# mateomarin/two_towers

Hardware: AMD Instinct MI355X
Metric: training pairs/sec at global batch=8192, 1/2/4/8 GPUs; MRR@10 match (higher is better)
Workload: dtype bf16; 1 GPU; BASELINE configs[2]: EnhancedTwoTowerModel(300, 256), seq_len 64, batch 8192 per GPU, bf16, hard-negative mining k=5 + margin 0.2, dropout 0.1, Adam; global_batch=8192, seq_len=64, hidden=256, embedding_dim=300, parallelism=dp1, loss=hardneg_margin

## Files before the change

include/tt_hip.h:

```cpp
#ifndef TT_HIP_H
#define TT_HIP_H
#include <stdint.h>

#ifdef __cplusplus
extern "C" {
#endif

#define TT_OK 0
#define TT_EINVAL 1000
#define TT_DT_F32 0
#define TT_DT_BF16 1

const char* tt_version(void);
const char* tt_last_error(void);
int tt_set_option(const char* name, int value);
int tt_get_option(const char* name, int* value);

int tt_embed_gather(int dtype, const void* table, long vocab, int ep, const int32_t* ids, long n,
                    void* out, void* stream);

int tt_pack_rows(int dtype, const float* src, long n, int e, int ep, void* out, void* stream);
typedef struct {
  const float* src;
  const float* src2;
  void* dst;
  int rows, cols, dcols;
  long lds, ldd;
  int dst_bf16;
} tt_pack_job;
int tt_pack_multi(const tt_pack_job* jobs, int njobs, void* stream);

int tt_cast(int dtype, const float* x, long n, void* y, void* stream);

int tt_colsum(const float* x, long rows, int cols, long ld, float* out, int accumulate, void* stream);

typedef struct {
  const void* a[4];
  const void* b[4];
  void* c[4];
  const float* bias[4];
  int bshift[4];
  const void* a_hi[4];
  int a_split;
  uint32_t drop_row0;
} tt_gemm_batch;

int tt_gemm(int dtype, int out_dtype, int a_kouter, int b_kouter, int m, int n, int k,
            const tt_gemm_batch* batch, int nbatch, long lda, long ldb, long ldc, float alpha,
            int beta_accum, int relu, int seq_t, uint32_t drop_seed, float drop_p, int splits,
            float* splitk_ws, void* stream);
long tt_gemm_ws_size(int m, int n, int nbatch, int splits);
int tt_gemm_pick_splits(int m, int n, int k, int nbatch);

typedef struct {
  const void* g;
  const void* whh;
  const float* bhn;
  void* y;
  void* x1;
  void* save;
  float* hstate;
  int dir;
  uint32_t drop_seed;
  int drop_col0;
  uint32_t drop_row0;
} tt_gru_fwd_rec;

int tt_gru_fwd(int dtype, const tt_gru_fwd_rec* recs, int nrec, int B, int T, int H, long ldg,
               long ldy, float drop_p, void* ws, long ws_bytes, void* stream);
int tt_gru_fwd_launches(int dtype, int T, int H);
long tt_gru_fwd_ws_size(int dtype, int nrec, int B, int T, int H, long ldg, long ldy);
int tt_gru_fwd_launches_for(int dtype, int nrec, int B, int T, int H, long ldg, long ldy);

typedef struct {
  const void* g; const void* whh; const float* bhn;
  void* y;
  void* hfinal;
  void* scratch;
  int dir;
} tt_gru_infer_rec;
int  tt_gru_fwd_infer(int dtype, const tt_gru_infer_rec* recs, int nrec, int B, int T, int H, long ldg,
                      long ldy, long ldf, void* ws, long ws_bytes, void* stream);
long tt_gru_infer_scratch_size(int dtype, int B, int T, int H, int final_only);

typedef struct {
  const void* save;
  const void* y;
  const void* dy;
  const float* dfinal;
  const void* whh;
  void* dgx;
  void* dgh;
  void* dhstate;
  float* dbias_part;
  int dir;
} tt_gru_bwd_rec;

int tt_gru_bwd(int dtype, const tt_gru_bwd_rec* recs, int nrec, int B, int T, int H, long ldy,
               long ldd, long ldf, void* stream);
int tt_gru_bwd_launches(int dtype, int T, int H);
int tt_gru_bwd_carry_on_chip(int dtype, int T, int H);
int tt_gru_bias_rows(int B);

typedef struct {
  const void* w1; const float* b1; const float* ln_g; const float* ln_b;
  const void* w2; const float* b2;
  const void* x;
  void* p1;
  float* mean;
  float* rstd;
  void* u;
  float* out;
} tt_head_fwd_io;

int tt_proj_head_fwd(int dtype, const tt_head_fwd_io* io, int ntower, int B, int h, float ln_eps,
                     void* stream);

typedef struct {
  const void* w1; const float* ln_g; const float* ln_b; const void* w2;
  const void* x; const void* p1; const float* mean; const float* rstd; const void* u;
  const float* dout;
  float* dx;
  float* dw1; float* db1; float* dg; float* dbeta; float* dw2; float* db2;
  void* ws;
} tt_head_bwd_io;

int tt_proj_head_bwd(int dtype, const tt_head_bwd_io* io, int ntower, int B, int h, float ln_eps,
                     void* stream);
long tt_proj_head_bwd_ws_size(int dtype, int B, int h);

typedef struct {
  const void* x;
  const void* w1; const float* b1; const float* ln_g; const float* ln_b;
  void* p1;
  float* mean;
  float* rstd;
  float* out;
} tt_head1_fwd_io;

int tt_proj_head1_fwd(int dtype, const tt_head1_fwd_io* io, long rows, int C, float ln_eps, float drop_p,
                      uint32_t drop_seed, void* stream);

typedef struct {
  const void* x; const void* w1; const float* ln_g; const float* ln_b;
  const void* p1; const float* mean; const float* rstd;
  const float* dout;
  float* dx;
  float* dw1; float* db1; float* dg; float* dbeta;
  void* ws;
} tt_head1_bwd_io;

int tt_proj_head1_bwd(int dtype, const tt_head1_bwd_io* io, long rows, int C, float drop_p, uint32_t drop_seed,
                      void* stream);
long tt_proj_head1_bwd_ws_size(int dtype, long rows, int C);

int tt_l2norm_fwd(int dtype, const float* x, long rows, int cols, float eps, void* y, float* y32,
                  float* norm, void* stream);
int tt_l2norm_bwd(const float* dy, const float* y32, const float* norm, long rows, int cols,
                  float eps, float* dx, int accumulate, void* stream);

int tt_infonce_fwd(int dtype, const void* qn, long bq, const void* dn, long nd, int h,
                   float inv_tau, float offdiag_sub, long label_offset, float* lse,
                   float* row_loss, void* ws, void* stream);
long tt_infonce_fwd_ws_size(long bq, long nd);
int tt_infonce_bwd(int dtype, const void* qn, long bq, const void* dn, long nd, int h,
                   float inv_tau, float offdiag_sub, long label_offset, const float* lse,
                   const float* gscale, float* dqn, float* ddn, void* ws, void* stream);
long tt_infonce_bwd_ws_size(int dtype, long bq, long nd, int h);

int tt_hardneg_topk(int dtype, const void* qn, long bq, const void* dn, long nd, int h,
                    long label_offset, int k, int32_t* idx, float* val, void* ws, void* stream);
long tt_hardneg_ws_size(int dtype, long bq, long nd, int h, int k);

int tt_search_topk(int dtype, const float* qn, long Q, const void* dn, long N, int h, int k,
                   int32_t* idx, float* val, void* ws, void* stream);
long tt_search_ws_size(int dtype, long Q, long N, int h, int k);

int tt_margin_fwd(const float* qn, long bq, const float* dn, long nd, int h, long label_offset,
                  const int32_t* idx, int k, float margin, float* row_loss, void* stream);
int tt_margin_bwd(const float* qn, long bq, const float* dn, long nd, int h, long label_offset,
                  const int32_t* idx, int k, float margin, const float* gscale, float* dqn, float* ddn,
                  void* ws, void* stream);
long tt_margin_bwd_ws_size(long bq, long nd, int h, int k);

int tt_sum(const float* x, long n, float scale, float* out, void* stream);
// ... 10 lines not shown
```

two_towers_amd/_lib.py:

```python
from __future__ import annotations

import contextlib
import ctypes
import os
from ctypes import POINTER, c_float, c_int, c_long, c_uint32, c_void_p

import torch

_HERE = os.path.dirname(os.path.abspath(__file__))
LIB_PATH = os.environ.get("TT_HIP_LIB", os.path.join(_HERE, "lib", "libtt_hip.so"))

DT_F32 = 0
DT_BF16 = 1
TT_EINVAL = 1000


class TTError(RuntimeError):
    pass


class GruTimeoutError(TTError):
    """A column-split GRU forward launch gave up waiting for one of its member workgroups
    (tt_gru_fwd's status word): that launch's outputs are invalid."""


class GemmBatch(ctypes.Structure):
    _fields_ = [
        ("a", c_void_p * 4),
        ("b", c_void_p * 4),
        ("c", c_void_p * 4),
        ("bias", c_void_p * 4),
        ("bshift", c_int * 4),
        ("a_hi", c_void_p * 4),
        ("a_split", c_int),
        ("drop_row0", c_uint32),
    ]


class PackJob(ctypes.Structure):
    _fields_ = [
        ("src", c_void_p),
        ("src2", c_void_p),
        ("dst", c_void_p),
        ("rows", c_int),
        ("cols", c_int),
        ("dcols", c_int),
        ("lds", c_long),
        ("ldd", c_long),
        ("dst_bf16", c_int),
    ]


class GruFwdRec(ctypes.Structure):
    _fields_ = [
        ("g", c_void_p), ("whh", c_void_p), ("bhn", c_void_p), ("y", c_void_p), ("x1", c_void_p),
        ("save", c_void_p), ("hstate", c_void_p), ("dir", c_int), ("drop_seed", c_uint32),
        ("drop_col0", c_int), ("drop_row0", c_uint32),
    ]


class GruInferRec(ctypes.Structure):
    _fields_ = [
        ("g", c_void_p), ("whh", c_void_p), ("bhn", c_void_p), ("y", c_void_p), ("hfinal", c_void_p),
        ("scratch", c_void_p), ("dir", c_int),
    ]


class GruBwdRec(ctypes.Structure):
    _fields_ = [
        ("save", c_void_p), ("y", c_void_p), ("dy", c_void_p), ("dfinal", c_void_p), ("whh", c_void_p),
        ("dgx", c_void_p), ("dgh", c_void_p), ("dhstate", c_void_p), ("dbias_part", c_void_p),
        ("dir", c_int),
    ]


class HeadFwdIO(ctypes.Structure):
    _fields_ = [
        ("w1", c_void_p), ("b1", c_void_p), ("ln_g", c_void_p), ("ln_b", c_void_p), ("w2", c_void_p),
        ("b2", c_void_p), ("x", c_void_p), ("p1", c_void_p), ("mean", c_void_p), ("rstd", c_void_p),
        ("u", c_void_p), ("out", c_void_p),
    ]


class HeadBwdIO(ctypes.Structure):
    _fields_ = [
        ("w1", c_void_p), ("ln_g", c_void_p), ("ln_b", c_void_p), ("w2", c_void_p), ("x", c_void_p),
        ("p1", c_void_p), ("mean", c_void_p), ("rstd", c_void_p), ("u", c_void_p), ("dout", c_void_p),
        ("dx", c_void_p), ("dw1", c_void_p), ("db1", c_void_p), ("dg", c_void_p), ("dbeta", c_void_p),
        ("dw2", c_void_p), ("db2", c_void_p), ("ws", c_void_p),
    ]


class Head1FwdIO(ctypes.Structure):
    _fields_ = [
        ("x", c_void_p), ("w1", c_void_p), ("b1", c_void_p), ("ln_g", c_void_p), ("ln_b", c_void_p),
        ("p1", c_void_p), ("mean", c_void_p), ("rstd", c_void_p), ("out", c_void_p),
    ]


class Head1BwdIO(ctypes.Structure):
    _fields_ = [
        ("x", c_void_p), ("w1", c_void_p), ("ln_g", c_void_p), ("ln_b", c_void_p), ("p1", c_void_p),
        ("mean", c_void_p), ("rstd", c_void_p), ("dout", c_void_p), ("dx", c_void_p), ("dw1", c_void_p),
        ("db1", c_void_p), ("dg", c_void_p), ("dbeta", c_void_p), ("ws", c_void_p),
    ]


_SIGS = {
    "tt_version": (ctypes.c_char_p, []),
    "tt_last_error": (ctypes.c_char_p, []),
    "tt_set_option": (c_int, [ctypes.c_char_p, c_int]),
    "tt_get_option": (c_int, [ctypes.c_char_p, POINTER(c_int)]),
    "tt_embed_gather": (c_int, [c_int, c_void_p, c_long, c_int, c_void_p, c_long, c_void_p, c_void_p]),
    "tt_pack_rows": (c_int, [c_int, c_void_p, c_long, c_int, c_int, c_void_p, c_void_p]),
    "tt_pack_multi": (c_int, [c_void_p, c_int, c_void_p]),
    "tt_cast": (c_int, [c_int, c_void_p, c_long, c_void_p, c_void_p]),
    "tt_colsum": (c_int, [c_void_p, c_long, c_int, c_long, c_void_p, c_int, c_void_p]),
    "tt_gemm": (c_int, [c_int, c_int, c_int, c_int, c_int, c_int, c_int, POINTER(GemmBatch), c_int, c_long,
                        c_long, c_long, c_float, c_int, c_int, c_int, c_uint32, c_float, c_int, c_void_p,
                        c_void_p]),
    "tt_gemm_ws_size": (c_long, [c_int, c_int, c_int, c_int]),
    "tt_gemm_pick_splits": (c_int, [c_int, c_int, c_int, c_int]),
    "tt_gru_fwd": (c_int, [c_int, POINTER(GruFwdRec), c_int, c_int, c_int, c_int, c_long, c_long, c_float,
                           c_void_p, c_long, c_void_p]),
    "tt_gru_bwd": (c_int, [c_int, POINTER(GruBwdRec), c_int, c_int, c_int, c_int, c_long, c_long, c_long,
                           c_void_p]),
    "tt_gru_bias_rows": (c_int, [c_int]),
    "tt_gru_bwd_launches": (c_int, [c_int, c_int, c_int]),
    "tt_gru_bwd_carry_on_chip": (c_int, [c_int, c_int, c_int]),
    "tt_gru_fwd_launches": (c_int, [c_int, c_int, c_int]),
    "tt_gru_fwd_ws_size": (c_long, [c_int, c_int, c_int, c_int, c_int, c_long, c_long]),
    "tt_gru_fwd_launches_for": (c_int, [c_int, c_int, c_int, c_int, c_int, c_long, c_long]),
    "tt_gru_fwd_infer": (c_int, [c_int, POINTER(GruInferRec), c_int, c_int, c_int, c_int, c_long, c_long, c_long,
                                 c_void_p, c_long, c_void_p]),
    "tt_gru_infer_scratch_size": (c_long, [c_int, c_int, c_int, c_int, c_int]),
    "tt_proj_head_fwd": (c_int, [c_int, POINTER(HeadFwdIO), c_int, c_int, c_int, c_float, c_void_p]),
    "tt_proj_head_bwd": (c_int, [c_int, POINTER(HeadBwdIO), c_int, c_int, c_int, c_float, c_void_p]),
    "tt_proj_head_bwd_ws_size": (c_long, [c_int, c_int, c_int]),
    "tt_proj_head1_fwd": (c_int, [c_int, POINTER(Head1FwdIO), c_long, c_int, c_float, c_float, c_uint32,
                                  c_void_p]),
    "tt_proj_head1_bwd": (c_int, [c_int, POINTER(Head1BwdIO), c_long, c_int, c_float, c_uint32, c_void_p]),
    "tt_proj_head1_bwd_ws_size": (c_long, [c_int, c_long, c_int]),
    "tt_l2norm_fwd": (c_int, [c_int, c_void_p, c_long, c_int, c_float, c_void_p, c_void_p, c_void_p, c_void_p]),
    "tt_l2norm_bwd": (c_int, [c_void_p, c_void_p, c_void_p, c_long, c_int, c_float, c_void_p, c_int, c_void_p]),
    "tt_infonce_fwd": (c_int, [c_int, c_void_p, c_long, c_void_p, c_long, c_int, c_float, c_float, c_long,
                               c_void_p, c_void_p, c_void_p, c_void_p]),
    "tt_infonce_fwd_ws_size": (c_long, [c_long, c_long]),
    "tt_infonce_bwd": (c_int, [c_int, c_void_p, c_long, c_void_p, c_long, c_int, c_float, c_float, c_long,
                               c_void_p, c_void_p, c_void_p, c_void_p, c_void_p, c_void_p]),
    "tt_infonce_bwd_ws_size": (c_long, [c_int, c_long, c_long, c_int]),
    "tt_hardneg_topk": (c_int, [c_int, c_void_p, c_long, c_void_p, c_long, c_int, c_long, c_int, c_void_p,
                                c_void_p, c_void_p, c_void_p]),
    "tt_hardneg_ws_size": (c_long, [c_int, c_long, c_long, c_int, c_int]),
    "tt_search_topk": (c_int, [c_int, c_void_p, c_long, c_void_p, c_long, c_int, c_int, c_void_p, c_void_p,
                               c_void_p, c_void_p]),
    "tt_search_ws_size": (c_long, [c_int, c_long, c_long, c_int, c_int]),
    "tt_margin_fwd": (c_int, [c_void_p, c_long, c_void_p, c_long, c_int, c_long, c_void_p, c_int, c_float,
                              c_void_p, c_void_p]),
    "tt_margin_bwd": (c_int, [c_void_p, c_long, c_void_p, c_long, c_int, c_long, c_void_p, c_int, c_float,
                              c_void_p, c_void_p, c_void_p, c_void_p, c_void_p]),
    "tt_margin_bwd_ws_size": (c_long, [c_long, c_long, c_int, c_int]),
    "tt_sum": (c_int, [c_void_p, c_long, c_float, c_void_p, c_void_p]),
    "tt_adam_multi": (c_int, [POINTER(c_void_p), POINTER(c_void_p), POINTER(c_void_p), POINTER(c_void_p),
                              POINTER(c_long), c_int, c_float, c_float, c_float, c_float, c_float, c_int,
                              c_void_p, c_void_p]),
}

EXPORTED = tuple(_SIGS)

_lib = None
_load_error: str | None = None


def load():
    global _lib, _load_error
    if _lib is not None:
        return _lib
    if _load_error is not None:
        raise TTError(_load_error)
    if not os.path.exists(LIB_PATH):
        _load_error = (f"two_towers_amd: native library not found at {LIB_PATH}; "
                       "build it with `python -c 'import __graft_entry__ as g; g.build()'` (hipcc, gfx950)")
        raise TTError(_load_error)
    lib = ctypes.CDLL(LIB_PATH, mode=ctypes.RTLD_GLOBAL)
    for name, (res, args) in _SIGS.items():
        fn = getattr(lib, name)
        fn.restype = res
        fn.argtypes = args
    _lib = lib
    return lib


def check(rc: int, what: str = ""):
    if rc != 0:
        msg = _lib.tt_last_error().decode(errors="replace") if _lib is not None else ""
        raise TTError(f"{what or 'tt_hip'} failed (rc={rc}): {msg}")


def call(name: str, *args):
    lib = load()
    check(getattr(lib, name)(*args), name)


def get_option(name: str) -> int:
    v = c_int(0)
    call("tt_get_option", name.encode(), ctypes.byref(v))
    return v.value


def set_option(name: str, value: int) -> int:
# ... 43 lines not shown
```

two_towers_amd/csrc/tt_elem.hip:

```cpp
#include <algorithm>

#include "tt_api.h"
#include "tt_common.h"

namespace {

__global__ __launch_bounds__(256) void embed_gather_kernel(const uint4* __restrict__ table, long vocab,
                                                           int cpr, const int32_t* __restrict__ ids,
                                                           long n, uint4* __restrict__ out) {
  const long total = n * cpr;
  for (long e = (long)blockIdx.x * 256 + threadIdx.x; e < total; e += (long)gridDim.x * 256) {
    const long row = e / cpr;
    const int c = (int)(e - row * cpr);
    const int id = ids[row];
    uint4 v = make_uint4(0, 0, 0, 0);
    if (id >= 0 && id < vocab) v = table[(long)id * cpr + c];
    out[e] = v;
  }
}

template <typename T>
__global__ __launch_bounds__(256) void pack_rows_kernel(const float* __restrict__ src, long n, int e, int ep,
                                                        T* __restrict__ out) {
  const long total = n * ep;
  for (long i = (long)blockIdx.x * 256 + threadIdx.x; i < total; i += (long)gridDim.x * 256) {
    const long r = i / ep;
    const int c = (int)(i - r * ep);
    Elt<T>::st(out + i, c < e ? src[r * e + c] : 0.f);
  }
}

template <typename T>
__global__ __launch_bounds__(256) void cast_kernel(const float* __restrict__ x, long n, T* __restrict__ y) {
  for (long i = (long)blockIdx.x * 256 + threadIdx.x; i < n; i += (long)gridDim.x * 256) Elt<T>::st(y + i, x[i]);
}

__global__ __launch_bounds__(1024) void colsum_kernel(const float* __restrict__ x, long rows, int cols, long ld,
                                                      int accumulate, float* __restrict__ out) {
  __shared__ float red[16][64];
  const int wave = threadIdx.x >> 6, lane = threadIdx.x & 63;
  const int c = blockIdx.x * 64 + lane;
  float s = 0.f;
  if (c < cols)
    for (long r = wave; r < rows; r += 16) s += x[r * ld + c];
  red[wave][lane] = s;
  __syncthreads();
  if (wave == 0 && c < cols) {
    float t = 0.f;
#pragma unroll
    for (int w = 0; w < 16; ++w) t += red[w][lane];
    out[c] = accumulate ? out[c] + t : t;
  }
}

__global__ __launch_bounds__(256) void sum_kernel(const float* __restrict__ x, long n, float scale,
                                                  float* __restrict__ out) {
  __shared__ float part[4];
  float s = 0.f;
  for (long i = threadIdx.x; i < n; i += 256) s += x[i];
  s = wave_sum(s);
  if ((threadIdx.x & 63) == 0) part[threadIdx.x >> 6] = s;
  __syncthreads();
  if (threadIdx.x == 0) out[0] = scale * (part[0] + part[1] + part[2] + part[3]);
}

struct PackArgs {
  tt_pack_job j[16];
  long start[17];
  int n;
};
__global__ __launch_bounds__(256) void pack_multi_kernel(PackArgs a) {
  const long total = a.start[a.n];
  for (long i = blockIdx.x * 256L + threadIdx.x; i < total; i += (long)gridDim.x * 256) {
    int k = 0;
    while (k + 1 < a.n && i >= a.start[k + 1]) ++k;
    const tt_pack_job& J = a.j[k];
    const long q = i - a.start[k];
    const int g4 = J.dcols / 4;
    const long r = q / g4;
    const int c = (int)(q - r * g4) * 4;
    float4 v = make_float4(0.f, 0.f, 0.f, 0.f);
    if (c < J.cols) {
      v = *reinterpret_cast<const float4*>(J.src + r * J.lds + c);
      if (J.src2) {
        const float4 w = *reinterpret_cast<const float4*>(J.src2 + r * J.lds + c);
        v.x += w.x; v.y += w.y; v.z += w.z; v.w += w.w;
      }
    }
    if (J.dst_bf16) {
      const uint2 o = make_uint2((uint32_t)f2bf(v.x) | ((uint32_t)f2bf(v.y) << 16),
                                 (uint32_t)f2bf(v.z) | ((uint32_t)f2bf(v.w) << 16));
      *reinterpret_cast<uint2*>(static_cast<bf16_t*>(J.dst) + r * J.ldd + c) = o;
    } else {
      *reinterpret_cast<float4*>(static_cast<float*>(J.dst) + r * J.ldd + c) = v;
    }
  }
}

inline unsigned grid_for(long work, int per_block = 256, int cap = 8192) {
  long g = (work + per_block - 1) / per_block;
  if (g < 1) g = 1;
  return (unsigned)std::min<long>(g, cap);
}

}

extern "C" int tt_embed_gather(int dtype, const void* table, long vocab, int ep, const int32_t* ids, long n,
                               void* out, void* stream) {
  TT_CHECK_ARG(dtype == TT_DT_F32 || dtype == TT_DT_BF16, "tt_embed_gather: bad dtype");
  const int esz = dtype == TT_DT_BF16 ? 2 : 4;
  TT_CHECK_ARG((ep * esz) % 16 == 0, "tt_embed_gather: ep*sizeof(dtype) must be a multiple of 16 (ep=%d)", ep);
  if (n == 0) return 0;
  const int cpr = ep * esz / 16;
  hipLaunchKernelGGL(embed_gather_kernel, dim3(grid_for(n * cpr)), dim3(256), 0, (hipStream_t)stream,
                     (const uint4*)table, vocab, cpr, ids, n, (uint4*)out);
  TT_CHECK_LAUNCH("embed_gather_kernel");
  return 0;
}

extern "C" int tt_pack_rows(int dtype, const float* src, long n, int e, int ep, void* out, void* stream) {
  TT_CHECK_ARG(ep >= e, "tt_pack_rows: ep < e");
  if (n == 0) return 0;
  dim3 g(grid_for(n * ep));
  if (dtype == TT_DT_BF16)
    hipLaunchKernelGGL(pack_rows_kernel<bf16_t>, g, dim3(256), 0, (hipStream_t)stream, src, n, e, ep, (bf16_t*)out);
  else
    hipLaunchKernelGGL(pack_rows_kernel<float>, g, dim3(256), 0, (hipStream_t)stream, src, n, e, ep, (float*)out);
  TT_CHECK_LAUNCH("pack_rows_kernel");
  return 0;
}

extern "C" int tt_pack_multi(const tt_pack_job* jobs, int njobs, void* stream) {
  TT_CHECK_ARG(njobs >= 0 && njobs <= 16 && (njobs == 0 || jobs), "tt_pack_multi: njobs %d not in [0,16]", njobs);
  PackArgs a{};
  a.n = njobs;
  a.start[0] = 0;
  for (int k = 0; k < njobs; ++k) {
    const tt_pack_job& J = jobs[k];
    TT_CHECK_ARG(J.src && J.dst && J.rows >= 0 && J.cols >= 0 && J.dcols >= J.cols, "tt_pack_multi: job %d", k);
    TT_CHECK_ARG(J.cols % 4 == 0 && J.dcols % 4 == 0 && J.lds % 4 == 0 && J.ldd % 4 == 0 && J.lds >= J.cols &&
                     J.ldd >= J.dcols,
                 "tt_pack_multi: job %d: cols, dcols and leading dimensions must be multiples of 4", k);
    const bool src_ok = ((uintptr_t)J.src | (uintptr_t)J.src2) % 16 == 0;
    TT_CHECK_ARG(src_ok && (uintptr_t)J.dst % (J.dst_bf16 ? 8 : 16) == 0, "tt_pack_multi: job %d: misaligned operand", k);
    a.j[k] = J;
    a.start[k + 1] = a.start[k] + (long)J.rows * (J.dcols / 4);
  }
  if (a.start[njobs] == 0) return 0;
  hipLaunchKernelGGL(pack_multi_kernel, dim3(grid_for(a.start[njobs], 256, 4096)), dim3(256), 0, (hipStream_t)stream, a);
  TT_CHECK_LAUNCH("pack_multi_kernel");
  return 0;
}

extern "C" int tt_cast(int dtype, const float* x, long n, void* y, void* stream) {
  if (n == 0) return 0;
  dim3 g(grid_for(n));
  if (dtype == TT_DT_BF16)
    hipLaunchKernelGGL(cast_kernel<bf16_t>, g, dim3(256), 0, (hipStream_t)stream, x, n, (bf16_t*)y);
  else
    hipLaunchKernelGGL(cast_kernel<float>, g, dim3(256), 0, (hipStream_t)stream, x, n, (float*)y);
  TT_CHECK_LAUNCH("cast_kernel");
  return 0;
}

extern "C" int tt_colsum(const float* x, long rows, int cols, long ld, float* out, int accumulate, void* stream) {
  hipStream_t st = (hipStream_t)stream;
  if (cols == 0) return 0;
  if (rows == 0) {
    if (!accumulate) TT_CHECK_HIP(hipMemsetAsync(out, 0, sizeof(float) * cols, st));
    return 0;
  }
  hipLaunchKernelGGL(colsum_kernel, dim3(tt_ceil_div(cols, 64)), dim3(1024), 0, st, x, rows, cols, ld, accumulate,
                     out);
  TT_CHECK_LAUNCH("colsum_kernel");
  return 0;
}

extern "C" int tt_sum(const float* x, long n, float scale, float* out, void* stream) {
  hipLaunchKernelGGL(sum_kernel, dim3(1), dim3(256), 0, (hipStream_t)stream, x, n, scale, out);
  TT_CHECK_LAUNCH("sum_kernel");
  return 0;
}
```

two_towers_amd/csrc/tt_gemm.hip:

```cpp
#include <float.h>
#include <stdarg.h>
#include <stdlib.h>

#include <atomic>
#include <type_traits>

#include "tt_api.h"
#include "tt_gemm_core.h"

namespace tt {
static thread_local char g_err[512];
void set_error(const char* fmt, ...) {
  va_list ap;
  va_start(ap, fmt);
  vsnprintf(g_err, sizeof(g_err), fmt, ap);
  va_end(ap);
}
}

namespace tt {
namespace {
struct OptDef {
  const char* name;
  const char* env;
// ... 927 lines not shown
          if (i >= i0 && i < i0 + 2)
#pragma unroll
            for (int j = 0; j < 4; ++j)
#pragma unroll
              for (int rr = 0; rr < 4; ++rr)
                stg[(16 * (i - i0) + 4 * (lane >> 4) + rr) * 256 + wn + 16 * j + (lane & 15)] = acc[i][j][rr];
      }
      asm volatile("s_waitcnt lgkmcnt(0)" ::: "memory");
      __builtin_amdgcn_s_barrier();
#pragma unroll
      for (int k = 0; k < 2; ++k) {
        const int rl = rlo + 16 * k;
        const int gm = m0 + p * 32 + rl, gn = n0 + cg;
        if (gm < g.M && gn < g.N) {
          float v[8];
          const float4 x0 = *reinterpret_cast<const float4*>(stg + rl * 256 + cg);
          const float4 x1 = *reinterpret_cast<const float4*>(stg + rl * 256 + cg + 4);
          v[0] = x0.x; v[1] = x0.y; v[2] = x0.z; v[3] = x0.w; v[4] = x1.x; v[5] = x1.y; v[6] = x1.z; v[7] = x1.w;
#pragma unroll
          for (int e = 0; e < 8; ++e) {
            float x = v[e] * g.alpha + bv[e];
            if (g.relu) x = fmaxf(x, 0.f);
            if (g.drop_thresh) x *= tt_dropout_scale(g.drop_seed, g.drop_row0 + (uint32_t)gm, gn + e, g.drop_thresh, g.drop_inv_keep);
            v[e] = x;
          }
          TO* dst = C + (long)gm * g.ldc + gn;
          if (gn + 8 <= g.N && g.vec_ok) {
            if (g.stream_out)
              st8_sc1(crs, (int)(((long)(gm - m0) * g.ldc + (gn - n0)) * (long)sizeof(TO)), v, (TO*)nullptr);
            else
              st8(dst, v);
          } else {
            for (int e = 0; e < 8 && gn + e < g.N; ++e) Elt<TO>::st(dst + e, v[e]);
          }
        }
      }
      __builtin_amdgcn_s_barrier();
    }
    if (late && qn < qend) __builtin_amdgcn_s_barrier();
  }
  if constexpr (IE && A3 && !HN && PERSIST_BAL && std::is_same<TO, bf16_t>::value) {
    if (have_prev) {
      iepi(C0{}, C0{});
      iepi(C0{}, C1{});
      iepi(C1{}, C1{});
      iepi(C1{}, C0{});
    }
  }
  if constexpr (A3)
    if (!late) __builtin_amdgcn_s_barrier();
  asm volatile("s_waitcnt vmcnt(0)" ::: "memory");
}

template <typename TO, int V>
__global__ __launch_bounds__(256) void splitk_reduce_kernel(const float* ws, long part_stride, int splits,
                                                            int M, int N, GemmArgs g) {
  const int bi = blockIdx.y;
  const float* P = ws + (long)bi * splits * part_stride;
  TO* C = static_cast<TO*>(g.c[bi]);
  const float* bias = g.bias[bi];
  const long total = (long)M * N / V;
  for (long e = (long)blockIdx.x * 256 + threadIdx.x; e < total; e += (long)gridDim.x * 256) {
    float v[V];
    if constexpr (V == 4) {
      float4 a = make_float4(0.f, 0.f, 0.f, 0.f);
      for (int s = 0; s < splits; ++s) {
        const float4 b = reinterpret_cast<const float4*>(P + (long)s * part_stride)[e];
        a.x += b.x;
        a.y += b.y;
        a.z += b.z;
        a.w += b.w;
      }
      v[0] = a.x, v[1] = a.y, v[2] = a.z, v[3] = a.w;
    } else {
      v[0] = 0.f;
      for (int s = 0; s < splits; ++s) v[0] += P[(long)s * part_stride + e];
    }
    const int m = (int)(e * V / N), n0 = (int)(e * V % N);
#pragma unroll
    for (int u = 0; u < V; ++u) {
      float x = v[u] * g.alpha;
      if (bias) x += bias[n0 + u];
      TO* p = C + (long)m * g.ldc + n0 + u;
      if (g.beta) x += Elt<TO>::ld(p);
      Elt<TO>::st(p, x);
    }
  }
}

template <typename T, typename TO, int TBM, int TBN, int WGM, int WGN, bool DMA, bool A3 = false, bool BUF = false>
int launch_t(int akout, int bkout, bool shift, const GemmArgs& g, long nwg, hipStream_t st) {
  dim3 grid((unsigned)nwg), blk(64 * WGM * WGN);
#define TT_L(AK, BK, SH) \
  hipLaunchKernelGGL((gemm_kernel<T, AK, BK, SH, TO, TBM, TBN, WGM, WGN, DMA, A3, BUF>), grid, blk, 0, st, g)
  if (!akout && !bkout) TT_L(false, false, false);
  else if (!akout && bkout && !shift) TT_L(false, true, false);
  else if (!akout && bkout && shift) TT_L(false, true, true);
  else if (akout && !bkout) TT_L(true, false, false);
  else if (akout && bkout && !shift) TT_L(true, true, false);
  else TT_L(true, true, true);
#undef TT_L
  TT_CHECK_LAUNCH("gemm_kernel");
  return 0;
}

inline bool use_big(int m, int n, long tiles256) { return m >= 256 && n >= 256 && tiles256 >= 256; }

template <typename T, typename TO>
int launch_persist(int akout, int bkout, bool shift, const GemmArgs& g0, int ntiles, bool buf, hipStream_t st) {
  dim3 grid((unsigned)std::min(ntiles, 256)), blk(512);
  GemmArgs g = g0;
  g.walk_g = g.walk_x = 0;
  if (tt::opt(tt::OPT_GEMM_ORDER) && ntiles % 256 == 0 && ((g.N + 255) / 256) % 4 == 0) {
    g.walk_g = 4;
    g.walk_x = 8;
  }
#define TT_L(AK, BK, SH, A3, BUF) \
  hipLaunchKernelGGL((gemm_persist<T, AK, BK, SH, TO, A3, BUF>), grid, blk, 0, st, g, ntiles)
#define TT_L2(AK, BK, SH) \
  do {                     \
    if (a3 && buf) TT_L(AK, BK, SH, true, true); \
    else if (a3) TT_L(AK, BK, SH, true, false); \
    else TT_L(AK, BK, SH, false, false);   \
  } while (0)
  const bool a3 = tt::opt(tt::OPT_GEMM_A3) != 0;
  if constexpr (std::is_same<TO, bf16_t>::value) {
    if (PERSIST_IEPI && tt::opt(tt::OPT_GEMM_IEPI) && !akout && !bkout && !shift && a3 && buf && g.M % 256 == 0 &&
        g.N % 256 == 0 && g.vec_ok && g.bias_vec_ok && g.alpha == 1.f && !g.relu && !g.drop_thresh && !g.beta &&
        g.stream_out <= 2 && g.force_regstage == 0) {
      hipLaunchKernelGGL((gemm_persist<T, false, false, false, TO, true, true, false, true>), grid, blk, 0, st, g, ntiles);
      TT_CHECK_LAUNCH("gemm_persist");
      return 0;
    }
  }
  if (!akout && !bkout) TT_L2(false, false, false);
  else if (!akout && bkout && !shift) TT_L2(false, true, false);
  else if (!akout && bkout && shift) TT_L2(false, true, true);
  else if (akout && !bkout) TT_L2(true, false, false);
  else if (akout && bkout && !shift) TT_L2(true, true, false);
  else TT_L2(true, true, true);
#undef TT_L2
#undef TT_L
  TT_CHECK_LAUNCH("gemm_persist");
  return 0;
}

#ifndef W4_LEAD
#define W4_LEAD 2
#endif
namespace w4 {
constexpr int SLOT = 32768;
constexpr int NS = 4;
struct Frags {
  uint4 a[8], b[8];
};
TT_DEV uint4 frag(const char* img, int r0) {
  const int lane = threadIdx.x & 63;
  const int row = r0 + (lane & 15);
  return *reinterpret_cast<const uint4*>(img + row * 64 + (((lane >> 4) ^ ((row >> 1) & 3)) << 4));
}
}

template <bool RS>
__global__ __launch_bounds__(256, 1) void gemm_w4(GemmArgs g, int ntm, int ntn) {
  constexpr int NSL = RS ? 3 : w4::NS;
  __shared__ __attribute__((aligned(16))) char lds[NSL * w4::SLOT];
// ... 267 lines not shown
  }
  hipLaunchKernelGGL((gemm_persist<bf16_t, false, false, false, float, true, true, true>),
                     dim3((unsigned)std::min<long>(ntiles, 256)), dim3(512), 0, st, g, (int)ntiles);
  TT_CHECK_LAUNCH("gemm_persist (hard-negative scan)");
  return 0;
}

extern "C" long tt_gemm_ws_size(int m, int n, int nbatch, int splits) {
  (void)m;
  return splits > 1 ? (long)m * n * nbatch * splits : 0;
}

extern "C" int tt_gemm_pick_splits(int m, int n, int k, int nbatch) {
  const bool big = m >= 256 && n >= 256;
  const long tiles = big ? (long)tt_ceil_div(m, 256) * tt_ceil_div(n, 256) * nbatch
                         : (long)tt_ceil_div(m, BM) * tt_ceil_div(n, BN) * nbatch;
  const long target = big ? 512 : 1024;
  if (tiles >= target) return 1;
  const int smax = std::max(1, std::min(64, tt_ceil_div(k, 64) / 8));
  int best = 1;
  double best_eff = 0.0;
  const int s_lo = (int)std::min<long>(smax, std::max<long>(1, target / tiles));
  for (int s = s_lo; s <= std::min<long>(smax, 3 * target / tiles + 1); ++s) {
    const long w = tiles * s;
    const double eff = (double)w / (256.0 * (double)tt_ceil_div(w, 256));
    if (eff > best_eff + 1e-9) { best_eff = eff; best = s; }
  }
  return std::min(best, smax);
}

extern "C" int tt_gemm(int dtype, int out_dtype, int a_kouter, int b_kouter, int m, int n, int k,
                       const tt_gemm_batch* batch, int nbatch, long lda, long ldb, long ldc,
                       float alpha, int beta_accum, int relu, int seq_t, uint32_t drop_seed,
                       float drop_p, int splits, float* splitk_ws, void* stream) {
  TT_CHECK_ARG(dtype == TT_DT_F32 || dtype == TT_DT_BF16, "tt_gemm: bad dtype %d", dtype);
  TT_CHECK_ARG(out_dtype == TT_DT_F32 || out_dtype == dtype, "tt_gemm: bad out_dtype %d", out_dtype);
  TT_CHECK_ARG(nbatch >= 1 && nbatch <= 4, "tt_gemm: nbatch %d not in [1,4]", nbatch);
  TT_CHECK_ARG(m >= 0 && n >= 0 && k >= 0, "tt_gemm: negative dims");
  if (m == 0 || n == 0) return 0;
  const int esz = dtype == TT_DT_BF16 ? 2 : 4;
  const int epc = 16 / esz;
  (void)epc;
  TT_CHECK_ARG((lda * esz) % 16 == 0 && (ldb * esz) % 16 == 0,
               "tt_gemm: leading dimensions must be 16-byte multiples (lda=%ld ldb=%ld)", lda, ldb);
  if (splits < 1) splits = 1;
  TT_CHECK_ARG(splits == 1 || (relu == 0 && drop_p == 0.f), "tt_gemm: split-K excludes relu/dropout");
  TT_CHECK_ARG(splits == 1 || splitk_ws != nullptr, "tt_gemm: split-K needs a workspace");
  TT_CHECK_ARG(drop_p >= 0.f && drop_p < 1.f, "tt_gemm: drop_p %f", drop_p);
  bool shift = false;
  GemmArgs g{};
  for (int b = 0; b < nbatch; ++b) {
    TT_CHECK_ARG(batch->a[b] && batch->b[b] && batch->c[b], "tt_gemm: null operand in batch %d", b);
    TT_CHECK_ARG(((uintptr_t)batch->a[b] | (uintptr_t)batch->b[b]) % 16 == 0,
                 "tt_gemm: operands must be 16-byte aligned (batch %d)", b);
    g.a[b] = batch->a[b];
    g.b[b] = batch->b[b];
    g.c[b] = batch->c[b];
    g.bias[b] = batch->bias[b];
    g.bshift[b] = batch->bshift[b];
    g.a_hi[b] = batch->a_hi[b];
    if (batch->a_split > 0)
      TT_CHECK_ARG(batch->a_hi[b] && (uintptr_t)batch->a_hi[b] % 16 == 0, "tt_gemm: a_hi[%d] null or misaligned", b);
    if (batch->bshift[b] != 0) shift = true;
  }
  TT_CHECK_ARG(!shift || (b_kouter && seq_t > 0), "tt_gemm: bshift needs b_kouter and seq_t");
  TT_CHECK_ARG(batch->a_split >= 0 && (batch->a_split == 0 || (a_kouter && batch->a_split % (16 / esz) == 0)),
               "tt_gemm: a_split %d needs a_kouter and a 16-byte multiple", batch->a_split);
  g.a_split = batch->a_split;
  g.lda = lda; g.ldb = ldb; g.ldc = ldc;
  g.M = m; g.N = n; g.K = k;
  g.alpha = alpha; g.beta = beta_accum; g.relu = relu; g.seq_t = seq_t;
  g.force_regstage = tt::opt(tt::OPT_GEMM_REGSTAGE);
  g.nbatch = nbatch;
  g.skew = tt::opt(tt::OPT_GEMM_SKEW);
  g.drop_seed = drop_seed;
  g.drop_row0 = batch->drop_row0;
  g.drop_thresh = drop_p > 0.f ? (uint32_t)(drop_p * 16777216.0f + 0.5f) : 0u;
  g.drop_inv_keep = drop_p > 0.f ? 1.0f / (1.0f - drop_p) : 1.0f;
  const int nk = tt_ceil_div((long)k * esz, 128);
  if (splits > nk) splits = nk > 0 ? nk : 1;
  g.kt_per_split = nk > 0 ? tt_ceil_div(nk, splits) : 1;
  splits = nk > 0 ? tt_ceil_div(nk, g.kt_per_split) : 1;
  g.splits = splits;
  {
    const int osz = out_dtype == TT_DT_BF16 ? 2 : 4;
    bool ok = (ldc * osz) % 16 == 0;
    for (int b = 0; b < nbatch; ++b) ok = ok && ((uintptr_t)batch->c[b] % 16 == 0);
    g.vec_ok = ok;
    bool bok = true;
    for (int b = 0; b < nbatch; ++b) bok = bok && ((uintptr_t)batch->bias[b] % 16 == 0);
    g.bias_vec_ok = bok;
    g.stream_out = ok && (long)m * n * osz >= (64L << 20) && (long)256 * ldc * osz < (1L << 31);
    g.stream_out = g.stream_out ? tt::opt(tt::OPT_GEMM_STREAM_OUT) : 0;
  }
  hipStream_t st = static_cast<hipStream_t>(stream);
  TT_CHECK_ARG((long)tt_ceil_div(m, 128) * tt_ceil_div(n, 128) * nbatch * splits < (1L << 31), "tt_gemm: too many tiles");

  if (splits > 1) {
    GemmArgs gp = g;
    gp.part_stride = (long)m * n;
    gp.vec_ok = (n % 4 == 0);
    for (int b = 0; b < nbatch; ++b) gp.c[b] = splitk_ws + (long)b * splits * gp.part_stride;
    int rc = dtype == TT_DT_BF16 ? launch_gemm<bf16_t, float>(a_kouter, b_kouter, shift, gp, nbatch, st)
                                 : launch_gemm<float, float>(a_kouter, b_kouter, shift, gp, nbatch, st);
    if (rc) return rc;
    const bool v4 = n % 4 == 0 && (uintptr_t)splitk_ws % 16 == 0;
    const long total = (long)m * n / (v4 ? 4 : 1);
    dim3 rg((unsigned)std::min<long>(tt_ceil_div(total, 256), 2048), nbatch);
#define TT_RED(TO, V) hipLaunchKernelGGL((splitk_reduce_kernel<TO, V>), rg, dim3(256), 0, st, splitk_ws, gp.part_stride, splits, m, n, g)
    if (out_dtype == TT_DT_F32) {
      if (v4) TT_RED(float, 4); else TT_RED(float, 1);
    } else {
      if (v4) TT_RED(bf16_t, 4); else TT_RED(bf16_t, 1);
    }
#undef TT_RED
    TT_CHECK_LAUNCH("splitk_reduce_kernel");
    return 0;
  }
  if (dtype == TT_DT_BF16) {
    return out_dtype == TT_DT_BF16 ? launch_gemm<bf16_t, bf16_t>(a_kouter, b_kouter, shift, g, nbatch, st)
                                   : launch_gemm<bf16_t, float>(a_kouter, b_kouter, shift, g, nbatch, st);
  }
  return launch_gemm<float, float>(a_kouter, b_kouter, shift, g, nbatch, st);
}
```

two_towers_amd/csrc/tt_gru.hip:

```cpp
#include <algorithm>
#include <cstdlib>
#include <mutex>
#include <type_traits>

#include "tt_api.h"
#include "tt_gemm_core.h"

namespace {

struct FwdRec {
  const void* g; const void* whh; const float* bhn; void* y; void* x1; void* save; float* hs;
  int dir; uint32_t seed; int col0;
  uint32_t row0;
};
struct FwdArgs {
  FwdRec r[4];
  int B, T, H;
  long ldg, ldy;
  int s;
  uint32_t drop_thresh;
  float inv_keep;
#ifdef TT_DIAG
  int dbg;
#endif
};
struct InfArgs : FwdArgs {
  void* hfin[4];
  void* himg[4];
  long ldf;
};
TT_DEV void* inf_hfin(const FwdArgs&, int) { return nullptr; }
TT_DEV void* inf_hfin(const InfArgs& a, int rz) { return a.hfin[rz]; }
TT_DEV long inf_ldf(const FwdArgs&) { return 0; }
TT_DEV long inf_ldf(const InfArgs& a) { return a.ldf; }

struct BwdRec {
  const void* save; const void* y; const void* dy; const float* dfinal; const void* whh;
  void* dgx; void* dgh; void* dh; float* dbias; int dir;
};
struct BwdArgs {
  BwdRec r[4];
  int B, T, H;
  long ldy, ldd, ldf;
  int s;
  int skew;
#ifdef TT_DIAG
  int dbg;
#endif
};


TT_DEV void gru_cell(float xr, float xz, float xn, float lr, float lz, float ln, float bn, float hp, float& y,
                     float& ar, float& az, float& an, float& ghn) {
#pragma clang fp contract(off)
  constexpr float L2E = 0x1.715476p+0f;
  ghn = ln + bn;
  ar = xr + lr;
  az = xz + lz;
  const float rg = __builtin_amdgcn_rcpf(1.0f + __builtin_amdgcn_exp2f(L2E * -ar));
  const float zg = __builtin_amdgcn_rcpf(1.0f + __builtin_amdgcn_exp2f(L2E * -az));
  an = __builtin_fmaf(rg, ghn, xn);
  const float ng = 1.0f - 2.0f * __builtin_amdgcn_rcpf(__builtin_amdgcn_exp2f(L2E * (2.0f * an)) + 1.0f);
  y = __builtin_fmaf(zg, hp, (1.0f - zg) * ng);
}

template <typename T>
struct GateRows {
  static constexpr bool SHIFTED = false, KSPLIT = false;
  const T* w; int H, j0;
  TT_DEV const T* rowptr(int r) const {
    const int half = r / 96, rem = r - half * 96;
    const int g = rem >> 5, j = j0 + half * 32 + (rem & 31);
    return j < H ? w + (long)(g * H + j) * H : nullptr;
  }
  TT_DEV const T* at(int r, int k) const { const T* p = rowptr(r); return p ? p + k : nullptr; }
};

template <typename T, int BMR, int NS = 2, typename A = FwdArgs>
__global__ __launch_bounds__(2 * BMR) void gru_fwd_step(A a) {
  constexpr bool INF = std::is_same_v<A, InfArgs>;
  constexpr int NT = 2 * BMR;
  using ML = ttg::DLoop<T, false, false, BMR, 192, BMR / 64, 2, NS>;
  __shared__ __attribute__((aligned(16))) char lds[ML::LDS_BYTES];
  const int ntj = (a.H + 63) / 64, ntm = (a.B + BMR - 1) / BMR;
  const int id = ttg::xcd_remap(blockIdx.x, gridDim.x);
  const int rz = id / (ntm * ntj), rem = id - rz * ntm * ntj;
  const FwdRec R = a.r[rz];
  const int H = a.H, T_ = a.T, s = a.s;
  const int m0 = (rem / ntj) * BMR, j0 = (rem % ntj) * 64;
  const int t = R.dir ? T_ - 1 - s : s;
  const int tp = R.dir ? t + 1 : t - 1;
  const T* Y = static_cast<const T*>(R.y);

  f32x4 acc[ML::TM][ML::TN];
#pragma unroll
  for (int i = 0; i < ML::TM; ++i)
#pragma unroll
    for (int j = 0; j < ML::TN; ++j) acc[i][j] = f32x4{0.f, 0.f, 0.f, 0.f};
  bool prod = s > 0, epi = true;
#ifdef TT_DIAG
  if (a.dbg & 8) prod = false;
  if (a.dbg & 16) epi = false;
#endif
  const int tid = threadIdx.x;
  const int cur = s & 1, prv = cur ^ 1;
  const T* G = static_cast<const T*>(R.g);
  const float* hs_prv = R.hs + (long)prv * a.B * H;
  if (prod) {
    ttg::KCPlain<T> la{Y + (long)tp * a.ldy, (long)T_ * a.ldy, m0, a.B};
    if constexpr (INF) {
      if (!Y) la = ttg::KCPlain<T>{static_cast<const T*>(a.himg[rz]) + (long)prv * a.B * H, (long)H, m0, a.B};
    }
    GateRows<T> lb{static_cast<const T*>(R.whh), H, j0};
    const int nk = (H * (int)sizeof(T) + ttg::KTB - 1) / ttg::KTB;
    ML::run(la, lb, H, 0, nk, lds, acc);
  }
  if (!epi) {
    if (acc[0][0][0] == 1.2345f) static_cast<T*>(R.y)[0] = T(0);
    return;
  }

  const int wave = threadIdx.x >> 6, lane = threadIdx.x & 63;
  float* L = reinterpret_cast<float*>(lds);
  constexpr int FLD = 68;
  T* Yw = static_cast<T*>(R.y);
  T* X1 = static_cast<T*>(R.x1);
  T* S = static_cast<T*>(R.save);
  float* hs_cur = R.hs + (long)cur * a.B * H;
  const __amdgpu_buffer_rsrc_t srs = tt_rsrc(S + ((long)m0 * T_ + t) * (4L * H));
  const __amdgpu_buffer_rsrc_t xrs = tt_rsrc(X1 ? X1 + ((long)m0 * T_ + t) * a.ldy : Yw);
  for (int hf = 0; hf < BMR / 64; ++hf) {
    if ((wave >> 1) == hf) {
      const int nb = (wave & 1) * 32;
#pragma unroll
      for (int g = 0; g < 3; ++g)
#pragma unroll
        for (int i = 0; i < 4; ++i)
#pragma unroll
          for (int jh = 0; jh < 2; ++jh)
#pragma unroll
            for (int r = 0; r < 4; ++r)
              L[(g * 64 + 16 * i + 4 * (lane >> 4) + r) * FLD + nb + 16 * jh + (lane & 15)] = acc[i][g * 2 + jh][r];
    }
    __syncthreads();
#pragma unroll
    for (int k = 0; k < 512 / NT; ++k) {
      const int rl = (tid >> 3) + (NT / 8) * k, jg = (tid & 7) * 8;
      const int b = m0 + hf * 64 + rl, j = j0 + jg;
      if (b < a.B && j < H) {
        const long row = (long)b * T_ + t;
        float xr[8], xz[8], xn[8], hp[8], bn[8], y[8], sr[8], sz[8], sn[8], sg[8];
        ld8(G + row * a.ldg + j, xr);
        ld8(G + row * a.ldg + H + j, xz);
        ld8(G + row * a.ldg + 2 * H + j, xn);
        ld8(R.bhn + j, bn);
        if (s > 0) ld8(hs_prv + (long)b * H + j, hp);
        else {
#pragma unroll
          for (int e = 0; e < 8; ++e) hp[e] = 0.f;
        }
        const float* Lr = L + (0 * 64 + rl) * FLD + jg;
        const float* Lz = L + (1 * 64 + rl) * FLD + jg;
        const float* Ln = L + (2 * 64 + rl) * FLD + jg;
#pragma unroll
        for (int e = 0; e < 8; ++e)
          gru_cell(xr[e], xz[e], xn[e], Lr[e], Lz[e], Ln[e], bn[e], hp[e], y[e], sr[e], sz[e], sn[e], sg[e]);
        st8(hs_cur + (long)b * H + j, y);
        if constexpr (INF) {
          if (Yw) st8(Yw + row * a.ldy + j, y);
          else st8(static_cast<T*>(a.himg[rz]) + ((long)cur * a.B + b) * H + j, y);
          T* hf = static_cast<T*>(a.hfin[rz]);
          if (hf && s == T_ - 1) st8(hf + (long)b * a.ldf + j, y);
          continue;
        }
        st8(Yw + row * a.ldy + j, y);
        const int so = (int)((((long)(b - m0) * T_) * 4L * H + j) * (long)sizeof(T));
        st8_sc1(srs, so, sr, (T*)nullptr);
        st8_sc1(srs, so + H * (int)sizeof(T), sz, (T*)nullptr);
        st8_sc1(srs, so + 2 * H * (int)sizeof(T), sn, (T*)nullptr);
        st8_sc1(srs, so + 3 * H * (int)sizeof(T), sg, (T*)nullptr);
        if (X1) {
#pragma unroll
          for (int e = 0; e < 8; ++e)
            y[e] *= a.drop_thresh ? tt_dropout_scale(R.seed, R.row0 + (uint32_t)row, (uint32_t)(R.col0 + j + e),
                                                     a.drop_thresh, a.inv_keep)
                                  : 1.f;
          st8_sc1(xrs, (int)((((long)(b - m0) * T_) * a.ldy + j) * (long)sizeof(T)), y, (T*)nullptr);
        }
      }
    }
    __syncthreads();
  }
}

template <typename T, int BMR, int NS = 2>
__global__ __launch_bounds__(256) void gru_bwd_step(BwdArgs a) {
  using ML = ttg::DLoop<T, false, true, BMR, 128, 2, 2, NS>;
  constexpr int LDSB = ML::LDS_BYTES > 64 * 132 * 4 ? ML::LDS_BYTES : 64 * 132 * 4;
  __shared__ __attribute__((aligned(16))) char lds[LDSB];
  const int ntj = (a.H + 127) / 128, ntm = (a.B + BMR - 1) / BMR;
  const int id = ttg::xcd_remap(blockIdx.x, gridDim.x);
  const int rz = id / (ntm * ntj), rem = id - rz * ntm * ntj;
  const int mt = rem / ntj;
  const BwdRec R = a.r[rz];
  const int H = a.H, T_ = a.T, s = a.s;
  const int m0 = mt * BMR, j0 = (rem % ntj) * 128;
  const int t = R.dir ? T_ - 1 - s : s;
  const int tn = R.dir ? t - 1 : t + 1;
  const int tp = R.dir ? t + 1 : t - 1;
  const bool last = (s == T_ - 1);
  const T* DGX = static_cast<const T*>(R.dgx);
  const T* DGH = static_cast<const T*>(R.dgh);

  f32x4 acc[ML::TM][ML::TN];
#pragma unroll
  for (int i = 0; i < ML::TM; ++i)
#pragma unroll
    for (int j = 0; j < ML::TN; ++j) acc[i][j] = f32x4{0.f, 0.f, 0.f, 0.f};
  if (!last) {
    ttg::KCSplit<T> la{DGX + (long)tn * a.ldd, DGH + (long)tn * a.ldd, (long)T_ * a.ldd, m0, a.B, 2 * H};
    ttg::KOPlain<T> lb{static_cast<const T*>(R.whh), H, j0, H - j0};
    const int K = 3 * H;
    const int nk = (K * (int)sizeof(T) + ttg::KTB - 1) / ttg::KTB;
    ML::run(la, lb, K, 0, nk, lds, acc);
  }

  const int wave = threadIdx.x >> 6, lane = threadIdx.x & 63, tid = threadIdx.x;
  float* L = reinterpret_cast<float*>(lds);
  constexpr int BLD = 132;
  const int cur = s & 1, nxt = cur ^ 1;
  const T* S = static_cast<const T*>(R.save);
  const T* Y = static_cast<const T*>(R.y);
  const T* DY = static_cast<const T*>(R.dy);
  T* DGXw = static_cast<T*>(R.dgx);
  T* DGHw = static_cast<T*>(R.dgh);
  T* cr_cur = static_cast<T*>(R.dh) + (long)cur * a.B * H;
  const T* cr_nxt = static_cast<const T*>(R.dh) + (long)nxt * a.B * H;
  const long S4 = 4L * H;
  const int jg = (tid & 15) * 8;
  const int j = j0 + jg;
  const __amdgpu_buffer_rsrc_t grs = tt_rsrc(DGXw + ((long)m0 * T_ + t) * a.ldd);
  float bsum[4][8];
#pragma unroll
  for (int q = 0; q < 4; ++q)
#pragma unroll
    for (int e = 0; e < 8; ++e) bsum[q][e] = 0.f;
  for (int hf = 0; hf < BMR / 64; ++hf) {
    const int wrow = (wave >> 1) * (BMR / 2) - hf * 64;
    if (wrow >= 0 && wrow < 64) {
      const int wn = (wave & 1) * 64;
#pragma unroll
      for (int i = 0; i < ML::TM; ++i)
#pragma unroll
        for (int jt = 0; jt < 4; ++jt)
#pragma unroll
          for (int r = 0; r < 4; ++r)
            L[(wrow + 16 * i + 4 * (lane >> 4) + r) * BLD + wn + 16 * jt + (lane & 15)] = acc[i][jt][r];
    }
// ... 870 lines not shown
      bn[4] = bn1.x; bn[5] = bn1.y; bn[6] = bn1.z; bn[7] = bn1.w;
#pragma unroll
      for (int h = 0; h < 2; ++h) {
        const float4 v0 = *reinterpret_cast<const float4*>(stg + stg_off(rl, 0 * 64 + jg + 4 * h));
        const float4 v1 = *reinterpret_cast<const float4*>(stg + stg_off(rl, 1 * 64 + jg + 4 * h));
        const float4 v2 = *reinterpret_cast<const float4*>(stg + stg_off(rl, 2 * 64 + jg + 4 * h));
        lr[4 * h] = v0.x; lr[4 * h + 1] = v0.y; lr[4 * h + 2] = v0.z; lr[4 * h + 3] = v0.w;
        lz[4 * h] = v1.x; lz[4 * h + 1] = v1.y; lz[4 * h + 2] = v1.z; lz[4 * h + 3] = v1.w;
        ln[4 * h] = v2.x; ln[4 * h + 1] = v2.y; ln[4 * h + 2] = v2.z; ln[4 * h + 3] = v2.w;
      }
#pragma unroll
      for (int e = 0; e < 8; ++e) {
#ifdef TT_DIAG
        if (a.dbg & 4) {
          sg[e] = ln[e] + bn[e];
          sr[e] = xr[e] + lr[e]; sz[e] = xz[e] + lz[e];
          const float rg = sr[e] * 0.25f + 0.5f, zg = sz[e] * 0.25f + 0.5f;
          sn[e] = xn[e] + rg * sg[e];
          y[e] = (1.f - zg) * sn[e] * 0.5f + zg * hreg[0][e];
          continue;
        }
#endif
        gru_cell(xr[e], xz[e], xn[e], lr[e], lz[e], ln[e], bn[e], hreg[0][e], y[e], sr[e], sz[e], sn[e], sg[e]);
      }
      float ynew[8];
#pragma unroll
      for (int e = 0; e < 8; ++e) ynew[e] = y[e];
      {
        const uint32_t oy = sok ? (uint32_t)(lrow * (int)a.ldy + j) * 2u : 0x80000000u;
        const uint32_t os = sok ? (uint32_t)(lrow * 4 * H + j) * 2u : 0x80000000u;
        st16_buf(rY, oy, 0, pack8bf(y));
        if constexpr (INF) {
          const uint32_t of = sok && s == T_ - 1 ? (uint32_t)(rl * (int)a.ldf + j) * 2u : 0x80000000u;
          st16_buf(rS, os, 0, pack8bf(y));
          st16_buf(rS, os, 2 * H, pack8bf(y));
          st16_buf(rS, os, 4 * H, pack8bf(y));
          st16_buf(rS, os, 6 * H, pack8bf(y));
          st16_buf(rX1, of, 0, pack8bf(y));
        } else {
          st16_buf(rS, os, 0, pack8bf(sr));
          st16_buf(rS, os, 2 * H, pack8bf(sz));
          st16_buf(rS, os, 4 * H, pack8bf(sn));
          st16_buf(rS, os, 6 * H, pack8bf(sg));
          if (X1 && a.drop_thresh) {
#pragma unroll
            for (int e = 0; e < 8; ++e)
              y[e] *= tt_dropout_scale(R.seed, R.row0 + (uint32_t)row, (uint32_t)(R.col0 + j + e), a.drop_thresh,
                                       a.inv_keep);
          }
          st16_buf(rX1, oy, 0, pack8bf(y));
        }
      }
      TT_STAMP(e2);
      TT_ACC(4, e2 - e1);
#pragma unroll
      for (int i = 0; i < PH_MAX / 64 - 1; ++i)
#pragma unroll
        for (int e = 0; e < 8; ++e) hreg[i][e] = hreg[i + 1][e];
#pragma unroll
      for (int e = 0; e < 8; ++e) hreg[PH_MAX / 64 - 1][e] = ynew[e];
    }
    for (int r = nblk; r < PH_MAX / 64; ++r) {
#pragma unroll
      for (int e = 0; e < 8; ++e) {
        const float v = hreg[0][e];
#pragma unroll
        for (int i = 0; i < PH_MAX / 64 - 1; ++i) hreg[i][e] = hreg[i + 1][e];
        hreg[PH_MAX / 64 - 1][e] = v;
      }
    }
#pragma unroll
    for (int i = 0; i < PH_MAX / 64; ++i) {
      if (i < nblk) {
        uint32_t w[4];
#pragma unroll
        for (int k = 0; k < 4; ++k)
          w[k] = (uint32_t)f2bf(hreg[i][2 * k]) | ((uint32_t)f2bf(hreg[i][2 * k + 1]) << 16);
        *reinterpret_cast<uint4*>(hb + i * (PR * ttg::KTB) + ttg::kc_off(rl, tid & 7)) =
            make_uint4(w[0], w[1], w[2], w[3]);
      }
    }
    __syncthreads();
  }
#ifdef TT_DIAG
  TT_STAMP(k_end);
  prf[7] = k_end - k_start;
  if (threadIdx.x == 0 && blockIdx.x < 2048)
    for (int i = 0; i < 8; ++i) g_fwd_prof[blockIdx.x][i] = prf[i];
#endif
}

typedef __attribute__((address_space(1))) unsigned xc_gu32;
#ifndef XC_G_AUX
#define XC_G_AUX 2
#endif
#ifndef XC_OUT_AUX
#define XC_OUT_AUX 2
#endif
#ifndef XC_VALU_PER_MFMA
#define XC_VALU_PER_MFMA 3
#endif
namespace xc {
constexpr int NT = 256;
constexpr int CR = 32;
constexpr int RR = 256;
constexpr int NCH = RR / CR;
constexpr int SSTR = 68;
constexpr int STG = CR * 192 * 4;
constexpr int CSTR = 64;
constexpr unsigned OOB = 0x80000000u;
template <int H>
struct Cfg {
  static constexpr int M = H / 64;
  static constexpr int NKT = H / 32;
  static constexpr int QPW = H / 64;
  static constexpr int SLOT = CR * H * 2;
  static constexpr int ST = RR * SSTR * 4;
  static constexpr int LDS = ST + 2 * SLOT + STG;
};
static_assert(Cfg<512>::LDS <= 163840 && Cfg<256>::LDS <= 163840, "gru_fwd_xc LDS budget");
}

struct XcWs {
  bf16_t* xb;
  unsigned* cnt;
  unsigned* err;
  unsigned* status;
  unsigned spins;
  int skip;
  int xmap;
  int qg;
  int nrec;
  int rpg;
  int nround;
  int fast_ok;
  int skew;
};

TT_DEV void xc_wait(xc_gu32* cnt, unsigned target, const XcWs& ws) {
  xc_gu32* err = (xc_gu32*)(uintptr_t)ws.err;
  for (unsigned spins = 0;; ++spins) {
    if (__hip_atomic_load(cnt, __ATOMIC_RELAXED, __HIP_MEMORY_SCOPE_AGENT) >= target) return;
    if ((spins & 1023u) == 1023u) {
      if (__hip_atomic_load(err, __ATOMIC_RELAXED, __HIP_MEMORY_SCOPE_AGENT) != 0u) return;
      if (spins > ws.spins) {
        __hip_atomic_store(err, 1u, __ATOMIC_RELAXED, __HIP_MEMORY_SCOPE_AGENT);
        __hip_atomic_fetch_or((xc_gu32*)(uintptr_t)ws.status, 1u, __ATOMIC_RELAXED, __HIP_MEMORY_SCOPE_AGENT);
        return;
      }
    }
    __builtin_amdgcn_s_sleep(1);
  }
}

TT_DEV bool xc_group_on_one_xcd(unsigned* cntw, int M, int mem, bool allowed, const XcWs& ws) {
  __shared__ int s_fast;
  if (threadIdx.x == 0) {
    unsigned xcc;
    asm volatile("s_getreg_b32 %0, hwreg(HW_REG_XCC_ID)" : "=s"(xcc));
    xc_gu32* w = (xc_gu32*)(uintptr_t)cntw;
    __hip_atomic_store(w + 8 + mem, (xcc & 15u) + 1u, __ATOMIC_RELAXED, __HIP_MEMORY_SCOPE_AGENT);
    asm volatile("s_waitcnt vmcnt(0)" ::: "memory");
    __hip_atomic_fetch_add(w + 1, 1u, __ATOMIC_RELAXED, __HIP_MEMORY_SCOPE_AGENT);
    xc_wait(w + 1, (unsigned)M, ws);
    unsigned first = __hip_atomic_load(w + 8, __ATOMIC_RELAXED, __HIP_MEMORY_SCOPE_AGENT);
    bool same = allowed && first != 0u;
    for (int m = 1; m < M; ++m) same &= __hip_atomic_load(w + 8 + m, __ATOMIC_RELAXED, __HIP_MEMORY_SCOPE_AGENT) == first;
    s_fast = same ? 1 : 0;
  }
  __syncthreads();
  return s_fast != 0;
}

template <int H>
TT_DEV void xc_h_offsets(uint32_t (&ho)[xc::Cfg<H>::QPW]) {
  const int lane = threadIdx.x & 63, w = threadIdx.x >> 6;
#pragma unroll
  for (int p = 0; p < xc::Cfg<H>::QPW; ++p) {
    const int q = w * xc::Cfg<H>::QPW + p, kt = q >> 1, rb = q & 1;
    ho[p] = (uint32_t)(((rb * 16 + (lane & 15)) * H + kt * 32 + (lane >> 4) * 8) * 2);
  }
}
template <int H>
TT_DEV void xc_load_h(__amdgpu_buffer_rsrc_t rx, const uint32_t (&ho)[xc::Cfg<H>::QPW], int c,
                      tt_u32x4 (&hv)[xc::Cfg<H>::QPW]) {
#pragma unroll
  for (int p = 0; p < xc::Cfg<H>::QPW; ++p)
    hv[p] = __builtin_amdgcn_raw_buffer_load_b128(rx, (int)ho[p], c * xc::CR * H * 2, 16);
}
template <int H>
TT_DEV void xc_put_h(char* slot, const tt_u32x4 (&hv)[xc::Cfg<H>::QPW]) {
  const int lane = threadIdx.x & 63, w = threadIdx.x >> 6;
#pragma unroll
// ... 88 lines not shown
  }
  const bf16_t* G = static_cast<const bf16_t*>(R.g);
  bf16_t* Yw = static_cast<bf16_t*>(R.y);
  bf16_t* X1 = static_cast<bf16_t*>(R.x1);
  bf16_t* S = static_cast<bf16_t*>(R.save);
  const bool fast = xc_group_on_one_xcd(ws.cnt + grp * xc::CSTR, M, mem, ws.fast_ok != 0, ws);
  if (ws.skew > 0 && (grp & 1))
    for (int i = 0; i < ws.skew; ++i) __builtin_amdgcn_s_sleep(127);
  const int NS = ws.nround * T_;
  struct Step {
    int s, t, rb0, nrow;
  };
  auto step_of = [&](int idx) {
    Step q;
    const int r = idx / T_;
    q.s = idx - r * T_;
    q.t = R.dir ? T_ - 1 - q.s : q.s;
    q.rb0 = gb0 + r * xc::RR;
    q.nrow = min(min(ws.rpg - r * xc::RR, xc::RR), B - q.rb0);
    return q;
  };
  auto g_rsrc = [&](const Step& q) {
    return tt_rsrc_n(G + (long)(q.nrow > 0 ? q.rb0 : 0) * T_ * a.ldg, q.nrow > 0);
  };
  auto load_g = [&](const Step& q, __amdgpu_buffer_rsrc_t rG, int c, tt_u32x4 (&gx)[3]) {
    const uint32_t og = c * xc::CR + cr < q.nrow ? (uint32_t)(((c * xc::CR + cr) * T_ + q.t) * (int)a.ldg + j) * 2u
                                                  : xc::OOB;
#pragma unroll
    for (int g = 0; g < 3; ++g) gx[g] = __builtin_amdgcn_raw_buffer_load_b128(rG, (int)og, g * H * 2, XC_G_AUX);
  };
  tt_u32x4 hv[C::QPW];
  auto load_h = [&](const Step& q, int qidx, int c) {
    if (q.s == 0) {
#pragma unroll
      for (int p = 0; p < C::QPW; ++p) hv[p] = tt_u32x4{0u, 0u, 0u, 0u};
    } else {
      xc_load_h<H>(rx[(qidx - 1) & 1], ho, c, hv);
    }
  };
  float lr[8], lz[8], ln[8], hp[8];
  auto read_gates = [&](int c, bool first) {
    const int rr = c * xc::CR + cr;
#pragma unroll
    for (int h = 0; h < 2; ++h) {
      const float4 v0 = *reinterpret_cast<const float4*>(stg + stg_off(cr, 0 * 64 + u0 + 4 * h));
      const float4 v1 = *reinterpret_cast<const float4*>(stg + stg_off(cr, 1 * 64 + u0 + 4 * h));
      const float4 v2 = *reinterpret_cast<const float4*>(stg + stg_off(cr, 2 * 64 + u0 + 4 * h));
      const float4 p = *reinterpret_cast<const float4*>(stt + rr * xc::SSTR + u0 + 4 * h);
      lr[4 * h] = v0.x; lr[4 * h + 1] = v0.y; lr[4 * h + 2] = v0.z; lr[4 * h + 3] = v0.w;
      lz[4 * h] = v1.x; lz[4 * h + 1] = v1.y; lz[4 * h + 2] = v1.z; lz[4 * h + 3] = v1.w;
      ln[4 * h] = v2.x; ln[4 * h + 1] = v2.y; ln[4 * h + 2] = v2.z; ln[4 * h + 3] = v2.w;
      hp[4 * h] = first ? 0.f : p.x; hp[4 * h + 1] = first ? 0.f : p.y;
      hp[4 * h + 2] = first ? 0.f : p.z; hp[4 * h + 3] = first ? 0.f : p.w;
    }
  };
  f32x4 acc[2][3];
  for (int i = tid; i < 2 * C::SLOT / 16; i += xc::NT)
    reinterpret_cast<float4*>(slots)[i] = make_float4(0.f, 0.f, 0.f, 0.f);
  Step cur = step_of(0);
  __amdgpu_buffer_rsrc_t rGc = g_rsrc(cur);
  tt_u32x4 gq[2][3];
  load_g(cur, rGc, 0, gq[0]);
#pragma unroll
  for (int p = 0; p < C::QPW; ++p) hv[p] = tt_u32x4{0u, 0u, 0u, 0u};
  __syncthreads();
  xc_mfma<H>(slots, wa, acc);
  xc_stage(stg, acc);
  __syncthreads();
  read_gates(0, true);
  for (int idx = 0; idx < NS; ++idx) {
    const bool has_next = idx + 1 < NS;
    const Step nxt = step_of(has_next ? idx + 1 : idx);
    const __amdgpu_buffer_rsrc_t rGn = g_rsrc(nxt);
    const long r0w = (long)(cur.nrow > 0 ? cur.rb0 : 0) * T_;
    const bool on = cur.nrow > 0;
    bf16_t* HF = static_cast<bf16_t*>(inf_hfin(a, rz));
    const __amdgpu_buffer_rsrc_t rY =
        INF ? tt_rsrc_n(Yw ? (const void*)(Yw + r0w * a.ldy) : G, on && Yw != nullptr) : tt_rsrc_n(Yw + r0w * a.ldy, on);
    const __amdgpu_buffer_rsrc_t rX1 =
        INF ? tt_rsrc_n(HF ? (const void*)(HF + (long)(on ? cur.rb0 : 0) * inf_ldf(a)) : G, on && HF != nullptr && cur.s == T_ - 1)
            : tt_rsrc_n(X1 ? X1 + r0w * a.ldy : Yw, on && X1 != nullptr);
    const __amdgpu_buffer_rsrc_t rS = INF ? tt_rsrc_n(G, false) : tt_rsrc_n(S + r0w * 4L * H, on);
    const __amdgpu_buffer_rsrc_t rdst_h = rx[idx & 1];
    const int t = cur.t;
#pragma unroll
    for (int c = 0; c < xc::NCH; ++c) {
      const bool more = c + 1 < xc::NCH || has_next;
      if (c + 1 < xc::NCH) load_g(cur, rGc, c + 1, gq[(c + 1) & 1]);
      else if (has_next) load_g(nxt, rGn, 0, gq[0]);
      {
        const int rr = c * xc::CR + cr;
        const bool ok = rr < cur.nrow;
        float xr[8], xz[8], xn[8], y[8], sr[8], sz[8], sn[8], sg[8], msk[8];
        const uint32_t grow = (uint32_t)(cur.rb0 + rr) * (uint32_t)T_ + (uint32_t)t;
        const tt_u32x4(&gcur)[3] = gq[c & 1];
        unpack8(make_uint4(gcur[0][0], gcur[0][1], gcur[0][2], gcur[0][3]), xr);
        unpack8(make_uint4(gcur[1][0], gcur[1][1], gcur[1][2], gcur[1][3]), xz);
        unpack8(make_uint4(gcur[2][0], gcur[2][1], gcur[2][2], gcur[2][3]), xn);
        if (more) {
          const char* base = slots + ((c + 1) & 1) * C::SLOT + lane * 16;
          auto frag = [&](int kt, int rb) { return *reinterpret_cast<const tt_u32x4*>(base + (kt * 2 + rb) * 1024); };
#pragma unroll
          for (int rb = 0; rb < 2; ++rb)
#pragma unroll
            for (int g = 0; g < 3; ++g) acc[rb][g] = f32x4{0.f, 0.f, 0.f, 0.f};
          tt_u32x4 f[3][2];
          f[0][0] = frag(0, 0); f[0][1] = frag(0, 1);
          f[1][0] = frag(1, 0); f[1][1] = frag(1, 1);
          __builtin_amdgcn_sched_barrier(0);
#pragma unroll
          for (int kt = 0; kt < NKT; ++kt) {
            if (kt + 2 < NKT) {
              f[(kt + 2) % 3][0] = frag(kt + 2, 0);
              f[(kt + 2) % 3][1] = frag(kt + 2, 1);
            }
#pragma unroll
            for (int rb = 0; rb < 2; ++rb)
#pragma unroll
              for (int g = 0; g < 3; ++g)
                acc[rb][g] = __builtin_amdgcn_mfma_f32_16x16x32_bf16(
                    __builtin_bit_cast(bf16x8v, wa[g][kt]), __builtin_bit_cast(bf16x8v, f[kt % 3][rb]), acc[rb][g], 0, 0, 0);
            if constexpr (DROP) {
#pragma unroll
              for (int e = 0; e < 8; ++e)
                if (e * NKT / 8 == kt) {
                  msk[e] = tt_dropout_scale(R.seed, R.row0 + grow, (uint32_t)(R.col0 + j + e), a.drop_thresh, a.inv_keep);
                  asm volatile("" : "+v"(msk[e]));
                }
            }
#pragma unroll
            for (int e = 0; e < 8; ++e)
              if ((e + 1) * NKT / 8 - 1 == kt) {
                asm volatile("" : "+v"(xr[e]), "+v"(xz[e]), "+v"(xn[e]), "+v"(lr[e]), "+v"(lz[e]), "+v"(ln[e]),
                             "+v"(hp[e]));
                gru_cell(xr[e], xz[e], xn[e], lr[e], lz[e], ln[e], bn[e], hp[e], y[e], sr[e], sz[e], sn[e], sg[e]);
                asm volatile("" : "+v"(y[e]), "+v"(sr[e]), "+v"(sz[e]), "+v"(sn[e]), "+v"(sg[e]));
              }
#pragma unroll
            for (int i = 0; i < 6; ++i) {
              __builtin_amdgcn_sched_group_barrier(0x008, 1, 0);
              __builtin_amdgcn_sched_group_barrier(0x002, XC_VALU_PER_MFMA, 0);
            }
            __builtin_amdgcn_sched_barrier(0);
          }
        } else {
#pragma unroll
          for (int e = 0; e < 8; ++e) {
            gru_cell(xr[e], xz[e], xn[e], lr[e], lz[e], ln[e], bn[e], hp[e], y[e], sr[e], sz[e], sn[e], sg[e]);
            if constexpr (DROP)
              msk[e] = tt_dropout_scale(R.seed, R.row0 + grow, (uint32_t)(R.col0 + j + e), a.drop_thresh, a.inv_keep);
          }
        }
        *reinterpret_cast<float4*>(stt + rr * xc::SSTR + u0) = make_float4(y[0], y[1], y[2], y[3]);
        *reinterpret_cast<float4*>(stt + rr * xc::SSTR + u0 + 4) = make_float4(y[4], y[5], y[6], y[7]);
        const uint4 yb = pack8bf(y);
        if (fast) st16_buf(rdst_h, (uint32_t)(rr * H + j) * 2u, 0, yb);
        else st16_buf_sc1(rdst_h, (uint32_t)(rr * H + j) * 2u, 0, yb);
        asm volatile("" ::: "memory");
        const int lrow = rr * T_ + t;
        const uint32_t oy = ok ? (uint32_t)(lrow * (int)a.ldy + j) * 2u : xc::OOB;
        const uint32_t os = ok ? (uint32_t)(lrow * 4 * H + j) * 2u : xc::OOB;
        st16_buf_aux<XC_OUT_AUX>(rY, (int)oy, yb);
        if constexpr (INF) {
          st16_buf_aux<XC_OUT_AUX>(rS, (int)os, yb);
          st16_buf_aux<XC_OUT_AUX>(rS, (int)(os + 2u * H), yb);
          st16_buf_aux<XC_OUT_AUX>(rS, (int)(os + 4u * H), yb);
          st16_buf_aux<XC_OUT_AUX>(rS, (int)(os + 6u * H), yb);
          st16_buf_aux<XC_OUT_AUX>(rX1, (int)(ok ? (uint32_t)(rr * (int)a.ldf + j) * 2u : xc::OOB), yb);
        } else {
          st16_buf_aux<XC_OUT_AUX>(rS, (int)os, pack8bf(sr));
          st16_buf_aux<XC_OUT_AUX>(rS, (int)(os + 2u * H), pack8bf(sz));
          st16_buf_aux<XC_OUT_AUX>(rS, (int)(os + 4u * H), pack8bf(sn));
          st16_buf_aux<XC_OUT_AUX>(rS, (int)(os + 6u * H), pack8bf(sg));
          if constexpr (DROP) {
#pragma unroll
            for (int e = 0; e < 8; ++e) y[e] *= msk[e];
            st16_buf_aux<XC_OUT_AUX>(rX1, (int)oy, pack8bf(y));
          } else {
            st16_buf_aux<XC_OUT_AUX>(rX1, (int)oy, yb);
          }
        }
      }
      if (c == 3 || c == 7) asm volatile("s_nop 0\n\ts_waitcnt vmcnt(6)" ::: "memory");
      if (c + 2 < xc::NCH || has_next) xc_put_h<H>(slots + (c & 1) * C::SLOT, hv);
      if (c + 3 < xc::NCH) load_h(cur, idx, c + 3);
      else if (has_next) load_h(nxt, idx + 1, c + 3 - xc::NCH);
      if (tid == 0) {
        if (c == 0 && idx > 0) xc_wait(cntB, (unsigned)(M * idx), ws);
        if (c == 4 && has_next) xc_wait(cntA, (unsigned)(M * (idx + 1)), ws);
      }
      __syncthreads();
      if (tid == 0 && c == 3 && publish) __hip_atomic_fetch_add(cntA, 1u, __ATOMIC_RELAXED, __HIP_MEMORY_SCOPE_AGENT);
      if (tid == 0 && c == 7 && publish) __hip_atomic_fetch_add(cntB, 1u, __ATOMIC_RELAXED, __HIP_MEMORY_SCOPE_AGENT);
      if (more) {
        xc_stage(stg, acc);
        __syncthreads();
        if (c + 1 < xc::NCH) read_gates(c + 1, cur.s == 0);
        else read_gates(0, nxt.s == 0);
      }
    }
    cur = nxt;
    rGc = rGn;
  }
}

#ifndef XS_VPRIO
#define XS_VPRIO 0
#endif
#ifndef XS_MPUB
#define XS_MPUB 1
#endif
#ifndef XS_MPOLL
#define XS_MPOLL 1
#endif
#ifndef XS_GA
#define XS_GA 1
#endif
namespace xs {
constexpr int NT = 512;
template <int H>
struct Cfg {
  static constexpr int SLOT = xc::Cfg<H>::SLOT;
  static constexpr int LDS = 2 * SLOT + 2 * xc::STG;
};
static_assert(Cfg<512>::LDS <= 163840, "gru_fwd_xs LDS budget");
}

template <int H, bool DROP, typename A = FwdArgs>
__global__ __launch_bounds__(xs::NT, 1) __attribute__((amdgpu_waves_per_eu(2, 2))) void gru_fwd_xs(A a, XcWs ws) {
  constexpr bool INF = std::is_same_v<A, InfArgs>;
  static_assert(!(INF && DROP), "no dropout copy in the inference form");
  using C = xc::Cfg<H>;
  constexpr int M = C::M, NKT = C::NKT, QPW = C::QPW;
#ifdef TT_DIAG
  const int dbg = a.dbg;
#else
  constexpr int dbg = 0;
#endif
// ... 93 lines not shown
    for (int idx = 0; idx < NS; ++idx) {
      const bool has_next = idx + 1 < NS;
#pragma unroll
      for (int c = 0; c < xc::NCH; ++c) {
        if (c + 1 < xc::NCH || has_next) chunk(slots + ((c + 1) & 1) * C::SLOT, stgb + ((c + 1) & 1) * (xc::STG / 4));
#if XS_MPOLL
        if (tid == 0 && !(dbg & 32)) {
          if (c == 0 && idx > 0) xc_wait(cntB, (unsigned)(M * idx), ws);
          if (c == 4 && has_next) xc_wait(cntA, (unsigned)(M * (idx + 1)), ws);
        }
#endif
        __syncthreads();
#if XS_MPUB
        if (tid == 0 && c == 3 && publish) __hip_atomic_fetch_add(cntA, 1u, __ATOMIC_RELAXED, __HIP_MEMORY_SCOPE_AGENT);
        if (tid == 0 && c == 7 && publish) __hip_atomic_fetch_add(cntB, 1u, __ATOMIC_RELAXED, __HIP_MEMORY_SCOPE_AGENT);
#endif
      }
    }
    return;
  }
  uint32_t ho[QPW];
#pragma unroll
  for (int p = 0; p < QPW; ++p) {
    const int q = vw * QPW + p, kt = q >> 1, rb = q & 1;
    ho[p] = (uint32_t)(((rb * 16 + (lane & 15)) * H + kt * 32 + (lane >> 4) * 8) * 2);
  }
  const int cr = vt >> 3, u0 = (vt & 7) * 8, j = 64 * mem + u0;
  float bn[8];
  {
    const float4 b0 = *reinterpret_cast<const float4*>(R.bhn + j);
    const float4 b1 = *reinterpret_cast<const float4*>(R.bhn + j + 4);
    bn[0] = b0.x; bn[1] = b0.y; bn[2] = b0.z; bn[3] = b0.w;
    bn[4] = b1.x; bn[5] = b1.y; bn[6] = b1.z; bn[7] = b1.w;
  }
  const bf16_t* G = static_cast<const bf16_t*>(R.g);
  bf16_t* Yw = static_cast<bf16_t*>(R.y);
  bf16_t* X1 = static_cast<bf16_t*>(R.x1);
  bf16_t* S = static_cast<bf16_t*>(R.save);
  auto g_rsrc = [&](const Step& q) { return tt_rsrc_n(G + (long)(q.nrow > 0 ? q.rb0 : 0) * T_ * a.ldg, q.nrow > 0); };
  auto load_g = [&](const Step& q, __amdgpu_buffer_rsrc_t rG, int c, tt_u32x4 (&gx)[3]) {
    const uint32_t og = c * xc::CR + cr < q.nrow ? (uint32_t)(((c * xc::CR + cr) * T_ + q.t) * (int)a.ldg + j) * 2u
                                                  : xc::OOB;
#pragma unroll
    for (int g = 0; g < 3; ++g)
      gx[g] = (dbg & 2) ? tt_u32x4{0u, 0u, 0u, 0u} : __builtin_amdgcn_raw_buffer_load_b128(rG, (int)og, g * H * 2, XC_G_AUX);
  };
  tt_u32x4 hv[QPW];
  auto load_h = [&](const Step& q, int qidx, int c) {
    if (q.s == 0 || (dbg & 4)) {
#pragma unroll
      for (int p = 0; p < QPW; ++p) hv[p] = tt_u32x4{0u, 0u, 0u, 0u};
    } else {
#pragma unroll
      for (int p = 0; p < QPW; ++p)
        hv[p] = __builtin_amdgcn_raw_buffer_load_b128(rx[(qidx - 1) & 1], (int)ho[p], c * xc::CR * H * 2, 16);
    }
  };
  float st[xc::NCH][8];
  Step cur = step_of(0);
  __amdgpu_buffer_rsrc_t rGc = g_rsrc(cur);
  constexpr int GR = XS_GA < 2 ? 2 : 4;
  static_assert(XS_GA >= 1 && XS_GA < GR && xc::NCH % GR == 0, "gate-input ring");
  tt_u32x4 gq[GR][3];
#pragma unroll
  for (int c = 0; c < XS_GA; ++c) load_g(cur, rGc, c, gq[c]);
#pragma unroll
  for (int p = 0; p < QPW; ++p) hv[p] = tt_u32x4{0u, 0u, 0u, 0u};
  __syncthreads();
  if (XS_VPRIO) __builtin_amdgcn_s_setprio(1);
  for (int idx = 0; idx < NS; ++idx) {
    const bool has_next = idx + 1 < NS;
    const Step nxt = step_of(has_next ? idx + 1 : idx);
    const __amdgpu_buffer_rsrc_t rGn = g_rsrc(nxt);
    const long r0w = (long)(cur.nrow > 0 ? cur.rb0 : 0) * T_;
    const bool on = cur.nrow > 0;
    bf16_t* HF = static_cast<bf16_t*>(inf_hfin(a, rz));
    const __amdgpu_buffer_rsrc_t rY =
        INF ? tt_rsrc_n(Yw ? (const void*)(Yw + r0w * a.ldy) : G, on && Yw != nullptr) : tt_rsrc_n(Yw + r0w * a.ldy, on);
    const __amdgpu_buffer_rsrc_t rX1 =
        INF ? tt_rsrc_n(HF ? (const void*)(HF + (long)(on ? cur.rb0 : 0) * inf_ldf(a)) : G, on && HF != nullptr && cur.s == T_ - 1)
            : tt_rsrc_n(X1 ? X1 + r0w * a.ldy : Yw, on && X1 != nullptr);
    const __amdgpu_buffer_rsrc_t rS = INF ? tt_rsrc_n(G, false) : tt_rsrc_n(S + r0w * 4L * H, on);
    const __amdgpu_buffer_rsrc_t rdst_h = rx[idx & 1];
    const int t = cur.t;
    const bool first = cur.s == 0;
#pragma unroll
    for (int c = 0; c < xc::NCH; ++c) {
      const int gslot = c % GR, gnext = (c + XS_GA) % GR;
      if (c + XS_GA < xc::NCH) load_g(cur, rGc, c + XS_GA, gq[gnext]);
      else if (has_next) load_g(nxt, rGn, c + XS_GA - xc::NCH, gq[gnext]);
      {
        const int rr = c * xc::CR + cr;
        const bool ok = rr < cur.nrow;
        const float* gb = stgb + (c & 1) * (xc::STG / 4);
        float xr[8], xz[8], xn[8], lr[8], lz[8], ln[8], y[8], sr[8], sz[8], sn[8], sg[8];
        const tt_u32x4(&gcur)[3] = gq[gslot];
        unpack8(make_uint4(gcur[0][0], gcur[0][1], gcur[0][2], gcur[0][3]), xr);
        unpack8(make_uint4(gcur[1][0], gcur[1][1], gcur[1][2], gcur[1][3]), xz);
        unpack8(make_uint4(gcur[2][0], gcur[2][1], gcur[2][2], gcur[2][3]), xn);
#pragma unroll
        for (int h = 0; h < 2; ++h) {
          const float4 v0 = *reinterpret_cast<const float4*>(gb + stg_off(cr, 0 * 64 + u0 + 4 * h));
          const float4 v1 = *reinterpret_cast<const float4*>(gb + stg_off(cr, 1 * 64 + u0 + 4 * h));
          const float4 v2 = *reinterpret_cast<const float4*>(gb + stg_off(cr, 2 * 64 + u0 + 4 * h));
          lr[4 * h] = v0.x; lr[4 * h + 1] = v0.y; lr[4 * h + 2] = v0.z; lr[4 * h + 3] = v0.w;
          lz[4 * h] = v1.x; lz[4 * h + 1] = v1.y; lz[4 * h + 2] = v1.z; lz[4 * h + 3] = v1.w;
          ln[4 * h] = v2.x; ln[4 * h + 1] = v2.y; ln[4 * h + 2] = v2.z; ln[4 * h + 3] = v2.w;
        }
        const uint32_t grow = (uint32_t)(cur.rb0 + rr) * (uint32_t)T_ + (uint32_t)t;
#pragma unroll
        for (int e = 0; e < 8; ++e) {
          const float hp = first ? 0.f : st[c][e];
          if (dbg & 16) {
            y[e] = xr[e] + lr[e] + hp; sr[e] = xz[e] + lz[e]; sz[e] = xn[e] + ln[e]; sn[e] = bn[e]; sg[e] = hp;
          } else {
            gru_cell(xr[e], xz[e], xn[e], lr[e], lz[e], ln[e], bn[e], hp, y[e], sr[e], sz[e], sn[e], sg[e]);
          }
          st[c][e] = y[e];
        }
        const uint4 yb = pack8bf(y);
        if (fast) st16_buf(rdst_h, (uint32_t)(rr * H + j) * 2u, 0, yb);
        else st16_buf_sc1(rdst_h, (uint32_t)(rr * H + j) * 2u, 0, yb);
        asm volatile("" ::: "memory");
        const int lrow = rr * T_ + t;
        const bool okd = ok && !(dbg & 1);
        const uint32_t oy = okd ? (uint32_t)(lrow * (int)a.ldy + j) * 2u : xc::OOB;
        const uint32_t os = okd ? (uint32_t)(lrow * 4 * H + j) * 2u : xc::OOB;
        st16_buf_aux<XC_OUT_AUX>(rY, (int)oy, yb);
        if constexpr (INF) {
          st16_buf_aux<XC_OUT_AUX>(rS, (int)os, yb);
          st16_buf_aux<XC_OUT_AUX>(rS, (int)(os + 2u * H), yb);
          st16_buf_aux<XC_OUT_AUX>(rS, (int)(os + 4u * H), yb);
          st16_buf_aux<XC_OUT_AUX>(rS, (int)(os + 6u * H), yb);
          st16_buf_aux<XC_OUT_AUX>(rX1, (int)(okd ? (uint32_t)(rr * (int)a.ldf + j) * 2u : xc::OOB), yb);
        } else {
          st16_buf_aux<XC_OUT_AUX>(rS, (int)os, pack8bf(sr));
          st16_buf_aux<XC_OUT_AUX>(rS, (int)(os + 2u * H), pack8bf(sz));
          st16_buf_aux<XC_OUT_AUX>(rS, (int)(os + 4u * H), pack8bf(sn));
          st16_buf_aux<XC_OUT_AUX>(rS, (int)(os + 6u * H), pack8bf(sg));
          if constexpr (DROP) {
#pragma unroll
            for (int e = 0; e < 8; ++e)
              y[e] *= tt_dropout_scale(R.seed, R.row0 + grow, (uint32_t)(R.col0 + j + e), a.drop_thresh, a.inv_keep);
            st16_buf_aux<XC_OUT_AUX>(rX1, (int)oy, pack8bf(y));
          } else {
            st16_buf_aux<XC_OUT_AUX>(rX1, (int)oy, yb);
          }
        }
      }
      if (c == 3 || c == 7) asm volatile("s_nop 0\n\ts_waitcnt vmcnt(6)" ::: "memory");
      if (c + 2 < xc::NCH || has_next) {
#pragma unroll
        for (int p = 0; p < QPW; ++p)
          *reinterpret_cast<tt_u32x4*>(slots + (c & 1) * C::SLOT + (vw * QPW + p) * 1024 + lane * 16) = hv[p];
      }
      if (c + 3 < xc::NCH) load_h(cur, idx, c + 3);
      else if (has_next) load_h(nxt, idx + 1, c + 3 - xc::NCH);
      if (!XS_MPOLL && vt == 0 && !(dbg & 32)) {
        if (c == 0 && idx > 0) xc_wait(cntB, (unsigned)(M * idx), ws);
        if (c == 4 && has_next) xc_wait(cntA, (unsigned)(M * (idx + 1)), ws);
      }
      __syncthreads();
      if (!XS_MPUB && vt == 0 && c == 3 && publish) __hip_atomic_fetch_add(cntA, 1u, __ATOMIC_RELAXED, __HIP_MEMORY_SCOPE_AGENT);
      if (!XS_MPUB && vt == 0 && c == 7 && publish) __hip_atomic_fetch_add(cntB, 1u, __ATOMIC_RELAXED, __HIP_MEMORY_SCOPE_AGENT);
    }
    cur = nxt;
    rGc = rGn;
  }
}
#ifdef TT_DIAG
}
extern "C" int tt_diag_fwd_prof(unsigned long long* out) {
  return hipMemcpyFromSymbol(out, HIP_SYMBOL(g_fwd_prof), sizeof(g_fwd_prof)) == hipSuccess ? 0 : 1;
}
namespace {
#endif
bool gru_fwd_persistent(int dtype, int H) {
  if (dtype != TT_DT_BF16 || H % 64 != 0 || H > PH_MAX) return false;
  return tt::opt(tt::OPT_GRU_STEP) != 1;
}

}

static int bwd_rows(int B, int H, int nrec) {
  const int o = tt::opt(tt::OPT_GRU_BWD_ROWS);
  if (o == 64 || o == 128) return o;
  return (long)tt_ceil_div(H, 128) * tt_ceil_div(B, 128) * nrec <= 256 ? 64 : 128;
}
extern "C" int tt_gru_bias_rows(int B) { return tt_ceil_div(B, 64); }

extern "C" int tt_gru_fwd_launches(int dtype, int T, int H) { return gru_fwd_persistent(dtype, H) ? 1 : T; }

static bool gru_bwd_persistent(int dtype, int H) {
  const int o = tt::opt(tt::OPT_GRU_BWD_PERSIST);
  return dtype == TT_DT_BF16 && (H == 256 || H == 512 || (H == 1024 && o == 2)) &&
         tt::opt(tt::OPT_GRU_BWD_ROWS) != 64 && o != 0;
}
extern "C" int tt_gru_bwd_launches(int dtype, int T, int H) { return gru_bwd_persistent(dtype, H) ? 1 : T; }
extern "C" int tt_gru_bwd_carry_on_chip(int dtype, int T, int H) {
  (void)T;
  return TT_BWD_CREG != 0 && gru_bwd_persistent(dtype, H) && H <= 512 ? 1 : 0;
}

struct SideStream {
  hipStream_t s = nullptr;
  hipEvent_t fork = nullptr, join = nullptr;
};
static int side_stream(SideStream** out) {
  static SideStream ss[64];
  static std::mutex mu;
  int dev = 0;
  TT_CHECK_HIP(hipGetDevice(&dev));
  TT_CHECK_ARG(dev >= 0 && dev < 64, "tt_gru_bwd: device %d", dev);
  std::lock_guard<std::mutex> lock(mu);
  SideStream& x = ss[dev];
  if (!x.s) {
    SideStream n;
    TT_CHECK_HIP(hipStreamCreateWithFlags(&n.s, hipStreamNonBlocking));
    TT_CHECK_HIP(hipEventCreateWithFlags(&n.fork, hipEventDisableTiming));
    TT_CHECK_HIP(hipEventCreateWithFlags(&n.join, hipEventDisableTiming));
    x = n;
  }
  *out = &x;
  return 0;
}

constexpr int XC_MAX_GROUPS = 512;
constexpr long XC_HDR = 256;
struct XcGeo {
  XcWs w{};
  int grid = 0, ng = 0;
  long cnt_bytes = 0, img_off = 0, bytes = 0;
};

struct XcDev {
  int cus = 0;
  int occ[2][2] = {{0, 0}, {0, 0}};
  int occ_xs[2] = {0, 0};
  int occ_inf[2] = {0, 0};
  int occ_xs_inf = 0;
};
static std::mutex g_xc_mu;
static XcDev g_xc[64];

template <int H, bool DROP>
static const void* xc_kernel() {
  return reinterpret_cast<const void*>(&gru_fwd_xcp<H, DROP>);
}
template <bool DROP>
static const void* xs_kernel() {
  return reinterpret_cast<const void*>(&gru_fwd_xs<512, DROP>);
}
template <int H>
static const void* xc_infer_kernel() {
  return reinterpret_cast<const void*>(&gru_fwd_xcp<H, false, InfArgs>);
}
static const void* xs_infer_kernel() { return reinterpret_cast<const void*>(&gru_fwd_xs<512, false, InfArgs>); }
static bool xs_on(int H) { return H == 512 && tt::opt(tt::OPT_GRU_FWD_XS) != 0; }

static int xc_device(XcDev** out) {
  int dev = 0;
  TT_CHECK_HIP(hipGetDevice(&dev));
  TT_CHECK_ARG(dev >= 0 && dev < 64, "tt_gru_fwd: device %d", dev);
  std::lock_guard<std::mutex> lock(g_xc_mu);
  XcDev& x = g_xc[dev];
  if (!x.cus) {
    int cus = 0;
    TT_CHECK_HIP(hipDeviceGetAttribute(&cus, hipDeviceAttributeMultiprocessorCount, dev));
    const void* k[2][2] = {{xc_kernel<256, false>(), xc_kernel<256, true>()},
                           {xc_kernel<512, false>(), xc_kernel<512, true>()}};
    for (int h = 0; h < 2; ++h)
      for (int d = 0; d < 2; ++d) TT_CHECK_HIP(hipOccupancyMaxActiveBlocksPerMultiprocessor(&x.occ[h][d], k[h][d], xc::NT, 0));
    const void* kx[2] = {xs_kernel<false>(), xs_kernel<true>()};
    for (int d = 0; d < 2; ++d) TT_CHECK_HIP(hipOccupancyMaxActiveBlocksPerMultiprocessor(&x.occ_xs[d], kx[d], xs::NT, 0));
    const void* ki[2] = {xc_infer_kernel<256>(), xc_infer_kernel<512>()};
    for (int h = 0; h < 2; ++h) TT_CHECK_HIP(hipOccupancyMaxActiveBlocksPerMultiprocessor(&x.occ_inf[h], ki[h], xc::NT, 0));
    TT_CHECK_HIP(hipOccupancyMaxActiveBlocksPerMultiprocessor(&x.occ_xs_inf, xs_infer_kernel(), xs::NT, 0));
    x.cus = cus;
  }
  *out = &x;
  return 0;
}

static bool xc_geometry(const XcDev& dev, int dtype, int H, int nrec, int B, int T, long ldg, long ldy, bool drop,
// ... 77 lines not shown
  const hipError_t e = tt::opt(tt::OPT_GRU_XC_COOP)
                           ? hipLaunchCooperativeKernel(fn, dim3(g.grid), dim3(nt), args, 0, st)
                           : hipLaunchKernel(fn, dim3(g.grid), dim3(nt), args, 0, st);
  if (e == hipErrorCooperativeLaunchTooLarge) {
    (void)hipGetLastError();
    return 0;
  }
  TT_CHECK_HIP(e);
  TT_CHECK_LAUNCH("gru_fwd_xcp");
  *used = true;
  return 0;
}

extern "C" int tt_gru_fwd_launches_for(int dtype, int nrec, int B, int T, int H, long ldg, long ldy) {
  XcGeo g;
  bool ok = false;
  if (xc_plan(dtype, nrec, B, T, H, ldg, ldy, true, g, &ok) == 0 && ok) return 1;
  return tt_gru_fwd_launches(dtype, T, H);
}

template <typename A>
static int launch_fwd_seq(const A& a, int nrec, int B, int H, hipStream_t st) {
  const dim3 grid(tt_ceil_div(B, PR) * nrec);
  int depth = (H / 64) % 4 == 0 ? 4 : (H / 64) % 2 == 0 ? 2 : 1;
  depth = std::min(depth, tt::opt(tt::OPT_GRU_DEPTH));
#define TT_SEQ(D, N) (gru_fwd_seq<D, N, A>)
  if (depth >= 4 && H == 512) hipLaunchKernelGGL(TT_SEQ(4, 8), grid, dim3(PNT), 0, st, a);
  else if (depth >= 4 && H == 256) hipLaunchKernelGGL(TT_SEQ(4, 4), grid, dim3(PNT), 0, st, a);
  else if (depth >= 4) hipLaunchKernelGGL(TT_SEQ(4, 0), grid, dim3(PNT), 0, st, a);
  else if (depth == 2 && H == 512) hipLaunchKernelGGL(TT_SEQ(2, 8), grid, dim3(PNT), 0, st, a);
  else if (depth == 2 && H == 256) hipLaunchKernelGGL(TT_SEQ(2, 4), grid, dim3(PNT), 0, st, a);
  else if (depth == 2) hipLaunchKernelGGL(TT_SEQ(2, 0), grid, dim3(PNT), 0, st, a);
  else if (H == 512) hipLaunchKernelGGL(TT_SEQ(1, 8), grid, dim3(PNT), 0, st, a);
  else if (H == 256) hipLaunchKernelGGL(TT_SEQ(1, 4), grid, dim3(PNT), 0, st, a);
  else hipLaunchKernelGGL(TT_SEQ(1, 0), grid, dim3(PNT), 0, st, a);
#undef TT_SEQ
  TT_CHECK_LAUNCH("gru_fwd_seq");
  return 0;
}

template <typename A>
static int launch_fwd_steps(int dtype, A a, int nrec, int B, int T, int H, long ldg, long ldy, hipStream_t st) {
  const int esz = dtype == TT_DT_BF16 ? 2 : 4;
  int bmr = tt::opt(tt::OPT_GRU_FWD_STEP_ROWS);
  if (bmr != 128 && bmr != 256)
    bmr = (long)tt_ceil_div(H, 64) * tt_ceil_div(B, 256) * nrec >= 512 ? 256 : 128;
  const long span = (long)T * std::max({4L * H, ldy, ldg}) * esz;
  if (bmr == 256 && 256L * span >= (1L << 31)) bmr = 128;
  TT_CHECK_ARG((long)bmr * span < (1L << 31), "tt_gru_fwd: tile byte offsets exceed 2 GiB (B tile %d)", bmr);
  dim3 grid(tt_ceil_div(H, 64) * tt_ceil_div(B, bmr) * nrec);
  XcDev* xd = nullptr;
  TT_PROPAGATE(xc_device(&xd));
  const bool ring = tt::opt(tt::OPT_GRU_STEP_RING) >= 3 && (long)grid.x <= xd->cus;
#define TT_STEP(T, R, NS) (gru_fwd_step<T, R, NS, A>)
  for (int s = 0; s < T; ++s) {
    a.s = s;
    if (dtype == TT_DT_BF16) {
      if (bmr == 256) hipLaunchKernelGGL(TT_STEP(bf16_t, 256, 2), grid, dim3(512), 0, st, a);
      else if (ring) hipLaunchKernelGGL(TT_STEP(bf16_t, 128, 3), grid, dim3(256), 0, st, a);
      else hipLaunchKernelGGL(TT_STEP(bf16_t, 128, 2), grid, dim3(256), 0, st, a);
    } else {
      if (bmr == 256) hipLaunchKernelGGL(TT_STEP(float, 256, 2), grid, dim3(512), 0, st, a);
      else if (ring) hipLaunchKernelGGL(TT_STEP(float, 128, 3), grid, dim3(256), 0, st, a);
      else hipLaunchKernelGGL(TT_STEP(float, 128, 2), grid, dim3(256), 0, st, a);
    }
    TT_CHECK_LAUNCH("gru_fwd_step");
  }
#undef TT_STEP
  return 0;
}

extern "C" int tt_gru_fwd(int dtype, const tt_gru_fwd_rec* recs, int nrec, int B, int T, int H, long ldg,
                          long ldy, float drop_p, void* ws, long ws_bytes, void* stream) {
  TT_CHECK_ARG(dtype == TT_DT_F32 || dtype == TT_DT_BF16, "tt_gru_fwd: bad dtype");
  TT_CHECK_ARG(nrec >= 1 && nrec <= 4, "tt_gru_fwd: nrec %d", nrec);
  TT_CHECK_ARG(B > 0 && T > 0 && H > 0, "tt_gru_fwd: bad shape");
  TT_CHECK_ARG(ws_bytes >= 0 && (ws != nullptr || ws_bytes == 0), "tt_gru_fwd: ws / ws_bytes");
  const int esz = dtype == TT_DT_BF16 ? 2 : 4;
  TT_CHECK_ARG(H % 8 == 0 && (ldy * esz) % 16 == 0, "tt_gru_fwd: H=%d (multiple of 8)/ldy=%ld misaligned", H, ldy);
  TT_CHECK_ARG(drop_p >= 0.f && drop_p < 1.f, "tt_gru_fwd: drop_p");
  TT_CHECK_ARG(tt_ceil_div(B, 128) <= 65535, "tt_gru_fwd: B too large");
  TT_CHECK_ARG(128L * T * std::max({4L * H, ldy, ldg}) * esz < (1L << 31), "tt_gru_fwd: tile byte offsets exceed 2 GiB");
  FwdArgs a{};
  for (int i = 0; i < nrec; ++i) {
    const tt_gru_fwd_rec& r = recs[i];
    TT_CHECK_ARG(r.g && r.whh && r.bhn && r.y && r.save && r.hstate, "tt_gru_fwd: null pointer in rec %d", i);
    a.r[i] = FwdRec{r.g, r.whh, r.bhn, r.y, r.x1, r.save, r.hstate, r.dir, r.drop_seed, r.drop_col0, r.drop_row0};
  }
  a.B = B; a.T = T; a.H = H; a.ldg = ldg; a.ldy = ldy;
  a.drop_thresh = drop_p > 0.f ? (uint32_t)(drop_p * 16777216.0f + 0.5f) : 0u;
  a.inv_keep = drop_p > 0.f ? 1.0f / (1.0f - drop_p) : 1.0f;
#ifdef TT_DIAG
  if (const char* e = getenv("TT_GRU_DBG")) a.dbg = atoi(e);
#endif
  hipStream_t st = (hipStream_t)stream;
  if (dtype == TT_DT_BF16) {
    bool used = false;
    TT_PROPAGATE(gru_fwd_xc_launch(a, nrec, B, T, H, ldg, ldy, ws, ws_bytes, st, &used));
    if (used) return 0;
  }
  if (gru_fwd_persistent(dtype, H)) return launch_fwd_seq(a, nrec, B, H, st);
  return launch_fwd_steps(dtype, a, nrec, B, T, H, ldg, ldy, st);
}

extern "C" long tt_gru_infer_scratch_size(int dtype, int B, int T, int H, int final_only) {
  if ((dtype != TT_DT_F32 && dtype != TT_DT_BF16) || B <= 0 || T <= 0 || H <= 0) return 0;
  if (gru_fwd_persistent(dtype, H)) return 0;
  const long esz = dtype == TT_DT_BF16 ? 2 : 4;
  return 2L * B * H * 4 + (final_only ? 2L * B * H * esz : 0);
}

extern "C" int tt_gru_fwd_infer(int dtype, const tt_gru_infer_rec* recs, int nrec, int B, int T, int H, long ldg,
                                long ldy, long ldf, void* ws, long ws_bytes, void* stream) {
  TT_CHECK_ARG(dtype == TT_DT_F32 || dtype == TT_DT_BF16, "tt_gru_fwd_infer: bad dtype");
  TT_CHECK_ARG(nrec >= 1 && nrec <= 4, "tt_gru_fwd_infer: nrec %d", nrec);
  TT_CHECK_ARG(B > 0 && T > 0 && H > 0, "tt_gru_fwd_infer: bad shape");
  TT_CHECK_ARG(ws_bytes >= 0 && (ws != nullptr || ws_bytes == 0), "tt_gru_fwd_infer: ws / ws_bytes");
  const int esz = dtype == TT_DT_BF16 ? 2 : 4;
  TT_CHECK_ARG(H % 8 == 0 && (ldy * esz) % 16 == 0, "tt_gru_fwd_infer: H=%d (multiple of 8)/ldy=%ld misaligned", H, ldy);
  TT_CHECK_ARG(tt_ceil_div(B, 128) <= 65535, "tt_gru_fwd_infer: B too large");
  TT_CHECK_ARG(128L * T * std::max({4L * H, ldy, ldg}) * esz < (1L << 31),
               "tt_gru_fwd_infer: tile byte offsets exceed 2 GiB");
  const bool has_y = recs[0].y != nullptr, has_f = recs[0].hfinal != nullptr;
  TT_CHECK_ARG(has_y || has_f, "tt_gru_fwd_infer: neither y nor hfinal given");
  TT_CHECK_ARG(!has_f || (ldf >= H && (ldf * esz) % 16 == 0 && 256L * ldf * esz < (1L << 31)),
               "tt_gru_fwd_infer: ldf=%ld misaligned or below H", ldf);
  const bool persistent = gru_fwd_persistent(dtype, H);
  const long state = 2L * B * H * 4;
  InfArgs a{};
  for (int i = 0; i < nrec; ++i) {
    const tt_gru_infer_rec& r = recs[i];
    TT_CHECK_ARG(r.g && r.whh && r.bhn, "tt_gru_fwd_infer: null pointer in rec %d", i);
    TT_CHECK_ARG((r.y != nullptr) == has_y && (r.hfinal != nullptr) == has_f,
                 "tt_gru_fwd_infer: rec %d disagrees with rec 0 on y / hfinal", i);
    TT_CHECK_ARG(persistent || (r.scratch && ((uintptr_t)r.scratch & 15) == 0),
                 "tt_gru_fwd_infer: rec %d needs 16-byte aligned scratch (tt_gru_infer_scratch_size)", i);
    a.r[i] = FwdRec{r.g, r.whh, r.bhn, r.y, nullptr, nullptr, static_cast<float*>(r.scratch), r.dir, 0u, 0, 0u};
    for (int k = nrec; k < 4; ++k) a.hfin[k] = a.himg[k] = nullptr;
    a.hfin[i] = r.hfinal;
    a.himg[i] = r.scratch && !has_y ? static_cast<char*>(r.scratch) + state : nullptr;
  }
  a.B = B; a.T = T; a.H = H; a.ldg = ldg; a.ldy = ldy; a.ldf = ldf;
  a.inv_keep = 1.0f;
  hipStream_t st = (hipStream_t)stream;
  if (dtype == TT_DT_BF16) {
    bool used = false;
    TT_PROPAGATE(gru_fwd_xc_launch(a, nrec, B, T, H, ldg, ldy, ws, ws_bytes, st, &used));
    if (used) return 0;
  }
  if (persistent) return launch_fwd_seq(a, nrec, B, H, st);
  return launch_fwd_steps(dtype, a, nrec, B, T, H, ldg, ldy, st);
}

template <typename T, int BMR>
static void launch_bwd_step(int ring, dim3 grid, hipStream_t st, const BwdArgs& a) {
  if (ring >= 4) hipLaunchKernelGGL((gru_bwd_step<T, BMR, 4>), grid, dim3(256), 0, st, a);
  else if (ring == 3) hipLaunchKernelGGL((gru_bwd_step<T, BMR, 3>), grid, dim3(256), 0, st, a);
  else hipLaunchKernelGGL((gru_bwd_step<T, BMR>), grid, dim3(256), 0, st, a);
}

extern "C" int tt_gru_bwd(int dtype, const tt_gru_bwd_rec* recs, int nrec, int B, int T, int H, long ldy,
                          long ldd, long ldf, void* stream) {
  TT_CHECK_ARG(dtype == TT_DT_F32 || dtype == TT_DT_BF16, "tt_gru_bwd: bad dtype");
  TT_CHECK_ARG(nrec >= 1 && nrec <= 4, "tt_gru_bwd: nrec %d", nrec);
  TT_CHECK_ARG(B > 0 && T > 0 && H > 0, "tt_gru_bwd: bad shape");
  const int esz = dtype == TT_DT_BF16 ? 2 : 4;
  TT_CHECK_ARG(H % 8 == 0 && (ldd * esz) % 16 == 0, "tt_gru_bwd: H=%d (multiple of 8)/ldd=%ld misaligned", H, ldd);
  TT_CHECK_ARG(256L * T * std::max({ldd, ldy, 4L * H}) * esz < (1L << 31), "tt_gru_bwd: tile byte offsets exceed 2 GiB");
  hipStream_t st = (hipStream_t)stream;
  BwdArgs a{};
  for (int i = 0; i < nrec; ++i) {
    const tt_gru_bwd_rec& r = recs[i];
    TT_CHECK_ARG(r.save && r.y && r.whh && r.dgx && r.dgh && r.dhstate && r.dbias_part,
                 "tt_gru_bwd: null pointer in rec %d", i);
    a.r[i] = BwdRec{r.save, r.y, r.dy, r.dfinal, r.whh, r.dgx, r.dgh, r.dhstate, r.dbias_part, r.dir};
    TT_CHECK_HIP(hipMemsetAsync(r.dbias_part, 0, sizeof(float) * 4L * H * tt_gru_bias_rows(B), st));
  }
  a.B = B; a.T = T; a.H = H; a.ldy = ldy; a.ldd = ldd; a.ldf = ldf;
  a.skew = tt::opt(tt::OPT_GRU_BWD_SKEW);
#ifdef TT_DIAG
  if (const char* e = getenv("TT_GRU_DBG")) a.dbg = atoi(e);
#endif
  const int bmr = bwd_rows(B, H, nrec);
  if (gru_bwd_persistent(dtype, H)) {
    TT_CHECK_ARG(128L * T * std::max({ldd, ldy, 4L * H}) * esz < (1L << 31), "tt_gru_bwd: tile offsets exceed 2 GiB");
    const dim3 grid(tt_ceil_div(B, 128) * nrec);
    if (H == 1024) hipLaunchKernelGGL(gru_bwd_rows<1024>, grid, dim3(512), 0, st, a);
    else if (H == 512) hipLaunchKernelGGL(gru_bwd_rows<512>, grid, dim3(512), 0, st, a);
    else hipLaunchKernelGGL(gru_bwd_rows<256>, grid, dim3(512), 0, st, a);
    TT_CHECK_LAUNCH("gru_bwd_rows");
    return 0;
  }
  if (dtype == TT_DT_BF16 && H % 256 == 0 && bmr == 128 && tt::opt(tt::OPT_GRU_BWD_BIG) != 0) {
    const dim3 grid((H / 256) * tt_ceil_div(B, 256) * nrec);
    for (int s = T - 1; s >= 0; --s) {
      a.s = s;
      hipLaunchKernelGGL(gru_bwd_big, grid, dim3(512), 0, st, a);
      TT_CHECK_LAUNCH("gru_bwd_big");
    }
    return 0;
  }
  const int ngrp = (nrec >= 2 && tt::opt(tt::OPT_GRU_BWD_STREAMS) != 1) ? 2 : 1;
  BwdArgs ga[2] = {a, a};
  int gn[2] = {nrec, 0};
  if (ngrp == 2) {
    gn[0] = nrec / 2;
    gn[1] = nrec - gn[0];
    for (int i = 0; i < gn[1]; ++i) ga[1].r[i] = a.r[gn[0] + i];
  }
  hipStream_t gs[2] = {st, st};
  SideStream* side = nullptr;
  if (ngrp == 2) {
    TT_PROPAGATE(side_stream(&side));
    gs[1] = side->s;
    TT_CHECK_HIP(hipEventRecord(side->fork, st));
    TT_CHECK_HIP(hipStreamWaitEvent(side->s, side->fork, 0));
  }
  XcDev* xd = nullptr;
  TT_PROPAGATE(xc_device(&xd));
  long wgs = 0;
  for (int g = 0; g < ngrp; ++g) wgs += (long)tt_ceil_div(H, 128) * tt_ceil_div(B, bmr) * gn[g];
  const int ring = wgs <= xd->cus ? tt::opt(tt::OPT_GRU_STEP_RING) : 2;
  for (int s = T - 1; s >= 0; --s) {
    for (int g = 0; g < ngrp; ++g) {
      ga[g].s = s;
      const dim3 grid(tt_ceil_div(H, 128) * tt_ceil_div(B, bmr) * gn[g]);
      if (dtype == TT_DT_BF16) {
        if (bmr == 64) launch_bwd_step<bf16_t, 64>(ring, grid, gs[g], ga[g]);
        else launch_bwd_step<bf16_t, 128>(ring, grid, gs[g], ga[g]);
      } else {
        if (bmr == 64) launch_bwd_step<float, 64>(ring, grid, gs[g], ga[g]);
        else launch_bwd_step<float, 128>(ring, grid, gs[g], ga[g]);
      }
      TT_CHECK_LAUNCH("gru_bwd_step");
    }
  }
  if (ngrp == 2) {
    TT_CHECK_HIP(hipEventRecord(side->join, side->s));
    TT_CHECK_HIP(hipStreamWaitEvent(st, side->join, 0));
  }
  return 0;
}
```

two_towers_amd/csrc/tt_head.hip:

```cpp
#include <algorithm>
#include <climits>

#include "tt_api.h"
#include "tt_common.h"

namespace {

constexpr int LN_MAXC = 16;

template <typename T, typename TO>
__global__ __launch_bounds__(256) void ln_relu_fwd_kernel(const T* __restrict__ x, long rows, int C,
                                                          const float* __restrict__ gam,
                                                          const float* __restrict__ bet, float eps,
                                                          TO* __restrict__ u, float* __restrict__ mean,
                                                          float* __restrict__ rstd, uint32_t drop_seed,
                                                          uint32_t drop_thresh, float inv_keep) {
  const long row = (long)blockIdx.x * 4 + (threadIdx.x >> 6);
  const int lane = threadIdx.x & 63;
  if (row >= rows) return;
  const T* xr = x + row * C;
  float v[LN_MAXC];
  float s = 0.f;
#pragma unroll
  for (int q = 0; q < LN_MAXC; ++q) {
// ... 109 lines not shown
  *o_part = off; off = al(off + nblk * 4L * 2 * h * 4);
  const int s2 = tt_gemm_pick_splits(h, 2 * h, B, 1);
  const int s1 = tt_gemm_pick_splits(2 * h, 4 * h, B, 1);
  const long sk = std::max(tt_gemm_ws_size(h, 2 * h, 1, s2), tt_gemm_ws_size(2 * h, 4 * h, 1, s1));
  *o_sk = off; off = al(off + sk * 4);
  return off;
}

}

extern "C" long tt_proj_head_bwd_ws_size(int dtype, int B, int h) {
  long a, b, c, d, e;
  return head_ws_layout(dtype, B, h, &a, &b, &c, &d, &e);
}

extern "C" int tt_proj_head_fwd(int dtype, const tt_head_fwd_io* io, int ntower, int B, int h, float ln_eps,
                                void* stream) {
  TT_CHECK_ARG(ntower >= 1 && ntower <= 4, "tt_proj_head_fwd: ntower");
  TT_CHECK_ARG(2 * h <= 64 * LN_MAXC, "tt_proj_head_fwd: h=%d too large", h);
  hipStream_t st = (hipStream_t)stream;
  tt_gemm_batch g1{}, g2{};
  for (int i = 0; i < ntower; ++i) {
    g1.a[i] = io[i].x; g1.b[i] = io[i].w1; g1.c[i] = io[i].p1; g1.bias[i] = io[i].b1;
    g2.a[i] = io[i].u; g2.b[i] = io[i].w2; g2.c[i] = io[i].out; g2.bias[i] = io[i].b2;
  }
  TT_PROPAGATE(tt_gemm(dtype, dtype, 0, 0, B, 2 * h, 4 * h, &g1, ntower, 4 * h, 4 * h, 2 * h, 1.f, 0, 0, 0, 0,
                       0.f, 1, nullptr, stream));
  for (int i = 0; i < ntower; ++i) {
    dim3 grid(tt_ceil_div(B, 4));
    if (dtype == TT_DT_BF16)
      hipLaunchKernelGGL((ln_relu_fwd_kernel<bf16_t, bf16_t>), grid, dim3(256), 0, st, (const bf16_t*)io[i].p1,
                         (long)B, 2 * h, io[i].ln_g, io[i].ln_b, ln_eps, (bf16_t*)io[i].u, io[i].mean, io[i].rstd,
                         0u, 0u, 1.f);
    else
      hipLaunchKernelGGL((ln_relu_fwd_kernel<float, float>), grid, dim3(256), 0, st, (const float*)io[i].p1,
                         (long)B, 2 * h, io[i].ln_g, io[i].ln_b, ln_eps, (float*)io[i].u, io[i].mean, io[i].rstd,
                         0u, 0u, 1.f);
    TT_CHECK_LAUNCH("ln_relu_fwd_kernel");
  }
  TT_PROPAGATE(tt_gemm(dtype, TT_DT_F32, 0, 0, B, h, 2 * h, &g2, ntower, 2 * h, 2 * h, h, 1.f, 0, 0, 0, 0, 0.f, 1,
                       nullptr, stream));
  return 0;
}

extern "C" int tt_proj_head_bwd(int dtype, const tt_head_bwd_io* io, int ntower, int B, int h, float ln_eps,
                                void* stream) {
  (void)ln_eps;
  TT_CHECK_ARG(ntower >= 1 && ntower <= 4, "tt_proj_head_bwd: ntower");
  TT_CHECK_ARG(2 * h <= 64 * LN_MAXC, "tt_proj_head_bwd: h=%d too large", h);
  hipStream_t st = (hipStream_t)stream;
  long o_dout, o_du, o_dp1, o_part, o_sk;
  head_ws_layout(dtype, B, h, &o_dout, &o_du, &o_dp1, &o_part, &o_sk);
  const int C = 2 * h;
  const long nblk = tt_ceil_div(B, LN_ROWS_PER_BLOCK);
  for (int i = 0; i < ntower; ++i) {
    const tt_head_bwd_io& q = io[i];
    char* ws = static_cast<char*>(q.ws);
    void* dout_t = ws + o_dout;
    float* du = reinterpret_cast<float*>(ws + o_du);
    void* dp1 = ws + o_dp1;
    float* part = reinterpret_cast<float*>(ws + o_part);
    float* sk = reinterpret_cast<float*>(ws + o_sk);
    TT_PROPAGATE(tt_cast(dtype, q.dout, (long)B * h, dout_t, stream));
    {
      tt_gemm_batch g{};
      g.a[0] = dout_t; g.b[0] = q.u; g.c[0] = q.dw2;
      const int sp = tt_gemm_pick_splits(h, C, B, 1);
      TT_PROPAGATE(tt_gemm(dtype, TT_DT_F32, 1, 1, h, C, B, &g, 1, h, C, C, 1.f, 0, 0, 0, 0, 0.f, sp, sk, stream));
    }
    {
      tt_gemm_batch g{};
      g.a[0] = dout_t; g.b[0] = q.w2; g.c[0] = du;
      TT_PROPAGATE(tt_gemm(dtype, TT_DT_F32, 0, 1, B, C, h, &g, 1, h, C, C, 1.f, 0, 0, 0, 0, 0.f, 1, nullptr, stream));
    }
    if (dtype == TT_DT_BF16)
      hipLaunchKernelGGL((ln_relu_bwd_kernel<bf16_t, 4>), dim3(nblk), dim3(256), 0, st, du, (const bf16_t*)q.p1,
                         q.ln_g, q.ln_b, q.mean, q.rstd, (long)B, C, LN_ROWS_PER_BLOCK, (bf16_t*)dp1, part, 0u, 0u,
                         1.f, q.dout, h);
    else
      hipLaunchKernelGGL((ln_relu_bwd_kernel<float, 4>), dim3(nblk), dim3(256), 0, st, du, (const float*)q.p1,
                         q.ln_g, q.ln_b, q.mean, q.rstd, (long)B, C, LN_ROWS_PER_BLOCK, (float*)dp1, part, 0u, 0u,
                         1.f, q.dout, h);
    TT_CHECK_LAUNCH("ln_relu_bwd_kernel");
    TT_PROPAGATE(tt_colsum(part, nblk, C, 4L * C, q.dg, 0, stream));
    TT_PROPAGATE(tt_colsum(part + C, nblk, C, 4L * C, q.dbeta, 0, stream));
    TT_PROPAGATE(tt_colsum(part + 2 * C, nblk, C, 4L * C, q.db1, 0, stream));
    TT_PROPAGATE(tt_colsum(part + 3 * C, nblk, h, 4L * C, q.db2, 0, stream));
    {
      tt_gemm_batch g{};
      g.a[0] = dp1; g.b[0] = q.x; g.c[0] = q.dw1;
      const int sp = tt_gemm_pick_splits(C, 2 * C, B, 1);
      TT_PROPAGATE(tt_gemm(dtype, TT_DT_F32, 1, 1, C, 2 * C, B, &g, 1, C, 2 * C, 2 * C, 1.f, 0, 0, 0, 0, 0.f, sp, sk,
                           stream));
    }
    {
      tt_gemm_batch g{};
      g.a[0] = dp1; g.b[0] = q.w1; g.c[0] = q.dx;
      TT_PROPAGATE(tt_gemm(dtype, TT_DT_F32, 0, 1, B, 2 * C, C, &g, 1, C, 2 * C, 2 * C, 1.f, 0, 0, 0, 0, 0.f, 1,
                           nullptr, stream));
    }
  }
  return 0;
}

namespace {

inline long head1_ws_layout(int dtype, long rows, int C, long* o_dp1, long* o_part, long* o_sk) {
  const int esz = dtype == TT_DT_BF16 ? 2 : 4;
  auto al = [](long x) { return (x + 255) & ~255L; };
  long off = 0;
  *o_dp1 = off;  off = al(off + rows * C * esz);
  const long nblk = tt_ceil_div(rows, LN_ROWS_PER_BLOCK);
  *o_part = off; off = al(off + nblk * 3L * C * 4);
  const int sp = tt_gemm_pick_splits(C, 2 * C, (int)rows, 1);
  *o_sk = off;   off = al(off + tt_gemm_ws_size(C, 2 * C, 1, sp) * 4);
  return off;
}

inline void drop_params(float p, uint32_t* thresh, float* inv_keep) {
  *thresh = p > 0.f ? (uint32_t)(p * 16777216.0f + 0.5f) : 0u;
  *inv_keep = p > 0.f ? 1.f / (1.f - p) : 1.f;
}

}

extern "C" long tt_proj_head1_bwd_ws_size(int dtype, long rows, int C) {
  long a, b, c;
  return head1_ws_layout(dtype, rows, C, &a, &b, &c);
}

extern "C" int tt_proj_head1_fwd(int dtype, const tt_head1_fwd_io* io, long rows, int C, float ln_eps,
                                 float drop_p, uint32_t drop_seed, void* stream) {
  TT_CHECK_ARG(C >= 1 && C <= 64 * LN_MAXC, "tt_proj_head1_fwd: C=%d out of range", C);
  TT_CHECK_ARG(rows >= 1 && rows <= INT_MAX, "tt_proj_head1_fwd: rows");
  TT_CHECK_ARG(drop_p >= 0.f && drop_p < 1.f, "tt_proj_head1_fwd: drop_p");
  hipStream_t st = (hipStream_t)stream;
  tt_gemm_batch g{};
  g.a[0] = io->x; g.b[0] = io->w1; g.c[0] = io->p1; g.bias[0] = io->b1;
  TT_PROPAGATE(tt_gemm(dtype, dtype, 0, 0, (int)rows, C, 2 * C, &g, 1, 2 * C, 2 * C, C, 1.f, 0, 0, 0, 0, 0.f, 1,
                       nullptr, stream));
  uint32_t thresh;
  float inv_keep;
  drop_params(drop_p, &thresh, &inv_keep);
  dim3 grid(tt_ceil_div(rows, 4));
  if (dtype == TT_DT_BF16)
    hipLaunchKernelGGL((ln_relu_fwd_kernel<bf16_t, float>), grid, dim3(256), 0, st, (const bf16_t*)io->p1, rows, C,
                       io->ln_g, io->ln_b, ln_eps, io->out, io->mean, io->rstd, drop_seed, thresh, inv_keep);
  else
    hipLaunchKernelGGL((ln_relu_fwd_kernel<float, float>), grid, dim3(256), 0, st, (const float*)io->p1, rows, C,
                       io->ln_g, io->ln_b, ln_eps, io->out, io->mean, io->rstd, drop_seed, thresh, inv_keep);
  TT_CHECK_LAUNCH("ln_relu_fwd_kernel");
  return 0;
}

extern "C" int tt_proj_head1_bwd(int dtype, const tt_head1_bwd_io* io, long rows, int C, float drop_p,
                                 uint32_t drop_seed, void* stream) {
  TT_CHECK_ARG(C >= 1 && C <= 64 * LN_MAXC, "tt_proj_head1_bwd: C=%d out of range", C);
  TT_CHECK_ARG(rows >= 1 && rows <= INT_MAX, "tt_proj_head1_bwd: rows");
  TT_CHECK_ARG(drop_p >= 0.f && drop_p < 1.f, "tt_proj_head1_bwd: drop_p");
  hipStream_t st = (hipStream_t)stream;
  long o_dp1, o_part, o_sk;
  head1_ws_layout(dtype, rows, C, &o_dp1, &o_part, &o_sk);
  char* ws = static_cast<char*>(io->ws);
  void* dp1 = ws + o_dp1;
  float* part = reinterpret_cast<float*>(ws + o_part);
  float* sk = reinterpret_cast<float*>(ws + o_sk);
  uint32_t thresh;
  float inv_keep;
  drop_params(drop_p, &thresh, &inv_keep);
  const long nblk = tt_ceil_div(rows, LN_ROWS_PER_BLOCK);
// ... 28 lines not shown
```

two_towers_amd/ops.py:

```python
from __future__ import annotations

import ctypes
from typing import Sequence

import torch

from . import _lib
from ._lib import GemmBatch, call, dtype_code, ptr, stream_ptr


def _esz(dt: torch.dtype) -> int:
    return 2 if dt == torch.bfloat16 else 4


def pad_cols(e: int, dt: torch.dtype) -> int:
    epc = 128 // _esz(dt)
    return (e + epc - 1) // epc * epc


def gemm(a: Sequence[torch.Tensor], b: Sequence[torch.Tensor], c: Sequence[torch.Tensor], *, m: int, n: int,
         k: int, lda: int, ldb: int, ldc: int, a_kouter: bool, b_kouter: bool, dtype: torch.dtype,
         out_dtype: torch.dtype, bias: Sequence[torch.Tensor | None] | None = None,
         bshift: Sequence[int] | None = None, alpha: float = 1.0, accumulate: bool = False,
         relu: bool = False, seq_t: int = 0, drop_seed: int = 0, drop_p: float = 0.0, drop_row0: int = 0,
         splits: int | None = None, a_hi: Sequence[torch.Tensor] | None = None, a_split: int = 0):
    nb = len(a)
    assert 1 <= nb <= 4 and len(b) == nb and len(c) == nb
    bt = GemmBatch()
    for i in range(nb):
        assert a[i].dtype == dtype and b[i].dtype == dtype, (a[i].dtype, b[i].dtype, dtype)
        assert c[i].dtype == out_dtype, (c[i].dtype, out_dtype)
        bt.a[i] = a[i].data_ptr()
        bt.b[i] = b[i].data_ptr()
        bt.c[i] = c[i].data_ptr()
        bt.bias[i] = bias[i].data_ptr() if bias is not None and bias[i] is not None else None
        bt.bshift[i] = bshift[i] if bshift is not None else 0
        if a_split:
            bt.a_hi[i] = a_hi[i].data_ptr()
    bt.a_split = a_split
    bt.drop_row0 = drop_row0 & 0xFFFFFFFF
    lib = _lib.load()
    if splits is None:
        splits = lib.tt_gemm_pick_splits(m, n, k, nb)
    ws = None
    if splits > 1 and not relu and drop_p == 0.0:
        ws = torch.empty(lib.tt_gemm_ws_size(m, n, nb, splits), dtype=torch.float32, device=c[0].device)
    else:
        splits = 1
    call("tt_gemm", dtype_code(dtype), dtype_code(out_dtype), int(a_kouter), int(b_kouter), m, n, k,
         ctypes.byref(bt), nb, lda, ldb, ldc, alpha, int(accumulate), int(relu), seq_t, drop_seed & 0xFFFFFFFF,
         drop_p, splits, ptr(ws), stream_ptr(c[0].device))


def embed_gather(table: torch.Tensor, ids: torch.Tensor, out: torch.Tensor):
    assert ids.dtype == torch.int32 and ids.is_contiguous()
    assert table.dim() == 2 and out.shape[-1] == table.shape[1] and out.dtype == table.dtype
    call("tt_embed_gather", dtype_code(table.dtype), table.data_ptr(), table.shape[0], table.shape[1],
         ids.data_ptr(), ids.numel(), out.data_ptr(), stream_ptr(out.device))


def pack_rows(src: torch.Tensor, out: torch.Tensor):
    assert src.dtype == torch.float32 and src.is_contiguous()
    e = src.shape[-1]
    n = src.numel() // e
    call("tt_pack_rows", dtype_code(out.dtype), src.data_ptr(), n, e, out.shape[-1], out.data_ptr(),
         stream_ptr(out.device))


def cast(x: torch.Tensor, out: torch.Tensor):
    assert x.dtype == torch.float32 and x.is_contiguous() and out.numel() == x.numel()
    call("tt_cast", dtype_code(out.dtype), x.data_ptr(), x.numel(), out.data_ptr(), stream_ptr(out.device))


def colsum(x: torch.Tensor, rows: int, cols: int, ld: int, out: torch.Tensor, accumulate: bool = False):
    assert x.dtype == torch.float32 and out.dtype == torch.float32
    call("tt_colsum", x.data_ptr(), rows, cols, ld, out.data_ptr(), int(accumulate), stream_ptr(out.device))


def total(x: torch.Tensor, scale: float, out: torch.Tensor):
    call("tt_sum", x.data_ptr(), x.numel(), scale, out.data_ptr(), stream_ptr(out.device))


def l2norm_fwd(x: torch.Tensor, eps: float, dt: torch.dtype, want_f32: bool = True):
    assert x.dtype == torch.float32 and x.is_contiguous() and x.dim() == 2
    rows, cols = x.shape
    y = torch.empty(rows, cols, dtype=dt, device=x.device)
    y32 = y if dt == torch.float32 else (torch.empty_like(x) if want_f32 else None)
    norm = torch.empty(rows, dtype=torch.float32, device=x.device)
    call("tt_l2norm_fwd", dtype_code(dt), x.data_ptr(), rows, cols, eps, y.data_ptr(),
         None if y32 is y else ptr(y32), norm.data_ptr(), stream_ptr(x.device))
    return y, y32, norm


def l2norm_bwd(dy: torch.Tensor, y32: torch.Tensor, norm: torch.Tensor, eps: float, dx: torch.Tensor | None = None,
               accumulate: bool = False):
    assert dy.dtype == torch.float32 and dy.is_contiguous() and y32.dtype == torch.float32
    rows, cols = dy.shape
    if dx is None:
        dx = torch.empty_like(dy)
        accumulate = False
    call("tt_l2norm_bwd", dy.data_ptr(), y32.data_ptr(), norm.data_ptr(), rows, cols, eps, dx.data_ptr(),
         int(accumulate), stream_ptr(dy.device))
    return dx
```

two_towers_amd/towers.py:

```python
from __future__ import annotations

import ctypes
import os
import threading
from dataclasses import dataclass

import torch
import torch.nn.functional as F

from . import _lib, dist, ops, timing
from ._lib import GruBwdRec, GruFwdRec, GruInferRec, HeadBwdIO, HeadFwdIO, call, dtype_code, stream_ptr

PARAMS_PER_TOWER = 22
LN_EPS = 1e-5
HEAD_DT = torch.float32


def gru_param_names():
    names = []
    for layer in (0, 1):
        for sfx in ("", "_reverse"):
            for w in ("weight_ih", "weight_hh", "bias_ih", "bias_hh"):
                names.append(f"{w}_l{layer}{sfx}")
    return names
# ... 137 lines not shown
def reset_guard_if_reported(dev):
    dev = torch.device(dev)
    with _status_lock:
        due = dev in _guard_reset
        _guard_reset.discard(dev)
    if due:
        with torch.cuda.device(dev):
            step_guard(dev).zero_()


def watch_gru_status(ws, arm: bool = True):
    with torch.cuda.device(ws.device):
        st = torch.cuda.current_stream(ws.device)
        word = ws[:4].view(torch.int32)
        if arm:
            step_guard(ws.device).bitwise_or_(word)
        host = torch.zeros(1, dtype=torch.int32, pin_memory=True)
        host.copy_(word, non_blocking=True)
        ev = torch.cuda.Event()
        ev.record(st)
    with _status_lock:
        _status_pending.append((ev, host, torch.device(ws.device)))


def check_gru_status(wait: bool = True):
    with _status_lock:
        pend = list(_status_pending)
        _status_pending.clear()
    bad = 0
    keep = []
    bad_devs = set()
    for ev, host, dev in pend:
        if not wait and not ev.query():
            keep.append((ev, host, dev))
            continue
        ev.synchronize()
        if host.item() != 0:
            bad += 1
            bad_devs.add(dev)
    with _status_lock:
        if keep:
            _status_pending[:0] = keep
        _guard_reset.update(bad_devs)
    if bad:
        raise _lib.GruTimeoutError(
            f"{bad} column-split GRU forward launch(es) timed out waiting for a member workgroup "
            "(not all workgroups were resident); their outputs are invalid and the optimiser step "
            "that followed (two_towers_amd.Adam) left the weights unchanged. Set option gru_fwd_xc=0 "
            "(env TT_GRU_FWD_XC=0) to use the row-owning kernel.")


def _xs_selected() -> bool:
    try:
        return bool(_lib.get_option("gru_fwd_xs"))
    except _lib.TTError:
        return False


def table_cols(table, x):
    return getattr(table, "real_cols", table.shape[1])


def featurize(x: torch.Tensor, table: torch.Tensor | None, Ep: int, dt: torch.dtype) -> torch.Tensor:
    if x.dtype in (torch.int32, torch.int64):
        if table is None:
            raise _lib.TTError("integer token ids need an embedding table (model.set_embedding_table)")
        if table.dtype != dt or table.shape[1] != Ep:
            raise _lib.TTError(f"embedding table must be {dt} with {Ep} columns, got {table.dtype} {tuple(table.shape)}")
        ids = x.reshape(-1).to(torch.int32).contiguous()
        out = _alloc((ids.numel(), Ep), dt, x.device)
        esz = 2 if dt == torch.bfloat16 else 4
        gb = ids.numel() * (4 + 2 * table_cols(table, x) * esz)
        with timing.region("embed_gather", 1, gb, gb):
            ops.embed_gather(table, ids, out)
        return out
    if x.dim() != 3:
        raise ValueError(f"expected [B, T, E] embeddings or [B, T] token ids, got shape {tuple(x.shape)}")
    src = x.float().contiguous()
    out = _alloc((src.shape[0] * src.shape[1], Ep), dt, x.device)
    ops.pack_rows(src, out)
    return out


def _gru_layer_fwd(cfg, xs, K, ldx, packs, layer, B, T, seeds, want_x1, ws):
    n, H, dt, dev = cfg.ntowers, cfg.H, cfg.dtype, xs[0].device
    BT = B * T
    G = [_alloc((BT, 6 * H), dt, dev) for _ in range(n)]
    esz = 2 if dt == torch.bfloat16 else 4
    kr = cfg.E if layer == 0 else K
    with timing.region(f"input_proj_l{layer}", 1, 2.0 * BT * 6 * H * kr * n,
                       float(n * esz * (BT * kr + 6 * H * kr + BT * 6 * H))):
        ops.gemm(xs, [p.wih[layer] for p in packs], G, m=BT, n=6 * H, k=K, lda=ldx, ldb=K, ldc=6 * H,
                 a_kouter=False, b_kouter=False, dtype=dt, out_dtype=dt, bias=[p.bias[layer] for p in packs])
    Y = [_alloc((BT, 2 * H), dt, dev) for _ in range(n)]
    X1 = [_alloc((BT, 2 * H), dt, dev) for _ in range(n)] if want_x1 else None
    S = [[_alloc((BT, 4 * H), dt, dev) for _ in range(2)] for _ in range(n)]
    hs = _alloc((n * 2, 2, B, H), torch.float32, dev)
    recs = (GruFwdRec * (2 * n))()
    for ti in range(n):
        for d in range(2):
            r = recs[ti * 2 + d]
            r.g = G[ti][:, d * 3 * H:].data_ptr()
            r.whh = packs[ti].whh[layer][d].data_ptr()
            r.bhn = packs[ti].bhn[layer][d].data_ptr()
            r.y = Y[ti][:, d * H:].data_ptr()
            r.x1 = X1[ti][:, d * H:].data_ptr() if want_x1 else None
            r.save = S[ti][d].data_ptr()
            r.hstate = hs[ti * 2 + d].data_ptr()
            r.dir = d
            r.drop_seed = seeds[ti] & 0xFFFFFFFF
            r.drop_col0 = d * H
            r.drop_row0 = (cfg.rank * B * T) & 0xFFFFFFFF
    nl = _lib.load().tt_gru_fwd_launches_for(dtype_code(dt), 2 * n, B, T, H, 6 * H, 2 * H) if ws is not None \
        else _lib.load().tt_gru_fwd_launches(dtype_code(dt), T, H)
    per = esz * (8 + (1 if want_x1 else 0)) + (0 if nl == 1 else esz + 8)
    if nl == 1 and ws is not None:
        form = "gru_fwd_xs" if H == 512 and _xs_selected() else "gru_fwd_xcp"
        kname = f"{form}<{H}, {'true' if want_x1 and cfg.drop_p > 0 else 'false'}"
    elif nl == 1:
        kname = "gru_fwd_seq<"
    else:
        kname = "gru_fwd_step<"
    with timing.region("gru_fwd", nl, 2.0 * B * H * 3 * H * 2 * n * (T - 1), float(B * T * H * 2 * n * per),
                       kernel=kname):
        call("tt_gru_fwd", dtype_code(dt), recs, 2 * n, B, T, H, 6 * H, 2 * H, cfg.drop_p if want_x1 else 0.0,
             ws.data_ptr() if ws is not None else None, ws.numel() if ws is not None else 0, stream_ptr(dev))
    del G
    return Y, X1, S


def _gru_layer_infer(cfg, xs, K, ldx, packs, layer, B, T, ws, final_only):
    n, H, dt, dev = cfg.ntowers, cfg.H, cfg.dtype, xs[0].device
    BT = B * T
    lib = _lib.load()
    G = [_alloc((BT, 6 * H), dt, dev) for _ in range(n)]
    esz = 2 if dt == torch.bfloat16 else 4
    kr = cfg.E if layer == 0 else K
    with timing.region(f"input_proj_infer_l{layer}", 1, 2.0 * BT * 6 * H * kr * n,
                       float(n * esz * (BT * kr + 6 * H * kr + BT * 6 * H))):
        ops.gemm(xs, [p.wih[layer] for p in packs], G, m=BT, n=6 * H, k=K, lda=ldx, ldb=K, ldc=6 * H,
                 a_kouter=False, b_kouter=False, dtype=dt, out_dtype=dt, bias=[p.bias[layer] for p in packs])
    out = [_alloc((B, 2 * H) if final_only else (BT, 2 * H), dt, dev) for _ in range(n)]
    nb = lib.tt_gru_infer_scratch_size(dtype_code(dt), B, T, H, int(final_only))
    scr = _alloc((2 * n, nb), torch.uint8, dev) if nb > 0 else None
    recs = (GruInferRec * (2 * n))()
    for ti in range(n):
        for d in range(2):
            r = recs[ti * 2 + d]
            r.g = G[ti][:, d * 3 * H:].data_ptr()
            r.whh = packs[ti].whh[layer][d].data_ptr()
            r.bhn = packs[ti].bhn[layer][d].data_ptr()
            r.y = None if final_only else out[ti][:, d * H:].data_ptr()
            r.hfinal = out[ti][:, d * H:].data_ptr() if final_only else None
            r.scratch = scr[ti * 2 + d].data_ptr() if scr is not None else None
            r.dir = d
    nl = lib.tt_gru_fwd_launches_for(dtype_code(dt), 2 * n, B, T, H, 6 * H, 2 * H) if ws is not None \
        else lib.tt_gru_fwd_launches(dtype_code(dt), T, H)
    per = esz * (3 if final_only else 4) + (0 if nl == 1 else esz * (2 if final_only else 1) + 8)
    if nl == 1 and ws is not None:
        kname = f"{'gru_fwd_xs' if H == 512 and _xs_selected() else 'gru_fwd_xcp'}<{H}, false, (anonymous namespace)::InfArgs>"
    elif nl == 1:
        kname = "gru_fwd_seq<"
    else:
        kname = "gru_fwd_step<"
    with timing.region("gru_infer", nl, 2.0 * B * H * 3 * H * 2 * n * (T - 1), float(B * T * H * 2 * n * per),
                       kernel=kname):
        call("tt_gru_fwd_infer", dtype_code(dt), recs, 2 * n, B, T, H, 6 * H, 2 * H, 2 * H,
             ws.data_ptr() if ws is not None else None, ws.numel() if ws is not None else 0, stream_ptr(dev))
    return out


def towers_infer(cfg: TowerCfg, table, xs, params):
    n = cfg.ntowers
    _lib.require_gpu(*xs, *params)
    check_gru_status(wait=True)
    dt, E, H, h = cfg.dtype, cfg.E, cfg.H, cfg.h
    dev = xs[0].device
    reset_guard_if_reported(dev)
    B, T = xs[0].shape[0], xs[0].shape[1]
    for x in xs:
        if x.shape[0] != B or x.shape[1] != T:
            raise ValueError("query and doc inputs must share [B, T] in one fused call")
    Ep = ops.pad_cols(E, dt)
    npt = cfg.nparams
    with torch.no_grad():
        packs = [_packed(params[i * npt:(i + 1) * npt], cfg, Ep, True) for i in range(n)]
        X0 = [featurize(x, table, Ep, dt) for x in xs]
        ws = gru_fwd_workspace(2 * n, B, T, H, dt, dev)
        Y0 = _gru_layer_infer(cfg, X0, Ep, Ep, packs, 0, B, T, ws, False)
        del X0
        hfin = _gru_layer_infer(cfg, Y0, 2 * H, 2 * H, packs, 1, B, T, ws, True)
        del Y0
        if ws is not None:
            watch_gru_status(ws, arm=False)
        hcat = [f if f.dtype == HEAD_DT else f.to(HEAD_DT) for f in hfin]
        if cfg.head == "none":
            return tuple(hcat)
        outs, keep = [], []
        io = (HeadFwdIO * n)()
        for ti in range(n):
            pk = packs[ti]
            p1 = _alloc((B, 2 * h), HEAD_DT, dev)
            u = _alloc((B, 2 * h), HEAD_DT, dev)
            mean = _alloc((B,), torch.float32, dev)
            rstd = _alloc((B,), torch.float32, dev)
            out = _alloc((B, h), torch.float32, dev)
            q = io[ti]
            q.w1, q.b1, q.ln_g, q.ln_b = pk.w1.data_ptr(), pk.b1.data_ptr(), pk.ln_g.data_ptr(), pk.ln_b.data_ptr()
            q.w2, q.b2 = pk.w2.data_ptr(), pk.b2.data_ptr()
            q.x, q.p1, q.mean, q.rstd, q.u, q.out = (hcat[ti].data_ptr(), p1.data_ptr(), mean.data_ptr(),
                                                     rstd.data_ptr(), u.data_ptr(), out.data_ptr())
            outs.append(out)
            keep += [p1, u, mean, rstd]
        call("tt_proj_head_fwd", dtype_code(HEAD_DT), io, n, B, h, LN_EPS, stream_ptr(dev))
        return tuple(outs)


def _gru_layer_bwd(cfg, layer, B, T, S, Y, dY, dfinal, packs):
    n, H, dt, dev = cfg.ntowers, cfg.H, cfg.dtype, Y[0].device
    BT = B * T
    lib = _lib.load()
    dG = [_alloc((BT, 8 * H), dt, dev) for _ in range(n)]
    dhs = _alloc((n * 2, 2, B, H), dt, dev)
    nbr = lib.tt_gru_bias_rows(B)
    part = _alloc((n * 2, nbr, 4 * H), torch.float32, dev)
    recs = (GruBwdRec * (2 * n))()
    for ti in range(n):
        for d in range(2):
            r = recs[ti * 2 + d]
            r.save = S[ti][d].data_ptr()
            r.y = Y[ti][:, d * H:].data_ptr()
            r.dy = dY[ti][:, d * H:].data_ptr() if dY is not None else None
            r.dfinal = dfinal[ti][:, d * H:].data_ptr() if dfinal is not None else None
            r.whh = packs[ti].whh[layer][d].data_ptr()
            r.dgx = dG[ti][:, d * 3 * H:].data_ptr()
            r.dgh = dG[ti][:, 6 * H + d * H:].data_ptr()
            r.dhstate = dhs[ti * 2 + d].data_ptr()
            r.dbias_part = part[ti * 2 + d].data_ptr()
            r.dir = d
    ldf = dfinal[0].shape[1] if dfinal is not None else 0
    esz = 2 if dt == torch.bfloat16 else 4
    nl = lib.tt_gru_bwd_launches(dtype_code(dt), T, H)
    carry = 0 if lib.tt_gru_bwd_carry_on_chip(dtype_code(dt), T, H) else 2
    per = esz * (12 + carry + (1 if dY is not None else 0))
    kname = (f"gru_bwd_rows<{H}>" if nl == 1 else
             "gru_bwd_big" if dt == torch.bfloat16 and H % 256 == 0 and _lib.get_option("gru_bwd_big") else "gru_bwd_step<")
    with timing.region("gru_bwd", nl, 2.0 * B * 3 * H * H * 2 * n * (T - 1), float(B * T * H * 2 * n * per),
                       kernel=kname):
        call("tt_gru_bwd", dtype_code(dt), recs, 2 * n, B, T, H, 2 * H, 8 * H, ldf, stream_ptr(dev))
    sums = _alloc((n * 2, 4 * H), torch.float32, dev)
    for i in range(2 * n):
        ops.colsum(part[i], nbr, 4 * H, 4 * H, sums[i])
    dbih = [[sums[ti * 2 + d, : 3 * H] for d in range(2)] for ti in range(n)]
    dbhh = [[torch.cat([sums[ti * 2 + d, : 2 * H], sums[ti * 2 + d, 3 * H:]]) for d in range(2)] for ti in range(n)]
    return dG, dbih, dbhh


_WGRAD_T = os.environ.get("TT_WGRAD_T", "1") != "0"
WGRAD_OVERLAP = os.environ.get("TT_WGRAD_OVERLAP", "0") == "1"
_wgrad_streams: dict = {}


def _wgrad_stream(dev) -> torch.cuda.Stream:
    dev = torch.device(dev)
    with _status_lock:
        s = _wgrad_streams.get(dev)
        if s is None:
            s = _wgrad_streams[dev] = torch.cuda.Stream(device=dev)
    return s


def _weight_grads(cfg, B, T, dG, Xin, K, ldx, Y, kr=None):
    n, H, dt, dev = cfg.ntowers, cfg.H, cfg.dtype, dG[0].device
    BT = B * T
    dWih = [[_alloc((3 * H, K), torch.float32, dev) for _ in range(2)] for _ in range(n)]
    dWhh = [[_alloc((3 * H, H), torch.float32, dev) for _ in range(2)] for _ in range(n)]
    a_ih, b_ih, c_ih, a_hh, a_hi, b_hh, c_hh, sh = [], [], [], [], [], [], [], []
    for ti in range(n):
        for d in range(2):
            a_ih.append(dG[ti][:, d * 3 * H:])
            b_ih.append(Xin[ti])
            c_ih.append(dWih[ti][d])
            a_hh.append(dG[ti][:, d * 3 * H:])
            a_hi.append(dG[ti][:, 6 * H + d * H:])
            b_hh.append(Y[ti][:, d * H:])
            c_hh.append(dWhh[ti][d])
            sh.append(-1 if d == 0 else 1)
    esz = 2 if dt == torch.bfloat16 else 4
    kr = K if kr is None else kr
    with timing.region("wgrad_ih", 1, 2.0 * 3 * H * kr * BT * 2 * n,
                       float(n * (esz * BT * (6 * H + kr) + 2 * 3 * H * kr * 4))):
        if _WGRAD_T and dt == torch.bfloat16 and 0 < K % 256 <= 128:
            cT = [_alloc((K, 3 * H), torch.float32, dev) for _ in c_ih]
            ops.gemm(b_ih, a_ih, cT, m=K, n=3 * H, k=BT, lda=ldx, ldb=8 * H, ldc=3 * H, a_kouter=True,
                     b_kouter=True, dtype=dt, out_dtype=torch.float32)
            for c, ct in zip(c_ih, cT):
                c.copy_(ct.t())
        else:
            ops.gemm(a_ih, b_ih, c_ih, m=3 * H, n=K, k=BT, lda=8 * H, ldb=ldx, ldc=K, a_kouter=True,
                     b_kouter=True, dtype=dt, out_dtype=torch.float32)
    with timing.region("wgrad_hh", 1, 2.0 * 3 * H * H * BT * 2 * n,
                       float(n * (esz * BT * (6 * H + 2 * H) + 2 * 3 * H * H * 4))):
        ops.gemm(a_hh, b_hh, c_hh, m=3 * H, n=H, k=BT, lda=8 * H, ldb=2 * H, ldc=H, a_kouter=True, b_kouter=True,
                 dtype=dt, out_dtype=torch.float32, bshift=sh, seq_t=T, a_hi=a_hi, a_split=2 * H)
    return dWih, dWhh


class TowersFn(torch.autograd.Function):

    @staticmethod
    def forward(ctx, cfg: TowerCfg, table, group, cache_ok, *args):
        n = cfg.ntowers
        xs, params = args[:n], args[n:]
        _lib.require_gpu(*xs, *params)
        check_gru_status(wait=True)
        dt, E, H, h = cfg.dtype, cfg.E, cfg.H, cfg.h
        dev = xs[0].device
        reset_guard_if_reported(dev)
        B, T = xs[0].shape[0], xs[0].shape[1]
        for x in xs:
            if x.shape[0] != B or x.shape[1] != T:
                raise ValueError("query and doc inputs must share [B, T] in one fused call")
        Ep = ops.pad_cols(E, dt)
        npt = cfg.nparams
        packs = [_packed(params[i * npt:(i + 1) * npt], cfg, Ep, cache_ok) for i in range(n)]
        X0 = [featurize(x, table, Ep, dt) for x in xs]
        train_drop = cfg.drop_p > 0.0
        seeds = [int(torch.randint(0, 2 ** 31 - 1, (1,)).item()) for _ in range(n)] if train_drop else [0] * n
        ws = gru_fwd_workspace(2 * n, B, T, H, dt, dev)
        Y0, X1, S0 = _gru_layer_fwd(cfg, X0, Ep, Ep, packs, 0, B, T, seeds, train_drop, ws)
        Xl1 = X1 if train_drop else Y0
        Y1, _, S1 = _gru_layer_fwd(cfg, Xl1, 2 * H, 2 * H, packs, 1, B, T, seeds, False, ws)
        if ws is not None:
            watch_gru_status(ws, arm=any(ctx.needs_input_grad))
        hcat = []
        for ti in range(n):
            y = Y1[ti].view(B, T, 2 * H)
            hcat.append(torch.cat([y[:, T - 1, :H], y[:, 0, H:]], 1).to(HEAD_DT).contiguous())
        ctx.cfg = cfg
        ctx.group = group
        ctx.params = params
        ctx.dims = (B, T, Ep)
        ctx.seeds = seeds
        ctx.packs = packs
        if cfg.head == "none":
            ctx.acts = (X0, Y0, X1, S0, Y1, S1, None, None, None, None, None)
            return tuple(hcat)
        outs, p1s, means, rstds, us = [], [], [], [], []
        io = (HeadFwdIO * n)()
        for ti in range(n):
            pk = packs[ti]
            p1 = _alloc((B, 2 * h), HEAD_DT, dev)
            u = _alloc((B, 2 * h), HEAD_DT, dev)
            mean = _alloc((B,), torch.float32, dev)
            rstd = _alloc((B,), torch.float32, dev)
            out = _alloc((B, h), torch.float32, dev)
            q = io[ti]
            q.w1, q.b1, q.ln_g, q.ln_b = pk.w1.data_ptr(), pk.b1.data_ptr(), pk.ln_g.data_ptr(), pk.ln_b.data_ptr()
            q.w2, q.b2 = pk.w2.data_ptr(), pk.b2.data_ptr()
            q.x, q.p1, q.mean, q.rstd, q.u, q.out = (hcat[ti].data_ptr(), p1.data_ptr(), mean.data_ptr(),
                                                     rstd.data_ptr(), u.data_ptr(), out.data_ptr())
            outs.append(out); p1s.append(p1); means.append(mean); rstds.append(rstd); us.append(u)
        call("tt_proj_head_fwd", dtype_code(HEAD_DT), io, n, B, h, LN_EPS, stream_ptr(dev))
        ctx.acts = (X0, Y0, X1, S0, Y1, S1, hcat, p1s, means, rstds, us)
        return tuple(outs)

    @staticmethod
    def backward(ctx, *gouts):
        cfg = ctx.cfg
        check_gru_status(wait=False)
        n, dt, E, H, h = cfg.ntowers, cfg.dtype, cfg.E, cfg.H, cfg.h
        B, T, Ep = ctx.dims
        packs = ctx.packs
        X0, Y0, X1, S0, Y1, S1, hcat, p1s, means, rstds, us = ctx.acts
        dev = Y0[0].device
        lib = _lib.load()
        st = stream_ptr(dev)
        head_grads = [[] for _ in range(n)]
        dhcat = []
        if cfg.head == "none":
            for ti in range(n):
                g = gouts[ti]
                dhcat.append(torch.zeros(B, 2 * H, dtype=torch.float32, device=dev) if g is None
                             else g.float().contiguous())
        ws = None
        if cfg.head == "proj2":
            ws = _alloc((lib.tt_proj_head_bwd_ws_size(dtype_code(HEAD_DT), B, h),), torch.uint8, dev)
        for ti in range(n if cfg.head == "proj2" else 0):
            g = gouts[ti]
            g = torch.zeros(B, h, dtype=torch.float32, device=dev) if g is None else g.float().contiguous()
            pk = packs[ti]
            dx = _alloc((B, 2 * H), torch.float32, dev)
            dw1 = _alloc(pk.w1.shape, torch.float32, dev)
            db1 = _alloc((2 * h,), torch.float32, dev)
            dg = _alloc((2 * h,), torch.float32, dev)
            dbeta = _alloc((2 * h,), torch.float32, dev)
            dw2 = _alloc(pk.w2.shape, torch.float32, dev)
            db2 = _alloc((h,), torch.float32, dev)
            io = HeadBwdIO()
            io.w1, io.ln_g, io.ln_b, io.w2 = pk.w1.data_ptr(), pk.ln_g.data_ptr(), pk.ln_b.data_ptr(), pk.w2.data_ptr()
            io.x, io.p1, io.mean, io.rstd, io.u = (hcat[ti].data_ptr(), p1s[ti].data_ptr(), means[ti].data_ptr(),
                                                   rstds[ti].data_ptr(), us[ti].data_ptr())
            io.dout, io.dx = g.data_ptr(), dx.data_ptr()
            io.dw1, io.db1, io.dg, io.dbeta, io.dw2, io.db2 = (dw1.data_ptr(), db1.data_ptr(), dg.data_ptr(),
                                                               dbeta.data_ptr(), dw2.data_ptr(), db2.data_ptr())
            io.ws = ws.data_ptr()
            call("tt_proj_head_bwd", dtype_code(HEAD_DT), ctypes.byref(io), 1, B, h, LN_EPS, st)
            head_grads[ti] = [dw1, db1, dg, dbeta, dw2, db2]
            dhcat.append(dx)
        dG1, dbih1, dbhh1 = _gru_layer_bwd(cfg, 1, B, T, S1, Y1, None, dhcat, packs)
        Xl1 = X1 if X1 is not None else Y0
        red = dist.OverlapReducer(ctx.group[0]) if ctx.group is not None else None
        gl = [{} for _ in range(n)]

        def layer1_wgrads():
            dWih1, dWhh1 = _weight_grads(cfg, B, T, dG1, Xl1, 2 * H, 2 * H, Y1)
            _layer_grads(gl, 1, E, Ep, dWih1, dWhh1, dbih1, dbhh1)
            if red is not None:
                _reduce_into(red, gl, head_grads)

        main = torch.cuda.current_stream(dev)
        side = _wgrad_stream(dev) if WGRAD_OVERLAP else None
        if side is None:
            layer1_wgrads()
        dY0 = [_alloc((B * T, 2 * H), dt, dev) for _ in range(n)]
        esz = 2 if dt == torch.bfloat16 else 4
        with timing.region("dgrad_l1", 1, 2.0 * B * T * 2 * H * 6 * H * n,
                           float(n * esz * (B * T * 6 * H + B * T * 2 * H))):
            if X1 is None:
                ops.gemm(dG1, [p.wih[1] for p in packs], dY0, m=B * T, n=2 * H, k=6 * H, lda=8 * H, ldb=2 * H,
                         ldc=2 * H, a_kouter=False, b_kouter=True, dtype=dt, out_dtype=dt)
            else:
                for ti in range(n):
                    ops.gemm([dG1[ti]], [packs[ti].wih[1]], [dY0[ti]], m=B * T, n=2 * H, k=6 * H, lda=8 * H,
                             ldb=2 * H, ldc=2 * H, a_kouter=False, b_kouter=True, dtype=dt, out_dtype=dt,
                             drop_seed=ctx.seeds[ti], drop_p=cfg.drop_p, drop_row0=cfg.rank * B * T)
        if side is not None:
            side.wait_stream(main)
            for t in (*dG1, *Xl1, *Y1, *[g for hg in head_grads for g in hg], *[x for b in dbih1 for x in b],
                      *[x for b in dbhh1 for x in b]):
                t.record_stream(side)
            with torch.cuda.stream(side):
                layer1_wgrads()
        del dG1
        dG0, dbih0, dbhh0 = _gru_layer_bwd(cfg, 0, B, T, S0, Y0, dY0, None, packs)
        del dY0
        dWih0, dWhh0 = _weight_grads(cfg, B, T, dG0, X0, Ep, Ep, Y0, kr=E)
        gl0 = [{} for _ in range(n)]
        _layer_grads(gl0, 0, E, Ep, dWih0, dWhh0, dbih0, dbhh0)
        if side is not None:
            main.wait_stream(side)
            for t in [*[v for d in gl for v in d.values()], *[g for hg in head_grads for g in hg]]:
                t.record_stream(main)
        if red is not None:
            _reduce_into(red, gl0, [[] for _ in range(n)])
            red.finish(ctx.params)
        grads = []
        for ti in range(n):
            gl[ti].update(gl0[ti])
            grads.extend(gl[ti][k] for k in GRU_NAMES)
            grads.extend(head_grads[ti])
        ctx.acts = None
        ctx.packs = None
        ctx.params = None
        return (None, None, None, None, *([None] * n), *grads)


def _layer_grads(gl, layer, E, Ep, dWih, dWhh, dbih, dbhh):
    for ti in range(len(gl)):
        for d, sfx in enumerate(("", "_reverse")):
            w = dWih[ti][d]
            if layer == 0 and Ep != E:
                w = w[:, :E].contiguous()
            gl[ti][f"weight_ih_l{layer}{sfx}"] = w
            gl[ti][f"weight_hh_l{layer}{sfx}"] = dWhh[ti][d]
            gl[ti][f"bias_ih_l{layer}{sfx}"] = dbih[ti][d].contiguous()
            gl[ti][f"bias_hh_l{layer}{sfx}"] = dbhh[ti][d]


def _reduce_into(red, gl, head_grads):
    keys = [(ti, k) for ti in range(len(gl)) for k in gl[ti]]
    heads = [(ti, j) for ti in range(len(head_grads)) for j in range(len(head_grads[ti]))]
    views = red.launch([gl[ti][k] for ti, k in keys] + [head_grads[ti][j] for ti, j in heads])
    for (ti, k), v in zip(keys, views):
        gl[ti][k] = v
    for (ti, j), v in zip(heads, views[len(keys):]):
        head_grads[ti][j] = v


def run_towers(cfg: TowerCfg, table, xs, params, reduce_group=None, reduce: bool = False):
    if cfg.H % 8:
        raise ValueError(f"GRU hidden size {cfg.H} must be a multiple of 8 on the HIP path "
                         "(the step epilogues update 8 consecutive units per thread)")
    group = (reduce_group,) if reduce and dist.active(reduce_group) else None
    cache_ok = not (torch.is_grad_enabled() and any(p.requires_grad for p in params))
    if cache_ok and cfg.drop_p == 0.0:
        return towers_infer(cfg, table, xs, params)
    return TowersFn.apply(cfg, table, group, cache_ok, *xs, *params)
```

Before: 155,600 pairs/s.

## Fuse GRU final-state extraction, bias reductions, and transposed split-K wgrad stores

The GRU forward kernels now write the final hidden state of each direction directly into the head input buffer, so the slice, concat and cast step afterwards goes away. The per-direction bias column sums and the bias concat are replaced by one batched finish kernel, and the head's several colsum launches become one segmented colsum. The weight-gradient GEMM gains a strided split-K reduce that writes the transposed result straight into a trimmed output, skipping the temporary buffer and the transpose copy. These changes cut small launches and copies, at the cost of extra stores inside the recurrent kernels and more complex kernel code paths.

After: 155,700 pairs/s (median of 4 runs). Within noise of the previous version (+0.1%).

```diff
diff --git a/include/tt_hip.h b/include/tt_hip.h
--- a/include/tt_hip.h
+++ b/include/tt_hip.h
@@ -33,6 +33,8 @@
 int tt_cast(int dtype, const float* x, long n, void* y, void* stream);
 
 int tt_colsum(const float* x, long rows, int cols, long ld, float* out, int accumulate, void* stream);
+int tt_colsum_segments(const float* x, long rows, long ld, const int* cols, float* const* outs, int nseg,
+                       void* stream);
 
 typedef struct {
   const void* a[4];
@@ -43,6 +45,8 @@
   const void* a_hi[4];
   int a_split;
   uint32_t drop_row0;
+  long c_col_stride;
+  int c_row_limit;
 } tt_gemm_batch;
 
 int tt_gemm(int dtype, int out_dtype, int a_kouter, int b_kouter, int m, int n, int k,
@@ -64,6 +68,8 @@
   uint32_t drop_seed;
   int drop_col0;
   uint32_t drop_row0;
+  float* hfinal;
+  long ldf;
 } tt_gru_fwd_rec;
 
 int tt_gru_fwd(int dtype, const tt_gru_fwd_rec* recs, int nrec, int B, int T, int H, long ldg,
@@ -94,6 +100,7 @@
   void* dhstate;
   float* dbias_part;
   int dir;
+  int part_raw;
 } tt_gru_bwd_rec;
 
 int tt_gru_bwd(int dtype, const tt_gru_bwd_rec* recs, int nrec, int B, int T, int H, long ldy,
@@ -101,6 +108,13 @@
 int tt_gru_bwd_launches(int dtype, int T, int H);
 int tt_gru_bwd_carry_on_chip(int dtype, int T, int H);
 int tt_gru_bias_rows(int B);
+int tt_gru_bias_rows_filled(int dtype, int B, int T, int H);
+typedef struct {
+  const float* part;
+  float* dbih;
+  float* dbhh;
+} tt_gru_bias_rec;
+int tt_gru_bias_finish(const tt_gru_bias_rec* recs, int nrec, long rows, int H, void* stream);
 
 typedef struct {
   const void* w1; const float* b1; const float* ln_g; const float* ln_b;
diff --git a/two_towers_amd/_lib.py b/two_towers_amd/_lib.py
--- a/two_towers_amd/_lib.py
+++ b/two_towers_amd/_lib.py
@@ -34,6 +34,8 @@
         ("a_hi", c_void_p * 4),
         ("a_split", c_int),
         ("drop_row0", c_uint32),
+        ("c_col_stride", c_long),
+        ("c_row_limit", c_int),
     ]
 
 
@@ -55,7 +57,7 @@
     _fields_ = [
         ("g", c_void_p), ("whh", c_void_p), ("bhn", c_void_p), ("y", c_void_p), ("x1", c_void_p),
         ("save", c_void_p), ("hstate", c_void_p), ("dir", c_int), ("drop_seed", c_uint32),
-        ("drop_col0", c_int), ("drop_row0", c_uint32),
+        ("drop_col0", c_int), ("drop_row0", c_uint32), ("hfinal", c_void_p), ("ldf", c_long),
     ]
 
 
@@ -70,8 +72,12 @@
     _fields_ = [
         ("save", c_void_p), ("y", c_void_p), ("dy", c_void_p), ("dfinal", c_void_p), ("whh", c_void_p),
         ("dgx", c_void_p), ("dgh", c_void_p), ("dhstate", c_void_p), ("dbias_part", c_void_p),
-        ("dir", c_int),
-    ]
+        ("dir", c_int), ("part_raw", c_int),
+    ]
+
+
+class GruBiasRec(ctypes.Structure):
+    _fields_ = [("part", c_void_p), ("dbih", c_void_p), ("dbhh", c_void_p)]
 
 
 class HeadFwdIO(ctypes.Structure):
@@ -116,6 +122,7 @@
     "tt_pack_multi": (c_int, [c_void_p, c_int, c_void_p]),
     "tt_cast": (c_int, [c_int, c_void_p, c_long, c_void_p, c_void_p]),
     "tt_colsum": (c_int, [c_void_p, c_long, c_int, c_long, c_void_p, c_int, c_void_p]),
+    "tt_colsum_segments": (c_int, [c_void_p, c_long, c_long, POINTER(c_int), POINTER(c_void_p), c_int, c_void_p]),
     "tt_gemm": (c_int, [c_int, c_int, c_int, c_int, c_int, c_int, c_int, POINTER(GemmBatch), c_int, c_long,
                         c_long, c_long, c_float, c_int, c_int, c_int, c_uint32, c_float, c_int, c_void_p,
                         c_void_p]),
@@ -126,6 +133,8 @@
     "tt_gru_bwd": (c_int, [c_int, POINTER(GruBwdRec), c_int, c_int, c_int, c_int, c_long, c_long, c_long,
                            c_void_p]),
     "tt_gru_bias_rows": (c_int, [c_int]),
+    "tt_gru_bias_rows_filled": (c_int, [c_int, c_int, c_int, c_int]),
+    "tt_gru_bias_finish": (c_int, [POINTER(GruBiasRec), c_int, c_long, c_int, c_void_p]),
     "tt_gru_bwd_launches": (c_int, [c_int, c_int, c_int]),
     "tt_gru_bwd_carry_on_chip": (c_int, [c_int, c_int, c_int]),
     "tt_gru_fwd_launches": (c_int, [c_int, c_int, c_int]),
diff --git a/two_towers_amd/csrc/tt_elem.hip b/two_towers_amd/csrc/tt_elem.hip
--- a/two_towers_amd/csrc/tt_elem.hip
+++ b/two_towers_amd/csrc/tt_elem.hip
@@ -50,6 +50,55 @@
 #pragma unroll
     for (int w = 0; w < 16; ++w) t += red[w][lane];
     out[c] = accumulate ? out[c] + t : t;
+  }
+}
+
+struct ColsumSegArgs {
+  float* out[4];
+  int start[5];
+};
+__global__ __launch_bounds__(1024) void colsum_segments_kernel(const float* __restrict__ x, long rows, long ld,
+                                                               ColsumSegArgs a, int nseg) {
+  __shared__ float red[16][64];
+  const int wave = threadIdx.x >> 6, lane = threadIdx.x & 63;
+  const int c = blockIdx.x * 64 + lane, cols = a.start[nseg];
+  float s = 0.f;
+  if (c < cols)
+    for (long r = wave; r < rows; r += 16) s += x[r * ld + c];
+  red[wave][lane] = s;
+  __syncthreads();
+  if (wave == 0 && c < cols) {
+    float t = 0.f;
+#pragma unroll
+    for (int w = 0; w < 16; ++w) t += red[w][lane];
+    int k = 0;
+    while (k + 1 < nseg && c >= a.start[k + 1]) ++k;
+    a.out[k][c - a.start[k]] = t;
+  }
+}
+
+struct BiasFinishArgs {
+  const float* part[4];
+  float* dbih[4];
+  float* dbhh[4];
+};
+__global__ __launch_bounds__(1024) void gru_bias_finish_kernel(BiasFinishArgs a, long rows, int H) {
+  __shared__ float red[16][64];
+  const int wave = threadIdx.x >> 6, lane = threadIdx.x & 63;
+  const int c = blockIdx.x * 64 + lane, cols = 4 * H;
+  const float* x = a.part[blockIdx.y];
+  float s = 0.f;
+  if (c < cols)
+    for (long r = wave; r < rows; r += 16) s += x[r * cols + c];
+  red[wave][lane] = s;
+  __syncthreads();
+  if (wave == 0 && c < cols) {
+    float t = 0.f;
+#pragma unroll
+    for (int w = 0; w < 16; ++w) t += red[w][lane];
+    if (c < 3 * H) a.dbih[blockIdx.y][c] = t;
+    if (c < 2 * H) a.dbhh[blockIdx.y][c] = t;
+    else if (c >= 3 * H) a.dbhh[blockIdx.y][c - H] = t;
   }
 }
 
@@ -176,6 +225,40 @@
   return 0;
 }
 
+extern "C" int tt_colsum_segments(const float* x, long rows, long ld, const int* cols, float* const* outs, int nseg,
+                                  void* stream) {
+  TT_CHECK_ARG(nseg >= 1 && nseg <= 4 && cols && outs && x, "tt_colsum_segments: nseg %d not in [1,4]", nseg);
+  TT_CHECK_ARG(rows >= 0, "tt_colsum_segments: rows");
+  ColsumSegArgs a{};
+  for (int k = 0; k < nseg; ++k) {
+    TT_CHECK_ARG(cols[k] >= 0 && outs[k], "tt_colsum_segments: segment %d", k);
+    a.out[k] = outs[k];
+    a.start[k + 1] = a.start[k] + cols[k];
+  }
+  TT_CHECK_ARG(a.start[nseg] <= ld, "tt_colsum_segments: %d columns in rows of %ld", a.start[nseg], ld);
+  if (a.start[nseg] == 0) return 0;
+  hipLaunchKernelGGL(colsum_segments_kernel, dim3(tt_ceil_div(a.start[nseg], 64)), dim3(1024), 0, (hipStream_t)stream,
+                     x, rows, ld, a, nseg);
+  TT_CHECK_LAUNCH("colsum_segments_kernel");
+  return 0;
+}
+
+extern "C" int tt_gru_bias_finish(const tt_gru_bias_rec* recs, int nrec, long rows, int H, void* stream) {
+  TT_CHECK_ARG(nrec >= 1 && nrec <= 4 && recs, "tt_gru_bias_finish: nrec %d not in [1,4]", nrec);
+  TT_CHECK_ARG(rows >= 0 && H > 0, "tt_gru_bias_finish: bad shape");
+  BiasFinishArgs a{};
+  for (int i = 0; i < nrec; ++i) {
+    TT_CHECK_ARG(recs[i].part && recs[i].dbih && recs[i].dbhh, "tt_gru_bias_finish: null pointer in rec %d", i);
+    a.part[i] = recs[i].part;
+    a.dbih[i] = recs[i].dbih;
+    a.dbhh[i] = recs[i].dbhh;
+  }
+  hipLaunchKernelGGL(gru_bias_finish_kernel, dim3(tt_ceil_div(4 * H, 64), nrec), dim3(1024), 0, (hipStream_t)stream,
+                     a, rows, H);
+  TT_CHECK_LAUNCH("gru_bias_finish_kernel");
+  return 0;
+}
+
 extern "C" int tt_sum(const float* x, long n, float scale, float* out, void* stream) {
   hipLaunchKernelGGL(sum_kernel, dim3(1), dim3(256), 0, (hipStream_t)stream, x, n, scale, out);
   TT_CHECK_LAUNCH("sum_kernel");
diff --git a/two_towers_amd/csrc/tt_gemm.hip b/two_towers_amd/csrc/tt_gemm.hip
--- a/two_towers_amd/csrc/tt_gemm.hip
+++ b/two_towers_amd/csrc/tt_gemm.hip
@@ -1033,6 +1033,58 @@
       float x = v[u] * g.alpha;
       if (bias) x += bias[n0 + u];
       TO* p = C + (long)m * g.ldc + n0 + u;
+      if (g.beta) x += Elt<TO>::ld(p);
+      Elt<TO>::st(p, x);
+    }
+  }
+}
+
+template <typename TO, int V>
+__global__ __launch_bounds__(256) void splitk_reduce_strided_kernel(const float* ws, long part_stride, int splits,
+                                                                    int M, int N, long cs, int mlim, GemmArgs g) {
+  __shared__ float tile[32][33];
+  const int bi = blockIdx.y;
+  const float* P = ws + (long)bi * splits * part_stride;
+  TO* C = static_cast<TO*>(g.c[bi]);
+  const float* bias = g.bias[bi];
+  const int ntn = (N + 31) / 32;
+  const int m0 = (blockIdx.x / ntn) * 32, n0 = (blockIdx.x % ntn) * 32;
+  {
+    const int i = threadIdx.x >> 3, q = (threadIdx.x & 7) * 4;
+    const int m = m0 + i, n = n0 + q;
+    if (m < mlim && n < N) {
+      const float* p = P + (long)m * N + n;
+      float v[4] = {0.f, 0.f, 0.f, 0.f};
+      if constexpr (V == 4) {
+#pragma unroll 4
+        for (int s = 0; s < splits; ++s) {
+          const float4 b = *reinterpret_cast<const float4*>(p + (long)s * part_stride);
+          v[0] += b.x;
+          v[1] += b.y;
+          v[2] += b.z;
+          v[3] += b.w;
+        }
+      } else {
+        for (int s = 0; s < splits; ++s)
+#pragma unroll
+          for (int u = 0; u < 4; ++u)
+            if (n + u < N) v[u] += p[(long)s * part_stride + u];
+      }
+#pragma unroll
+      for (int u = 0; u < 4; ++u) {
+        float x = v[u] * g.alpha;
+        if (bias && n + u < N) x += bias[n + u];
+        tile[i][q + u] = x;
+      }
+    }
+  }
+  __syncthreads();
+  const int tx = threadIdx.x & 31, m = m0 + tx;
+  for (int i = threadIdx.x >> 5; i < 32; i += 8) {
+    const int n = n0 + i;
+    if (m < mlim && n < N) {
+      float x = tile[tx][i];
+      TO* p = C + (long)m * g.ldc + (long)n * cs;
       if (g.beta) x += Elt<TO>::ld(p);
       Elt<TO>::st(p, x);
     }
@@ -1466,6 +1518,9 @@
   g.kt_per_split = nk > 0 ? tt_ceil_div(nk, splits) : 1;
   splits = nk > 0 ? tt_ceil_div(nk, g.kt_per_split) : 1;
   g.splits = splits;
+  TT_CHECK_ARG(batch->c_col_stride >= 0 && batch->c_row_limit >= 0 && (batch->c_col_stride == 0 || splits > 1),
+               "tt_gemm: c_col_stride %ld / c_row_limit %d need a split-K reduction (splits %d after clamping)",
+               batch->c_col_stride, batch->c_row_limit, splits);
   {
     const int osz = out_dtype == TT_DT_BF16 ? 2 : 4;
     bool ok = (ldc * osz) % 16 == 0;
@@ -1488,6 +1543,20 @@
     int rc = dtype == TT_DT_BF16 ? launch_gemm<bf16_t, float>(a_kouter, b_kouter, shift, gp, nbatch, st)
                                  : launch_gemm<float, float>(a_kouter, b_kouter, shift, gp, nbatch, st);
     if (rc) return rc;
+    if (batch->c_col_stride != 0) {
+      const int mlim = batch->c_row_limit > 0 ? std::min(batch->c_row_limit, m) : m;
+      const bool v4 = n % 4 == 0 && (uintptr_t)splitk_ws % 16 == 0;
+      dim3 tg((unsigned)(tt_ceil_div(mlim, 32) * tt_ceil_div(n, 32)), nbatch);
+#define TT_REDS(TO, V) hipLaunchKernelGGL((splitk_reduce_strided_kernel<TO, V>), tg, dim3(256), 0, st, splitk_ws, gp.part_stride, splits, m, n, batch->c_col_stride, mlim, g)
+      if (out_dtype == TT_DT_F32) {
+        if (v4) TT_REDS(float, 4); else TT_REDS(float, 1);
+      } else {
+        if (v4) TT_REDS(bf16_t, 4); else TT_REDS(bf16_t, 1);
+      }
+#undef TT_REDS
+      TT_CHECK_LAUNCH("splitk_reduce_strided_kernel");
+      return 0;
+    }
     const bool v4 = n % 4 == 0 && (uintptr_t)splitk_ws % 16 == 0;
     const long total = (long)m * n / (v4 ? 4 : 1);
     dim3 rg((unsigned)std::min<long>(tt_ceil_div(total, 256), 2048), nbatch);
diff --git a/two_towers_amd/csrc/tt_gru.hip b/two_towers_amd/csrc/tt_gru.hip
--- a/two_towers_amd/csrc/tt_gru.hip
+++ b/two_towers_amd/csrc/tt_gru.hip
@@ -20,6 +20,8 @@
   int s;
   uint32_t drop_thresh;
   float inv_keep;
+  float* hf32[4];
+  long ldf32;
 #ifdef TT_DIAG
   int dbg;
 #endif
@@ -33,6 +35,18 @@
 TT_DEV void* inf_hfin(const InfArgs& a, int rz) { return a.hfin[rz]; }
 TT_DEV long inf_ldf(const FwdArgs&) { return 0; }
 TT_DEV long inf_ldf(const InfArgs& a) { return a.ldf; }
+
+template <typename T>
+TT_DEV void st8_final(float* p, const float (&y)[8]) {
+  if constexpr (std::is_same_v<T, float>) {
+    st8(p, y);
+  } else {
+    float f[8];
+#pragma unroll
+    for (int e = 0; e < 8; ++e) f[e] = bf2f(f2bf(y[e]));
+    st8(p, f);
+  }
+}
 
 struct BwdRec {
   const void* save; const void* y; const void* dy; const float* dfinal; const void* whh;
@@ -174,6 +188,7 @@
           continue;
         }
         st8(Yw + row * a.ldy + j, y);
+        if (a.hf32[rz] && s == T_ - 1) st8_final<T>(a.hf32[rz] + (long)b * a.ldf32 + j, y);
         const int so = (int)((((long)(b - m0) * T_) * 4L * H + j) * (long)sizeof(T));
         st8_sc1(srs, so, sr, (T*)nullptr);
         st8_sc1(srs, so + H * (int)sizeof(T), sz, (T*)nullptr);
@@ -1210,6 +1225,14 @@
     }
     __syncthreads();
   }
+  if constexpr (!INF) {
+    float* hf = a.hf32[rz];
+    if (hf && rowok) {
+#pragma unroll
+      for (int i = 0; i < PH_MAX / 64; ++i)
+        if (i < nblk) st8_final<bf16_t>(hf + (long)b * a.ldf32 + i * 64 + jg, hreg[i]);
+    }
+  }
 #ifdef TT_DIAG
   TT_STAMP(k_end);
   prf[7] = k_end - k_start;
@@ -1237,6 +1260,12 @@
 constexpr int STG = CR * 192 * 4;
 constexpr int CSTR = 64;
 constexpr unsigned OOB = 0x80000000u;
+}
+TT_DEV void xc_store_final(__amdgpu_buffer_rsrc_t r, uint32_t off, uint4 yb) {
+  st16_buf(r, off, 0, make_uint4(yb.x << 16, yb.x & 0xFFFF0000u, yb.y << 16, yb.y & 0xFFFF0000u));
+  st16_buf(r, off, 16, make_uint4(yb.z << 16, yb.z & 0xFFFF0000u, yb.w << 16, yb.w & 0xFFFF0000u));
+}
+namespace xc {
 template <int H>
 struct Cfg {
   static constexpr int M = H / 64;
@@ -1491,6 +1520,8 @@
             : tt_rsrc_n(X1 ? X1 + r0w * a.ldy : Yw, on && X1 != nullptr);
     const __amdgpu_buffer_rsrc_t rS = INF ? tt_rsrc_n(G, false) : tt_rsrc_n(S + r0w * 4L * H, on);
     const __amdgpu_buffer_rsrc_t rdst_h = rx[idx & 1];
+    float* hf32 = a.hf32[rz];
+    const __amdgpu_buffer_rsrc_t rHF = tt_rsrc_n(hf32 ? (const void*)(hf32 + (long)(on ? cur.rb0 : 0) * a.ldf32) : G, on && hf32 != nullptr);
     const int t = cur.t;
 #pragma unroll
     for (int c = 0; c < xc::NCH; ++c) {
@@ -1563,6 +1594,12 @@
         *reinterpret_cast<float4*>(stt + rr * xc::SSTR + u0) = make_float4(y[0], y[1], y[2], y[3]);
         *reinterpret_cast<float4*>(stt + rr * xc::SSTR + u0 + 4) = make_float4(y[4], y[5], y[6], y[7]);
         const uint4 yb = pack8bf(y);
+        if constexpr (!INF) {
+          if (hf32 && cur.s == T_ - 1) {
+            xc_store_final(rHF, ok ? (uint32_t)(rr * (int)a.ldf32 + j) * 4u : xc::OOB, yb);
+            asm volatile("" ::: "memory");
+          }
+        }
         if (fast) st16_buf(rdst_h, (uint32_t)(rr * H + j) * 2u, 0, yb);
         else st16_buf_sc1(rdst_h, (uint32_t)(rr * H + j) * 2u, 0, yb);
         asm volatile("" ::: "memory");
@@ -1822,6 +1859,8 @@
             : tt_rsrc_n(X1 ? X1 + r0w * a.ldy : Yw, on && X1 != nullptr);
     const __amdgpu_buffer_rsrc_t rS = INF ? tt_rsrc_n(G, false) : tt_rsrc_n(S + r0w * 4L * H, on);
     const __amdgpu_buffer_rsrc_t rdst_h = rx[idx & 1];
+    float* hf32 = a.hf32[rz];
+    const __amdgpu_buffer_rsrc_t rHF = tt_rsrc_n(hf32 ? (const void*)(hf32 + (long)(on ? cur.rb0 : 0) * a.ldf32) : G, on && hf32 != nullptr);
     const int t = cur.t;
     const bool first = cur.s == 0;
 #pragma unroll
@@ -1859,6 +1898,12 @@
           st[c][e] = y[e];
         }
         const uint4 yb = pack8bf(y);
+        if constexpr (!INF) {
+          if (hf32 && cur.s == T_ - 1) {
+            xc_store_final(rHF, ok && !(dbg & 1) ? (uint32_t)(rr * (int)a.ldf32 + j) * 4u : xc::OOB, yb);
+            asm volatile("" ::: "memory");
+          }
+        }
         if (fast) st16_buf(rdst_h, (uint32_t)(rr * H + j) * 2u, 0, yb);
         else st16_buf_sc1(rdst_h, (uint32_t)(rr * H + j) * 2u, 0, yb);
         asm volatile("" ::: "memory");
@@ -1940,6 +1985,10 @@
 extern "C" int tt_gru_bwd_carry_on_chip(int dtype, int T, int H) {
   (void)T;
   return TT_BWD_CREG != 0 && gru_bwd_persistent(dtype, H) && H <= 512 ? 1 : 0;
+}
+extern "C" int tt_gru_bias_rows_filled(int dtype, int B, int T, int H) {
+  (void)T;
+  return gru_bwd_persistent(dtype, H) ? tt_ceil_div(B, 128) : tt_gru_bias_rows(B);
 }
 
 struct SideStream {
@@ -2183,11 +2232,19 @@
   TT_CHECK_ARG(tt_ceil_div(B, 128) <= 65535, "tt_gru_fwd: B too large");
   TT_CHECK_ARG(128L * T * std::max({4L * H, ldy, ldg}) * esz < (1L << 31), "tt_gru_fwd: tile byte offsets exceed 2 GiB");
   FwdArgs a{};
+  const bool has_f = recs[0].hfinal != nullptr;
+  const long ldf = has_f ? recs[0].ldf : 0;
+  TT_CHECK_ARG(!has_f || (ldf >= H && ldf % 4 == 0 && 256L * ldf * 4 < (1L << 31)),
+               "tt_gru_fwd: hfinal ldf=%ld misaligned or below H", ldf);
   for (int i = 0; i < nrec; ++i) {
     const tt_gru_fwd_rec& r = recs[i];
     TT_CHECK_ARG(r.g && r.whh && r.bhn && r.y && r.save && r.hstate, "tt_gru_fwd: null pointer in rec %d", i);
+    TT_CHECK_ARG((r.hfinal != nullptr) == has_f && (!has_f || (r.ldf == ldf && ((uintptr_t)r.hfinal & 15) == 0)),
+                 "tt_gru_fwd: rec %d disagrees with rec 0 on hfinal / ldf, or hfinal is not 16-byte aligned", i);
     a.r[i] = FwdRec{r.g, r.whh, r.bhn, r.y, r.x1, r.save, r.hstate, r.dir, r.drop_seed, r.drop_col0, r.drop_row0};
-  }
+    a.hf32[i] = r.hfinal;
+  }
+  a.ldf32 = ldf;
   a.B = B; a.T = T; a.H = H; a.ldg = ldg; a.ldy = ldy;
   a.drop_thresh = drop_p > 0.f ? (uint32_t)(drop_p * 16777216.0f + 0.5f) : 0u;
   a.inv_keep = drop_p > 0.f ? 1.0f / (1.0f - drop_p) : 1.0f;
@@ -2275,7 +2332,8 @@
     TT_CHECK_ARG(r.save && r.y && r.whh && r.dgx && r.dgh && r.dhstate && r.dbias_part,
                  "tt_gru_bwd: null pointer in rec %d", i);
     a.r[i] = BwdRec{r.save, r.y, r.dy, r.dfinal, r.whh, r.dgx, r.dgh, r.dhstate, r.dbias_part, r.dir};
-    TT_CHECK_HIP(hipMemsetAsync(r.dbias_part, 0, sizeof(float) * 4L * H * tt_gru_bias_rows(B), st));
+    if (!r.part_raw || !tt_gru_bwd_carry_on_chip(dtype, T, H))
+      TT_CHECK_HIP(hipMemsetAsync(r.dbias_part, 0, sizeof(float) * 4L * H * tt_gru_bias_rows(B), st));
   }
   a.B = B; a.T = T; a.H = H; a.ldy = ldy; a.ldd = ldd; a.ldf = ldf;
   a.skew = tt::opt(tt::OPT_GRU_BWD_SKEW);
diff --git a/two_towers_amd/csrc/tt_head.hip b/two_towers_amd/csrc/tt_head.hip
--- a/two_towers_amd/csrc/tt_head.hip
+++ b/two_towers_amd/csrc/tt_head.hip
@@ -215,10 +215,11 @@
                          q.ln_g, q.ln_b, q.mean, q.rstd, (long)B, C, LN_ROWS_PER_BLOCK, (float*)dp1, part, 0u, 0u,
                          1.f, q.dout, h);
     TT_CHECK_LAUNCH("ln_relu_bwd_kernel");
-    TT_PROPAGATE(tt_colsum(part, nblk, C, 4L * C, q.dg, 0, stream));
-    TT_PROPAGATE(tt_colsum(part + C, nblk, C, 4L * C, q.dbeta, 0, stream));
-    TT_PROPAGATE(tt_colsum(part + 2 * C, nblk, C, 4L * C, q.db1, 0, stream));
-    TT_PROPAGATE(tt_colsum(part + 3 * C, nblk, h, 4L * C, q.db2, 0, stream));
+    {
+      const int cols[4] = {C, C, C, h};
+      float* const outs[4] = {q.dg, q.dbeta, q.db1, q.db2};
+      TT_PROPAGATE(tt_colsum_segments(part, nblk, 4L * C, cols, outs, 4, stream));
+    }
     {
       tt_gemm_batch g{};
       g.a[0] = dp1; g.b[0] = q.x; g.c[0] = q.dw1;
diff --git a/two_towers_amd/ops.py b/two_towers_amd/ops.py
--- a/two_towers_amd/ops.py
+++ b/two_towers_amd/ops.py
@@ -23,7 +23,8 @@
          out_dtype: torch.dtype, bias: Sequence[torch.Tensor | None] | None = None,
          bshift: Sequence[int] | None = None, alpha: float = 1.0, accumulate: bool = False,
          relu: bool = False, seq_t: int = 0, drop_seed: int = 0, drop_p: float = 0.0, drop_row0: int = 0,
-         splits: int | None = None, a_hi: Sequence[torch.Tensor] | None = None, a_split: int = 0):
+         splits: int | None = None, a_hi: Sequence[torch.Tensor] | None = None, a_split: int = 0,
+         c_col_stride: int = 0, c_row_limit: int = 0):
     nb = len(a)
     assert 1 <= nb <= 4 and len(b) == nb and len(c) == nb
     bt = GemmBatch()
@@ -39,6 +40,8 @@
             bt.a_hi[i] = a_hi[i].data_ptr()
     bt.a_split = a_split
     bt.drop_row0 = drop_row0 & 0xFFFFFFFF
+    bt.c_col_stride = c_col_stride
+    bt.c_row_limit = c_row_limit
     lib = _lib.load()
     if splits is None:
         splits = lib.tt_gemm_pick_splits(m, n, k, nb)
@@ -102,3 +105,23 @@
     call("tt_l2norm_bwd", dy.data_ptr(), y32.data_ptr(), norm.data_ptr(), rows, cols, eps, dx.data_ptr(),
          int(accumulate), stream_ptr(dy.device))
     return dx
+
+
+def gemm_splits(m: int, n: int, k: int, nb: int, dtype: torch.dtype) -> int:
+    s = _lib.load().tt_gemm_pick_splits(m, n, k, nb)
+    nk = (k * _esz(dtype) + 127) // 128
+    if nk <= 0 or s <= 1:
+        return 1
+    per = -(-nk // min(s, nk))
+    return -(-nk // per)
+
+
+def gru_bias_finish(part: torch.Tensor, rows: int, H: int, dbih: torch.Tensor, dbhh: torch.Tensor):
+    nrec = part.shape[0]
+    assert part.dtype == torch.float32 and part.is_contiguous() and part.shape[2] == 4 * H and rows <= part.shape[1]
+    assert dbih.shape == (nrec, 3 * H) and dbhh.shape == (nrec, 3 * H)
+    assert dbih.dtype == dbhh.dtype == torch.float32 and dbih.is_contiguous() and dbhh.is_contiguous()
+    recs = (_lib.GruBiasRec * nrec)()
+    for i in range(nrec):
+        recs[i].part, recs[i].dbih, recs[i].dbhh = part[i].data_ptr(), dbih[i].data_ptr(), dbhh[i].data_ptr()
+    call("tt_gru_bias_finish", recs, nrec, rows, H, stream_ptr(part.device))
diff --git a/two_towers_amd/towers.py b/two_towers_amd/towers.py
--- a/two_towers_amd/towers.py
+++ b/two_towers_amd/towers.py
@@ -243,7 +243,7 @@
     return out
 
 
-def _gru_layer_fwd(cfg, xs, K, ldx, packs, layer, B, T, seeds, want_x1, ws):
+def _gru_layer_fwd(cfg, xs, K, ldx, packs, layer, B, T, seeds, want_x1, ws, want_final=False):
     n, H, dt, dev = cfg.ntowers, cfg.H, cfg.dtype, xs[0].device
     BT = B * T
     G = [_alloc((BT, 6 * H), dt, dev) for _ in range(n)]
@@ -257,6 +257,7 @@
     X1 = [_alloc((BT, 2 * H), dt, dev) for _ in range(n)] if want_x1 else None
     S = [[_alloc((BT, 4 * H), dt, dev) for _ in range(2)] for _ in range(n)]
     hs = _alloc((n * 2, 2, B, H), torch.float32, dev)
+    hfin = [_alloc((B, 2 * H), HEAD_DT, dev) for _ in range(n)] if want_final else None
     recs = (GruFwdRec * (2 * n))()
     for ti in range(n):
         for d in range(2):
@@ -268,6 +269,9 @@
             r.x1 = X1[ti][:, d * H:].data_ptr() if want_x1 else None
             r.save = S[ti][d].data_ptr()
             r.hstate = hs[ti * 2 + d].data_ptr()
+            if want_final:
+                r.hfinal = hfin[ti][:, d * H:].data_ptr()
+                r.ldf = 2 * H
             r.dir = d
             r.drop_seed = seeds[ti] & 0xFFFFFFFF
             r.drop_col0 = d * H
@@ -287,7 +291,7 @@
         call("tt_gru_fwd", dtype_code(dt), recs, 2 * n, B, T, H, 6 * H, 2 * H, cfg.drop_p if want_x1 else 0.0,
              ws.data_ptr() if ws is not None else None, ws.numel() if ws is not None else 0, stream_ptr(dev))
     del G
-    return Y, X1, S
+    return Y, X1, S, hfin
 
 
 def _gru_layer_infer(cfg, xs, K, ldx, packs, layer, B, T, ws, final_only):
@@ -398,6 +402,7 @@
             r.dgh = dG[ti][:, 6 * H + d * H:].data_ptr()
             r.dhstate = dhs[ti * 2 + d].data_ptr()
             r.dbias_part = part[ti * 2 + d].data_ptr()
+            r.part_raw = 1
             r.dir = d
     ldf = dfinal[0].shape[1] if dfinal is not None else 0
     esz = 2 if dt == torch.bfloat16 else 4
@@ -409,11 +414,11 @@
     with timing.region("gru_bwd", nl, 2.0 * B * 3 * H * H * 2 * n * (T - 1), float(B * T * H * 2 * n * per),
                        kernel=kname):
         call("tt_gru_bwd", dtype_code(dt), recs, 2 * n, B, T, H, 2 * H, 8 * H, ldf, stream_ptr(dev))
-    sums = _alloc((n * 2, 4 * H), torch.float32, dev)
-    for i in range(2 * n):
-        ops.colsum(part[i], nbr, 4 * H, 4 * H, sums[i])
-    dbih = [[sums[ti * 2 + d, : 3 * H] for d in range(2)] for ti in range(n)]
-    dbhh = [[torch.cat([sums[ti * 2 + d, : 2 * H], sums[ti * 2 + d, 3 * H:]]) for d in range(2)] for ti in range(n)]
+    bih = _alloc((2 * n, 3 * H), torch.float32, dev)
+    bhh = _alloc((2 * n, 3 * H), torch.float32, dev)
+    ops.gru_bias_finish(part, lib.tt_gru_bias_rows_filled(dtype_code(dt), B, T, H), H, bih, bhh)
+    dbih = [[bih[ti * 2 + d] for d in range(2)] for ti in range(n)]
+    dbhh = [[bhh[ti * 2 + d] for d in range(2)] for ti in range(n)]
     return dG, dbih, dbhh
 
 
@@ -452,11 +457,18 @@
     with timing.region("wgrad_ih", 1, 2.0 * 3 * H * kr * BT * 2 * n,
                        float(n * (esz * BT * (6 * H + kr) + 2 * 3 * H * kr * 4))):
         if _WGRAD_T and dt == torch.bfloat16 and 0 < K % 256 <= 128:
-            cT = [_alloc((K, 3 * H), torch.float32, dev) for _ in c_ih]
-            ops.gemm(b_ih, a_ih, cT, m=K, n=3 * H, k=BT, lda=ldx, ldb=8 * H, ldc=3 * H, a_kouter=True,
-                     b_kouter=True, dtype=dt, out_dtype=torch.float32)
-            for c, ct in zip(c_ih, cT):
-                c.copy_(ct.t())
+            if ops.gemm_splits(K, 3 * H, BT, len(c_ih), dt) > 1:
+                for ti in range(n):
+                    for d in range(2):
+                        dWih[ti][d] = c_ih[ti * 2 + d] = _alloc((3 * H, kr), torch.float32, dev)
+                ops.gemm(b_ih, a_ih, c_ih, m=K, n=3 * H, k=BT, lda=ldx, ldb=8 * H, ldc=1, a_kouter=True,
+                         b_kouter=True, dtype=dt, out_dtype=torch.float32, c_col_stride=kr, c_row_limit=kr)
+            else:
+                cT = [_alloc((K, 3 * H), torch.float32, dev) for _ in c_ih]
+                ops.gemm(b_ih, a_ih, cT, m=K, n=3 * H, k=BT, lda=ldx, ldb=8 * H, ldc=3 * H, a_kouter=True,
+                         b_kouter=True, dtype=dt, out_dtype=torch.float32)
+                for c, ct in zip(c_ih, cT):
+                    c.copy_(ct.t())
         else:
             ops.gemm(a_ih, b_ih, c_ih, m=3 * H, n=K, k=BT, lda=8 * H, ldb=ldx, ldc=K, a_kouter=True,
                      b_kouter=True, dtype=dt, out_dtype=torch.float32)
@@ -489,15 +501,11 @@
         train_drop = cfg.drop_p > 0.0
         seeds = [int(torch.randint(0, 2 ** 31 - 1, (1,)).item()) for _ in range(n)] if train_drop else [0] * n
         ws = gru_fwd_workspace(2 * n, B, T, H, dt, dev)
-        Y0, X1, S0 = _gru_layer_fwd(cfg, X0, Ep, Ep, packs, 0, B, T, seeds, train_drop, ws)
+        Y0, X1, S0, _ = _gru_layer_fwd(cfg, X0, Ep, Ep, packs, 0, B, T, seeds, train_drop, ws)
         Xl1 = X1 if train_drop else Y0
-        Y1, _, S1 = _gru_layer_fwd(cfg, Xl1, 2 * H, 2 * H, packs, 1, B, T, seeds, False, ws)
+        Y1, _, S1, hcat = _gru_layer_fwd(cfg, Xl1, 2 * H, 2 * H, packs, 1, B, T, seeds, False, ws, want_final=True)
         if ws is not None:
             watch_gru_status(ws, arm=any(ctx.needs_input_grad))
-        hcat = []
-        for ti in range(n):
-            y = Y1[ti].view(B, T, 2 * H)
-            hcat.append(torch.cat([y[:, T - 1, :H], y[:, 0, H:]], 1).to(HEAD_DT).contiguous())
         ctx.cfg = cfg
         ctx.group = group
         ctx.params = params
@@ -631,11 +639,11 @@
     for ti in range(len(gl)):
         for d, sfx in enumerate(("", "_reverse")):
             w = dWih[ti][d]
-            if layer == 0 and Ep != E:
+            if layer == 0 and w.shape[1] != E:
                 w = w[:, :E].contiguous()
             gl[ti][f"weight_ih_l{layer}{sfx}"] = w
             gl[ti][f"weight_hh_l{layer}{sfx}"] = dWhh[ti][d]
-            gl[ti][f"bias_ih_l{layer}{sfx}"] = dbih[ti][d].contiguous()
+            gl[ti][f"bias_ih_l{layer}{sfx}"] = dbih[ti][d]
             gl[ti][f"bias_hh_l{layer}{sfx}"] = dbhh[ti][d]
 
 
```
